# thangvubk/SoftGroup

Measured on AMD Instinct MI355X. Metric: scans/sec ScanNet-v2-like inference (softgroup_scannet.yaml, full forward_test), higher is better.
Workload: dtype f32

## Files before the change

### include/softgroup_hip.h

```cpp
#ifndef SOFTGROUP_HIP_H
#define SOFTGROUP_HIP_H

#include <stddef.h>
#include <stdint.h>

#ifdef __cplusplus
extern "C" {
#endif

typedef void *sg_stream_t;

#define SG_OK 0
#define SG_ERR_ARG (-1)
#define SG_ERR_WORKSPACE (-2)
#define SG_ERR_LAUNCH (-3)
#define SG_ERR_UNSUPPORTED (-4)

#define SG_BALLQUERY_MAX_NEIGHBORS 1000
#define SG_OCTREE_NUM_NODES 585
#define SG_OCTREE_NUM_LEAVES 512
#define SG_LISTS_SORTED 1
#define SG_LISTS_RADIUS 2

int sg_version(void);
const char *sg_last_error(void);
int sg_device_info(char *name_host, int name_cap, int *num_cu_host, int *clock_khz_host);

int sg_stream_release(sg_stream_t stream);
int sg_stream_create(sg_stream_t *stream_out);
int sg_stream_destroy(sg_stream_t stream);
int sg_stream_create_priority(sg_stream_t *stream_out, int level);

int sg_voxelize_idx_host(const int64_t *coords_host, int n, int ncol, int mode,
                         int32_t *input_map_host, int32_t *num_voxels_host,
                         int32_t *max_active_host);
int sg_voxelize_idx_fill_host(const int64_t *coords_host, int n, int ncol, int mode,
                              const int32_t *input_map_host, int num_voxels, int max_active,
                              int64_t *out_coords_host, int32_t *out_map_host);
size_t sg_voxelize_idx_workspace_bytes(int n);
int sg_voxelize_idx_build(const int64_t *coords, int n, int ncol, int mode, int32_t *input_map,
                          int32_t *meta, void *ws, size_t ws_bytes, sg_stream_t stream);
int sg_voxelize_idx_fill(const int64_t *coords, int n, int ncol, int mode,
                         const int32_t *input_map, int num_voxels, int max_active,
                         int64_t *out_coords, int32_t *out_map, void *ws, size_t ws_bytes,
                         sg_stream_t stream);

int sg_voxelize_fp(const float *feats, const int32_t *rules, int num_voxels, int max_active,
                   int channels, int average, float *out, sg_stream_t stream);
int sg_voxelize_bp(const float *d_out, const int32_t *rules, int num_voxels, int max_active,
                   int channels, int average, float *d_feats, sg_stream_t stream);

size_t sg_ballquery_workspace_bytes(int n);
int sg_ballquery_build_grid(const float *xyz, const int32_t *batch_idxs, int n, float radius,
                            void *ws, size_t ws_bytes, sg_stream_t stream);
int sg_ballquery_count(const float *xyz, const int32_t *batch_idxs, int n, float radius,
                       int32_t *start_len, int32_t *meta, void *ws, size_t ws_bytes,
                       sg_stream_t stream);
int sg_ballquery_fill(const float *xyz, const int32_t *batch_idxs, int n, float radius,
                      const int32_t *start_len, int32_t *idx, void *ws, size_t ws_bytes,
                      sg_stream_t stream);
size_t sg_scan_workspace_bytes(int n);
int sg_exclusive_scan_startlen(int32_t *start_len, int n, int32_t *meta, void *ws,
                               size_t ws_bytes, sg_stream_t stream);

int sg_octree_build_host(const float *points_host, const float *xyzwhl_host, int num_points,
                         int num_levels, float *boxes_host, int32_t *pt_inds_host,
                         int32_t *pt_start_len_host);
size_t sg_octree_build_workspace_bytes(int n);
int sg_octree_build(const float *points, int n, float *boxes, int32_t *pt_inds, int32_t *pt_start_len,
                    void *ws, size_t ws_bytes, sg_stream_t stream);
size_t sg_pyramid_inverse_map_workspace_bytes(int n_points, int n_voxels, int n_prop);
int sg_pyramid_inverse_map(const int32_t *proposals_idx, int64_t num_pairs, int n_prop,
                           const int32_t *l2p_map, int n_points, int n_voxels, int32_t *out_idx,
                           int32_t *out_offsets, int32_t *n_out_dev, void *ws, size_t ws_bytes,
                           sg_stream_t stream);
int sg_octree_ballquery_count(const float *points, const float *boxes, const int32_t *pt_inds,
                              const int32_t *pt_start_len, int n, float radius,
                              int32_t *start_len, sg_stream_t stream);
int sg_octree_ballquery_fill(const float *points, const float *boxes, const int32_t *pt_inds,
                             const int32_t *pt_start_len, int n, float radius,
                             const int32_t *start_len, int32_t *idx, sg_stream_t stream);

size_t sg_bfs_workspace_bytes(int n, int64_t n_edges);
int sg_bfs_cluster_label(const int32_t *bq_idxs, const int32_t *start_len, int n,
// ... 558 lines not shown
```

### softgroup_amd/_lib.py

```python
import ctypes as C
import os

_HERE = os.path.dirname(os.path.abspath(__file__))
LIB_PATH = os.path.join(_HERE, 'lib', os.environ.get('SG_LIB_NAME', 'libsoftgroup_hip.so'))

_lib = None

_vp, _i, _f, _i64, _sz, _d = C.c_void_p, C.c_int, C.c_float, C.c_int64, C.c_size_t, C.c_double
_pi32 = C.POINTER(C.c_int32)

SIGNATURES = {
    'sg_version': (_i, []),
    'sg_last_error': (C.c_char_p, []),
    'sg_device_info': (_i, [C.c_char_p, _i, C.POINTER(_i), C.POINTER(_i)]),
    'sg_stream_release': (_i, [_vp]),
    'sg_host_copy_2d': (_i, [_vp, _i64, _vp, _i64, _i64, _i64]),
    'sg_host_cast_f64_f32': (_i, [_vp, _vp, _i64]),
    'sg_host_fill_i64_strided': (_i, [_vp, _i64, _i64, _i64]),
    'sg_host_colmax_i64': (_i, [_vp, _i64, _i64, _vp]),
    'sg_stream_create': (_i, [_vp]),
    'sg_stream_create_priority': (_i, [_vp, _i]),
    'sg_stream_destroy': (_i, [_vp]),
    'sg_voxelize_idx_host': (_i, [_vp, _i, _i, _i, _vp, _pi32, _pi32]),
    'sg_voxelize_idx_fill_host': (_i, [_vp, _i, _i, _i, _vp, _i, _i, _vp, _vp]),
    'sg_voxelize_idx_workspace_bytes': (_sz, [_i]),
    'sg_voxelize_idx_build': (_i, [_vp, _i, _i, _i, _vp, _vp, _vp, _sz, _vp]),
    'sg_voxelize_idx_fill': (_i, [_vp, _i, _i, _i, _vp, _i, _i, _vp, _vp, _vp, _sz, _vp]),
    'sg_voxelize_fp': (_i, [_vp, _vp, _i, _i, _i, _i, _vp, _vp]),
    'sg_voxelize_bp': (_i, [_vp, _vp, _i, _i, _i, _i, _vp, _vp]),
    'sg_ballquery_workspace_bytes': (_sz, [_i]),
    'sg_ballquery_build_grid': (_i, [_vp, _vp, _i, _f, _vp, _sz, _vp]),
    'sg_ballquery_count': (_i, [_vp, _vp, _i, _f, _vp, _vp, _vp, _sz, _vp]),
    'sg_ballquery_fill': (_i, [_vp, _vp, _i, _f, _vp, _vp, _vp, _sz, _vp]),
    'sg_scan_workspace_bytes': (_sz, [_i]),
    'sg_exclusive_scan_startlen': (_i, [_vp, _i, _vp, _vp, _sz, _vp]),
    'sg_octree_build_host': (_i, [_vp, _vp, _i, _i, _vp, _vp, _vp]),
    'sg_octree_build_workspace_bytes': (_sz, [_i]),
    'sg_octree_build': (_i, [_vp, _i, _vp, _vp, _vp, _vp, _sz, _vp]),
    'sg_pyramid_inverse_map_workspace_bytes': (_sz, [_i, _i, _i]),
    'sg_pyramid_inverse_map': (_i, [_vp, _i64, _i, _vp, _i, _i, _vp, _vp, _vp, _vp, _sz, _vp]),
    'sg_octree_ballquery_count': (_i, [_vp, _vp, _vp, _vp, _i, _f, _vp, _vp]),
    'sg_octree_ballquery_fill': (_i, [_vp, _vp, _vp, _vp, _i, _f, _vp, _vp, _vp]),
    'sg_bfs_workspace_bytes': (_sz, [_i, _i64]),
    'sg_bfs_cluster_label': (_i, [_vp, _vp, _i, _i64, _i, _vp, _vp, _i, _pi32, _pi32, _vp, _sz, _vp]),
    'sg_bfs_cluster_emit': (_i, [_vp, _vp, _i, _i64, _vp, _vp, _i, _i, _vp, _vp, _vp, _sz, _vp]),
    'sg_sec_mean': (_i, [_vp, _vp, _i, _i, _vp, _vp]),
    'sg_sec_min': (_i, [_vp, _vp, _i, _i, _vp, _vp]),
    'sg_sec_max': (_i, [_vp, _vp, _i, _i, _vp, _vp]),
    'sg_global_avg_pool_fp': (_i, [_vp, _vp, _i, _i, _vp, _vp]),
    'sg_global_avg_pool_bp': (_i, [_vp, _vp, _vp, _i, _i, _vp]),
    'sg_get_mask_iou_on_cluster': (_i, [_vp, _vp, _vp, _vp, _i, _i, _vp, _vp]),
    'sg_get_mask_iou_on_pred': (_i, [_vp, _vp, _vp, _vp, _vp, _i, _i, _vp, _vp]),
    'sg_get_mask_label': (_i, [_vp, _vp, _vp, _vp, _vp, _i, _i, _f, _vp, _vp]),
    'sg_spconv_hash_workspace_bytes': (_sz, [_i]),
    'sg_spconv_subm_rulebook': (_i, [_vp, _i, _pi32, _vp, _vp, _sz, _vp]),
    'sg_spconv_pyramid_workspace_bytes': (_sz, [_i, _i]),
    'sg_spconv_pyramid_rows': (_i, [_vp, _i, _pi32, _i, _vp, _vp, _sz, _vp]),
    'sg_spconv_pyramid_build_workspace_bytes': (_sz, [_vp, _i]),
    'sg_spconv_pyramid_build': (_i, [_vp, _i, _pi32, _i, _vp, _vp, _sz, _vp, _sz, _vp]),
    'sg_spconv_down_build': (_i, [_vp, _i, _pi32, _vp, _vp, _vp, _sz, _vp]),
    'sg_spconv_down_fill': (_i, [_vp, _i, _vp, _i, _vp, _vp, _vp, _sz, _vp]),
    'sg_spconv_inverse_rulebook': (_i, [_vp, _vp, _i, _vp, _vp]),
    'sg_spconv_plan_workspace_bytes': (_sz, [_i]),
    'sg_spconv_plan': (_i, [_vp, _i, _i, _vp, _vp, _vp, _vp, _sz, _vp]),
    'sg_spconv_set_arithmetic': (_i, [_i]),
    'sg_spconv_set_combine': (_i, [_i]),
    'sg_spconv_set_chain': (_i, [_i]),
    'sg_spconv_chain_stats': (_i, [_vp, _vp]),
# ... 162 lines not shown
```

### softgroup_amd/csrc/bfs.hip

```cpp
#include <stdlib.h>

#include <map>
#include <mutex>
#include <utility>

#include "common.h"
#include "scan.h"

namespace sg {

constexpr int kCap = SG_BALLQUERY_MAX_NEIGHBORS;
constexpr int kEmitThreads = 512;
constexpr int kEmitWaves = kEmitThreads / 64;

#define SG_LD(p) __hip_atomic_load((p), __ATOMIC_RELAXED, __HIP_MEMORY_SCOPE_AGENT)
#define SG_ST(p, v) __hip_atomic_store((p), (v), __ATOMIC_RELAXED, __HIP_MEMORY_SCOPE_AGENT)

struct BfsWs {
  int32_t *parent, *lab, *size, *cid, *coff, *owner, *seeds, *ebase, *wcnt, *asym_nodes;
  int4 *label;
  int2 *erec;
  int32_t *counters;
  void *scan_ws;
  size_t scan_bytes;
  int32_t *big_stage[2];
  unsigned long long *big_rec[2];
};

constexpr int kBigFastWgs = 16;
constexpr int kBigSlice = 8192;
constexpr int kBigClusterMin = 16384;
inline bool big_fast_on() {
  const char *e = getenv("SG_BFS_BIG_FAST");
  return !(e && atoi(e) == 0);
}
inline int thin_levels_on() {
  const char *e = getenv("SG_BFS_THIN");
  return e ? atoi(e) : 0;
}
inline bool big_local_on() {
  const char *e = getenv("SG_BFS_BIG_LOCAL");
  return !(e && atoi(e) == 0);
}
inline size_t big_stage_entries(int n) {
  return n > kBigClusterMin && big_fast_on() ? static_cast<size_t>(n) + static_cast<size_t>(kBigFastWgs) * kBigSlice : 0;
}

static bool bfs_carve(void *ws, size_t ws_bytes, int n, int64_t n_edges, BfsWs *w) {
  Workspace a(ws, ws_bytes);
  const size_t nn = static_cast<size_t>(n > 0 ? n : 1);
  w->parent = a.take<int32_t>(nn);
  w->lab = a.take<int32_t>(nn);
  w->label = a.take<int4>(nn);
  w->size = a.take<int32_t>(nn);
  w->cid = a.take<int32_t>(nn);
  w->coff = a.take<int32_t>(nn);
  w->owner = a.take<int32_t>(nn);
  w->seeds = a.take<int32_t>(nn);
  w->ebase = a.take<int32_t>(nn);
  w->wcnt = a.take<int32_t>(nn);
  w->asym_nodes = a.take<int32_t>(nn);
  w->counters = a.take<int32_t>(64);
  w->scan_bytes = scan_workspace_bytes(n);
  w->scan_ws = a.take<char>(w->scan_bytes);
  w->erec = a.take<int2>(static_cast<size_t>(n_edges > 0 ? n_edges : 1));
  bool ok = w->scan_ws != nullptr && w->erec != nullptr;
  const size_t be = big_stage_entries(n);
  for (int i = 0; i < 2; ++i) {
    w->big_stage[i] = be ? a.take<int32_t>(be) : nullptr;
    w->big_rec[i] = be ? a.take<unsigned long long>(be) : nullptr;
    ok = ok && (be == 0 || (w->big_stage[i] != nullptr && w->big_rec[i] != nullptr));
  }
  return ok;
}

__device__ __forceinline__ int uf_find(int32_t *parent, int x) {
  int cur = SG_LD(&parent[x]);
  if (cur != x) {
    int prev = x, next;
    while (cur > (next = SG_LD(&parent[cur]))) {
      SG_ST(&parent[prev], next);
      prev = cur;
      cur = next;
    }
  }
  return cur;
}

__device__ __forceinline__ void uf_union(int32_t *parent, int a, int b) {
  while (a != b) {
    if (a < b) { const int t = a; a = b; b = t; }
    const int old = atomicCAS(&parent[a], a, b);
    if (old == a) return;
    a = uf_find(parent, old);
    b = uf_find(parent, b);
  }
}

__device__ __forceinline__ bool list_has_sorted(const int32_t *__restrict__ lst, int len, int key) {
  int lo = 0, hi = len;
  while (lo < hi) {
    const int mid = (lo + hi) >> 1;
    const int v = lst[mid];
    if (v < key) lo = mid + 1; else hi = mid;
  }
  return lo < len && lst[lo] == key;
}

__global__ void __launch_bounds__(256) bfs_init_kernel(int n, int32_t *parent, int32_t *size,
                                                      int32_t *owner) {
  const int i = blockIdx.x * 256 + threadIdx.x;
  if (i < n) {
    parent[i] = i;
    size[i] = 0;
    owner[i] = 0x7fffffff;
  }
}

constexpr int kSample = 2;
template <int SAMPLE>
__global__ void __launch_bounds__(256) bfs_union_kernel(const int32_t *__restrict__ idx,
                                                       const int32_t *__restrict__ start_len, int n,
                                                       int lists_sorted, int radius_lists,
                                                       int32_t *parent, int32_t *asym_nodes,
                                                       int32_t *counters) {
  const int wave = threadIdx.x >> 6, lane = threadIdx.x & 63;
  for (int u = blockIdx.x * 4 + wave; u < n; u += gridDim.x * 4) {
    const int st = start_len[2 * u], ln_all = start_len[2 * u + 1];
    const int ln = SAMPLE ? min(ln_all, kSample) : ln_all;
    const bool u_capped = ln_all >= kCap;
    bool any_asym = false;
    const int ru = SAMPLE ? -1 : SG_LD(&parent[u]);
    for (int p0 = 0; p0 < ln; p0 += 64) {
      const int p = p0 + lane;
      const int v = p < ln ? idx[st + p] : u;
      bool sym = true;
      if (v != u) {
        const int vst = start_len[2 * v], vln = start_len[2 * v + 1];
        if (!radius_lists || u_capped || vln >= kCap) {
          if (lists_sorted) {
            sym = list_has_sorted(idx + vst, vln, u);
          } else {
            sym = false;
            for (int j = 0; j < vln; ++j)
              if (idx[vst + j] == u) { sym = true; break; }
          }
        }
        if (sym) {
          if (v < u && (SAMPLE || SG_LD(&parent[v]) != ru)) uf_union(parent, uf_find(parent, u), uf_find(parent, v));
        }
      }
      any_asym |= !sym;
    }
    if (!SAMPLE && __any(any_asym)) {
      if (lane == 0) asym_nodes[atomicAdd(&counters[0], 1)] = u;
    }
  }
}

__global__ void __launch_bounds__(256) bfs_hook_min_kernel(const int32_t *__restrict__ idx,
                                                          const int32_t *__restrict__ start_len, int n,
                                                          int lists_sorted, int radius_lists, int32_t *parent) {
  const int u = blockIdx.x * 256 + threadIdx.x;
  if (u >= n) return;
// ... 1404 lines not shown
  std::lock_guard<std::mutex> g(g_bfs_mu);
  auto it = g_bfs_side.find({dev, stream});
  if (it == g_bfs_side.end()) return;
  if (it->second.side) {
    hipStreamSynchronize(it->second.side);
    hipStreamDestroy(it->second.side);
    hipEventDestroy(it->second.fork);
    hipEventDestroy(it->second.join);
    hipEventDestroy(it->second.back);
  }
  g_bfs_side.erase(it);
}
struct BfsLabelNote {
  const void *ws = nullptr;
  int max_kept = -1;
};
static thread_local BfsLabelNote t_bfs_note;

void bfs_emit_defer(BfsDefer *d) { t_bfs_defer = d; }
int bfs_emit_join(const BfsDefer &d, hipStream_t stream) {
  if (!d.deferred) return SG_OK;
  BfsSide *side = bfs_side(stream);
  if (side == nullptr || side->side != d.side || hipEventRecord(side->join, side->side) != hipSuccess ||
      hipStreamWaitEvent(stream, side->join, 0) != hipSuccess) {
    set_error("bfs_emit_join: joining the side stream failed");
    return SG_ERR_LAUNCH;
  }
  return SG_OK;
}
int bfs_label_max_kept(const void *ws) { return t_bfs_note.ws == ws ? t_bfs_note.max_kept : -1; }

__global__ void __launch_bounds__(256) bfs_kept_members_kernel(const int32_t *__restrict__ l2p, int n_pts,
                                                              const int4 *__restrict__ label,
                                                              const int32_t *__restrict__ size,
                                                              const float *__restrict__ thr_dev,
                                                              int32_t *__restrict__ out) {
  __shared__ int wsum[4];
  const float thr = thr_dev[0];
  int mine = 0;
  for (int p = blockIdx.x * 256 + threadIdx.x; p < n_pts; p += gridDim.x * 256)
    mine += static_cast<float>(size[label[l2p[p]].x]) >= thr ? 1 : 0;
  const int w = wave_sum(mine);
  if ((threadIdx.x & 63) == 0) wsum[threadIdx.x >> 6] = w;
  __syncthreads();
  if (threadIdx.x == 0) atomicAdd(out, wsum[0] + wsum[1] + wsum[2] + wsum[3]);
}
int bfs_count_kept_members(const void *ws, size_t ws_bytes, int n, int64_t n_edges, const int32_t *l2p, int n_pts,
                           const float *thr_dev, int32_t *out, hipStream_t stream) {
  BfsWs w;
  if (!bfs_carve(const_cast<void *>(ws), ws_bytes, n, n_edges, &w)) {
    set_error("bfs_count_kept_members: workspace too small");
    return SG_ERR_WORKSPACE;
  }
  hipMemsetAsync(out, 0, 4, stream);
  bfs_kept_members_kernel<<<grid_for(n_pts, 256, 1024), 256, 0, stream>>>(l2p, n_pts, w.label, w.size, thr_dev, out);
  return check_launch("bfs_count_kept_members");
}

}

using namespace sg;

extern "C" {

size_t sg_bfs_workspace_bytes(int n, int64_t n_edges) {
  const size_t nn = static_cast<size_t>(n > 0 ? n : 1);
  const size_t ne = static_cast<size_t>(n_edges > 0 ? n_edges : 1);
  const size_t be = big_stage_entries(n);
  return 14 * align_up(nn * 4) + align_up(64 * 4) + align_up(scan_workspace_bytes(n)) +
         align_up(ne * sizeof(int2)) + 2 * (align_up(be * 4) + align_up(be * 8)) + 256;
}

int sg_bfs_cluster_label(const int32_t *bq_idxs, const int32_t *start_len, int n, int64_t n_edges,
                         int list_flags, const int32_t *seg_of_point, const float *seg_thr,
                         int n_seg, int32_t *n_cluster_host, int32_t *sum_npoint_host, void *ws,
                         size_t ws_bytes, sg_stream_t stream_) {
  SG_REQUIRE(n >= 0 && n_seg >= 1 && seg_thr != nullptr, "sg_bfs_cluster_label: bad arguments");
  hipStream_t stream = as_stream(stream_);
  BfsWs w;
  if (!bfs_carve(ws, ws_bytes, n, n_edges, &w)) {
    set_error("sg_bfs_cluster_label: workspace too small");
    return SG_ERR_WORKSPACE;
  }
  *n_cluster_host = 0;
  *sum_npoint_host = 0;
  if (n == 0) return SG_OK;
  const int grid = (n + 255) / 256;
  hipMemsetAsync(w.counters, 0, 64 * 4, stream);
  bfs_init_kernel<<<grid, 256, 0, stream>>>(n, w.parent, w.size, w.owner);
  static const bool one_pass = getenv("SG_BFS_ONE_PASS") != nullptr;
  if (!one_pass) {
    static const bool sample_env = getenv("SG_BFS_SAMPLE") != nullptr;
    if (sample_env || !(list_flags & SG_LISTS_SORTED))
      bfs_union_kernel<1><<<grid_for(n, 4, 256 * 16), 256, 0, stream>>>(bq_idxs, start_len, n,
                                                                      list_flags & SG_LISTS_SORTED,
                                                                      list_flags & SG_LISTS_RADIUS,
                                                                      w.parent, w.asym_nodes, w.counters);
    else
      bfs_hook_min_kernel<<<grid, 256, 0, stream>>>(bq_idxs, start_len, n, list_flags & SG_LISTS_SORTED,
                                                   list_flags & SG_LISTS_RADIUS, w.parent);
    bfs_compress_kernel<<<grid, 256, 0, stream>>>(n, w.parent);
  }
  bfs_union_kernel<0><<<grid_for(n, 4, 256 * 16), 256, 0, stream>>>(bq_idxs, start_len, n,
                                                                  list_flags & SG_LISTS_SORTED,
                                                                  list_flags & SG_LISTS_RADIUS,
                                                                  w.parent, w.asym_nodes, w.counters);
  bfs_flatten_kernel<<<grid, 256, 0, stream>>>(n, w.parent, w.lab);
  bfs_store_root_kernel<<<grid, 256, 0, stream>>>(n, w.lab, w.parent);

  int32_t *host_counters = pinned_words();
  SG_REQUIRE(host_counters != nullptr, "sg_bfs_cluster_label: pinned allocation failed");
  for (int i = 0; i < 5; ++i) host_counters[i] = 0;
  for (int pass = 0; pass < 2; ++pass) {
    if (pass == 1) {
      const int n_asym = host_counters[0];
      while (true) {
        hipMemsetAsync(w.counters + 1, 0, 4, stream);
        bfs_propagate_kernel<<<grid_for(n_asym, 4, 256 * 16), 256, 0, stream>>>(
            bq_idxs, start_len, w.asym_nodes, n_asym, w.parent, w.lab, w.counters);
        host_counters[8] = 0;
        hipMemcpyAsync(host_counters + 8, w.counters + 1, 4, hipMemcpyDeviceToHost, stream);
        if (hipStreamSynchronize(stream) != hipSuccess) return check_launch("bfs propagate");
        if (!host_counters[8]) break;
      }
      bfs_zero_size_kernel<<<grid, 256, 0, stream>>>(n, w.size);
    }
    bfs_label_kernel<<<grid, 256, 0, stream>>>(n, w.parent, w.lab, start_len, w.label, w.size);
    const int4 *label = w.label;
    const int32_t *size = w.size;
    int32_t *cid = w.cid, *coff = w.coff;
    auto keep = [label, size, seg_of_point, seg_thr] __device__(int64_t i) -> int {
      if (label[i].x != static_cast<int32_t>(i)) return 0;
      const float thr = seg_thr[seg_of_point ? seg_of_point[i] : 0];
      return static_cast<float>(size[i]) >= thr ? 1 : 0;
    };
    int32_t *max_kept = w.counters + 4;
    auto keep_size = [keep, size, max_kept] __device__(int64_t i) -> int {
      const int s = keep(i) ? size[i] : 0;
      if (s > kBigMin) atomicMax(max_kept, s);
      return s;
    };
    int rc = exclusive_scan(keep, [cid] __device__(int64_t i, int v) { cid[i] = v; }, n,
                            w.counters + 2, w.scan_ws, w.scan_bytes, stream);
    if (rc != SG_OK) return rc;
    rc = exclusive_scan(keep_size, [coff] __device__(int64_t i, int v) { coff[i] = v; }, n,
                        w.counters + 3, w.scan_ws, w.scan_bytes, stream);
    if (rc != SG_OK) return rc;
    hipMemcpyAsync(host_counters, w.counters, 5 * sizeof(int32_t), hipMemcpyDeviceToHost, stream);
    if (hipStreamSynchronize(stream) != hipSuccess) return check_launch("sg_bfs_cluster_label");
    if (host_counters[0] == 0) break;
    if (pass == 0) hipMemsetAsync(w.counters + 4, 0, 4, stream);
  }
  *n_cluster_host = host_counters[2];
  *sum_npoint_host = host_counters[3];
  t_bfs_note.ws = ws;
  t_bfs_note.max_kept = host_counters[4];
  return check_launch("sg_bfs_cluster_label");
}

int sg_bfs_cluster_emit(const int32_t *bq_idxs, const int32_t *start_len, int n, int64_t n_edges,
                        const int32_t *seg_of_point, const float *seg_thr, int n_cluster,
                        int sum_npoint, int32_t *cluster_idxs, int32_t *cluster_offsets, void *ws,
                        size_t ws_bytes, sg_stream_t stream_) {
  SG_REQUIRE(n >= 0 && n_cluster >= 0 && sum_npoint >= 0, "sg_bfs_cluster_emit: bad arguments");
  hipStream_t stream = as_stream(stream_);
  BfsWs w;
  if (!bfs_carve(ws, ws_bytes, n, n_edges, &w)) {
    set_error("sg_bfs_cluster_emit: workspace too small");
    return SG_ERR_WORKSPACE;
  }
  if (n_cluster == 0 || n == 0) {
    hipMemsetAsync(cluster_offsets, 0, 4, stream);
    return SG_OK;
  }
  bfs_seed_kernel<<<(n + 255) / 256, 256, 0, stream>>>(n, w.label, w.size, w.cid, w.coff,
                                                       seg_of_point, seg_thr, w.seeds,
                                                       cluster_offsets);
  bfs_edge_rec_kernel<<<grid_for(n, 4, 256 * 16), 256, 0, stream>>>(bq_idxs, w.label, w.cid, w.seeds, n,
                                                                     n_cluster, w.erec);
  static const bool want_stats = getenv("SG_BFS_STATS") != nullptr;
  int32_t *stats = nullptr;
  if (want_stats) {
    hipMalloc(&stats, 256 * 8 * 4);
    hipMemsetAsync(stats, 0, 256 * 8 * 4, stream);
  }
  static const bool big_on = !(getenv("SG_BFS_BIG") && atoi(getenv("SG_BFS_BIG")) == 0);
  const bool noted = t_bfs_note.ws == ws && t_bfs_note.max_kept >= 0;
  const bool has_big = big_on && n < (1 << 21) && sum_npoint > kBigMin && (!noted || t_bfs_note.max_kept > kBigMin);
  t_bfs_note.ws = nullptr;
  static const bool side_env = !(getenv("SG_BFS_BIG_SIDE") && atoi(getenv("SG_BFS_BIG_SIDE")) == 0);
  BfsSide *side = has_big && side_env && !want_stats ? bfs_side(stream) : nullptr;
  hipStream_t main_stream = stream;
  BfsDefer *defer = t_bfs_defer;
  t_bfs_defer = nullptr;
  if (defer != nullptr) defer->deferred = false;
  if (side != nullptr) {
    if (hipEventRecord(side->fork, stream) != hipSuccess || hipStreamWaitEvent(side->side, side->fork, 0) != hipSuccess) {
      set_error("sg_bfs_cluster_emit: forking the side stream failed");
      return SG_ERR_LAUNCH;
    }
  }
  bfs_emit_kernel<<<min(n_cluster, 4096), kEmitThreads, 0, stream>>>(
      bq_idxs, start_len, w.label, w.erec, w.seeds, cluster_offsets, n_cluster, w.owner, cluster_idxs,
      stats, big_on && n < (1 << 21) ? kBigMin : 0x7fffffff, -1, nullptr, thin_levels_on());
  if (side != nullptr) stream = side->side;
  if (has_big) {
    static const int big_wgs_env = getenv("SG_BFS_BIG_WGS") ? atoi(getenv("SG_BFS_BIG_WGS")) : 16;
    const int big_wgs = big_wgs_env < 8 ? 8 : big_wgs_env > kBigWgsMax ? kBigWgsMax : big_wgs_env;
    int32_t *sync = w.asym_nodes;
    static const bool flags_on = getenv("SG_BFS_BIG_FLAGS") && atoi(getenv("SG_BFS_BIG_FLAGS")) != 0;
    if (static_cast<size_t>(n) >= static_cast<size_t>(kBigSyncWords)) {
      hipMemsetAsync(sync, 0, kBigSyncWords * 4, stream);
      if (const char *e = getenv("SG_BFS_FORCE_FALLBACK"))
        if (atoi(e) & 1) hipMemsetAsync(sync + 1, 1, 1, stream);
      const int32_t *gate = nullptr;
      if (big_local_on() && big_fast_on() && w.big_stage[0] != nullptr &&
          static_cast<size_t>(n) >= static_cast<size_t>(kBigSyncWords) + 96) {
        const int lw_env = getenv("SG_BFS_BIG_LOCAL_WGS") ? atoi(getenv("SG_BFS_BIG_LOCAL_WGS")) : 16;
        const int lw = lw_env < 8 ? 8 : lw_env > kBigWgsMax ? kBigWgsMax : lw_env;
        const int every_env = getenv("SG_BFS_BIG_LOCAL_EVERY") ? atoi(getenv("SG_BFS_BIG_LOCAL_EVERY")) : 4;
        const int warm_env = getenv("SG_BFS_BIG_LOCAL_WARM") ? atoi(getenv("SG_BFS_BIG_LOCAL_WARM")) : 8;
        const int every = every_env < 1 ? 1 : every_env, warm = warm_env < 1 ? 1 : warm_env;
        const bool novis = getenv("SG_BFS_BIG_LOCAL_NOVIS") && atoi(getenv("SG_BFS_BIG_LOCAL_NOVIS")) != 0;
        int32_t *sync3 = sync + kBigSyncWords;
        const size_t rows = big_stage_entries(n) / (2 * static_cast<size_t>(lw));
// ... 93 lines not shown
```

### softgroup_amd/csrc/common.h

```cpp
#pragma once
#include <hip/hip_runtime.h>
#include <stdint.h>
#include <stdio.h>

#include "../../include/softgroup_hip.h"

namespace sg {

constexpr int kWave = 64;

void set_error(const char *fmt, ...);
int32_t *pinned_words();

inline hipStream_t as_stream(sg_stream_t s) { return reinterpret_cast<hipStream_t>(s); }

inline int check_launch(const char *what) {
  hipError_t e = hipGetLastError();
  if (e != hipSuccess) {
    set_error("%s: %s", what, hipGetErrorString(e));
    return SG_ERR_LAUNCH;
  }
  return SG_OK;
}

#define SG_REQUIRE(cond, ...)      \
  do {                             \
    if (!(cond)) {                 \
      sg::set_error(__VA_ARGS__);  \
      return SG_ERR_ARG;           \
    }                              \
  } while (0)

inline size_t align_up(size_t x, size_t a = 256) { return (x + a - 1) / a * a; }

struct Workspace {
  char *base;
  size_t size, off;
  Workspace(void *p, size_t n) : base(static_cast<char *>(p)), size(n), off(0) {}
  template <typename T>
  T *take(size_t count) {
    size_t bytes = align_up(count * sizeof(T));
    if (off + bytes > size) return nullptr;
    T *r = reinterpret_cast<T *>(base + off);
    off += bytes;
    return r;
  }
};

inline int grid_for(int64_t work_items, int block, int max_blocks = 256 * 8) {
  int64_t g = (work_items + block - 1) / block;
  if (g < 1) g = 1;
  if (g > max_blocks) g = max_blocks;
  return static_cast<int>(g);
}

__device__ __forceinline__ int lane_id() { return threadIdx.x & 63; }

__device__ __forceinline__ uint64_t mix64(uint64_t x) {
  x ^= x >> 33;
  x *= 0xff51afd7ed558ccdULL;
  x ^= x >> 33;
  x *= 0xc4ceb9fe1a85ec53ULL;
  return x ^ (x >> 33);
}

__device__ __forceinline__ int mask_prefix(uint64_t m) {
  return __builtin_amdgcn_mbcnt_hi(static_cast<uint32_t>(m >> 32),
                                   __builtin_amdgcn_mbcnt_lo(static_cast<uint32_t>(m), 0u));
}

template <int CTRL, int ROW_MASK = 0xf, int BANK_MASK = 0xf>
__device__ __forceinline__ int dpp_or_zero(int v) {
  return __builtin_amdgcn_update_dpp(0, v, CTRL, ROW_MASK, BANK_MASK, false);
}
__device__ __forceinline__ int wave_incl_scan(int v) {
  v += dpp_or_zero<0x111>(v);
  v += dpp_or_zero<0x112>(v);
  v += dpp_or_zero<0x114>(v);
  v += dpp_or_zero<0x118>(v);
  v += dpp_or_zero<0x142, 0xa>(v);
  v += dpp_or_zero<0x143, 0xc>(v);
  return v;
}
__device__ __forceinline__ int wave_sum(int v) {
  return __builtin_amdgcn_readlane(wave_incl_scan(v), 63);
}
__device__ __forceinline__ int wave_max(int v) {
#pragma unroll
  for (int o = 32; o > 0; o >>= 1) v = max(v, __shfl_xor(v, o, 64));
  return v;
}

constexpr int kFillMax = 16;
struct FillList {
  uint32_t *p[kFillMax];
  size_t words[kFillMax];
  uint32_t pattern[kFillMax];
  int n = 0;
  void add(void *ptr, size_t bytes, int byte) {
    if (bytes == 0 || ptr == nullptr || n >= kFillMax) return;
    p[n] = static_cast<uint32_t *>(ptr);
    words[n] = bytes / 4;
    pattern[n] = 0x01010101u * static_cast<uint32_t>(byte & 0xff);
    ++n;
  }
};
static __global__ void __launch_bounds__(256) fill_many_kernel(FillList f) {
  const int r = blockIdx.y;
  uint32_t *p = f.p[r];
  const size_t w = f.words[r];
  const uint32_t v = f.pattern[r];
  const size_t head = (16 - (reinterpret_cast<uintptr_t>(p) & 15)) / 4 % 4;
  const size_t h = head < w ? head : w;
  const size_t quads = (w - h) / 4;
  uint4 *q = reinterpret_cast<uint4 *>(p + h);
  const uint4 vv = make_uint4(v, v, v, v);
  for (size_t i = blockIdx.x * 256ull + threadIdx.x; i < quads; i += gridDim.x * 256ull) q[i] = vv;
  if (blockIdx.x == 0) {
    if (threadIdx.x < h) p[threadIdx.x] = v;
    const size_t t0 = h + quads * 4;
    if (threadIdx.x < w - t0) p[t0 + threadIdx.x] = v;
  }
}
inline void fill_many(const FillList &f, hipStream_t stream) {
  if (f.n == 0) return;
  size_t mx = 0;
  for (int i = 0; i < f.n; ++i) mx = f.words[i] > mx ? f.words[i] : mx;
  const int gx = grid_for(static_cast<int64_t>(mx / 4 + 1), 256, 1024);
  fill_many_kernel<<<dim3(gx, f.n), 256, 0, stream>>>(f);
}

extern thread_local int t_conv_arith;
void conv_chain_begin(hipStream_t stream);
bool conv_chain_recording();
int conv_chain_end();
void conv_chain_abort();
int conv_chain_concat(const float *a, const float *b, int64_t rows, int ca, int cb, const float *scale,
                      const float *shift, float *out, float *out_act);
int conv_chain_bn_relu(const float *x, const float *scale, const float *shift, int64_t rows, int c, float *out);
int conv_chain_check_abort(const char *who);
int conv_gather_rows(const void *in, int num_in_rows, const int32_t *nbr, int M_out, int K, int Cin, int Cout,
                     const float *w_k8, const float *post_scale, const float *post_shift, const void *residual,
                     const float *act_scale, const float *act_shift, void *out_act, const int32_t *order,
                     const uint32_t *tile_mask, const int32_t *nbr_tiles, void *out, void *ws, size_t ws_bytes,
                     sg_stream_t stream, int in16, int out16, int res16);
int spconv_wgrad_layout(const void *in, int in_bf16, const void *g_out, int g_bf16, const int32_t *nbr_t, int M_out,
                        int K, int Cin, int Cout, float *dw, int out_oki, void *ws, size_t ws_bytes,
                        sg_stream_t stream);
struct PackJob {
  const float *w;
  float *out;
  int cout, kvol, cin, mode;
};
int spconv_pack_weights(const PackJob *jobs, int n, sg_stream_t stream);
size_t octree_stash_bytes(int n);
int octree_ballquery_count_stash(const float *points, const float *boxes, const int32_t *pt_inds,
                                 const int32_t *pt_start_len, int n, float radius, int32_t *start_len, int32_t *stash,
                                 hipStream_t stream);
int octree_ballquery_fill_stash(const float *points, const float *boxes, const int32_t *pt_inds,
                                const int32_t *pt_start_len, int n, float radius, const int32_t *start_len,
                                const int32_t *stash, int32_t *idx, hipStream_t stream);
void conv_release_stream(int dev, hipStream_t stream);
void unet_release_stream(int dev, hipStream_t stream);
void scan_release_stream(int dev, hipStream_t stream);
void bfs_release_stream(int dev, hipStream_t stream);
constexpr int kBfsGiantMin = 16384;
struct BfsDefer {
  bool deferred = false;
  hipStream_t side = nullptr;
};
void bfs_emit_defer(BfsDefer *d);
int bfs_emit_join(const BfsDefer &d, hipStream_t stream);
int bfs_label_max_kept(const void *ws);
int bfs_count_kept_members(const void *ws, size_t ws_bytes, int n, int64_t n_edges, const int32_t *l2p, int n_pts,
                           const float *thr_dev, int32_t *out, hipStream_t stream);

}
```

### softgroup_amd/csrc/core.hip

```cpp
#include <stdarg.h>
#include <string.h>

#include "common.h"
#include "scan.h"

namespace sg {

static thread_local char g_err[512] = "";

int32_t *pinned_words() {
  static thread_local int32_t *p = nullptr;
  if (p == nullptr && hipHostMalloc(reinterpret_cast<void **>(&p), 256) != hipSuccess) p = nullptr;
  return p;
}

void set_error(const char *fmt, ...) {
  va_list ap;
  va_start(ap, fmt);
  vsnprintf(g_err, sizeof(g_err), fmt, ap);
  va_end(ap);
}

__global__ void __launch_bounds__(kScanBlock) scan_block_sums_kernel(int32_t *block_sums,
                                                                    int num_blocks,
                                                                    int32_t *total_out) {
  __shared__ int lds4[4];
  int carry = 0;
  for (int base = 0; base < num_blocks; base += kScanBlock) {
    int idx = base + threadIdx.x;
    int v = idx < num_blocks ? block_sums[idx] : 0;
    int tot;
    int incl = block_incl_scan_256(v, lds4, &tot);
    if (idx < num_blocks) block_sums[idx] = carry + incl - v;
    carry += tot;
  }
  if (threadIdx.x == 0 && total_out) *total_out = carry;
}

void launch_scan_block_sums(int32_t *block_sums, int num_blocks, int32_t *total_out,
                            hipStream_t stream) {
  scan_block_sums_kernel<<<1, kScanBlock, 0, stream>>>(block_sums, num_blocks, total_out);
}

}

extern "C" {

int sg_version(void) { return 1; }

const char *sg_last_error(void) { return sg::g_err; }

int sg_device_info(char *name_host, int name_cap, int *num_cu_host, int *clock_khz_host) {
  int dev = 0;
  if (hipGetDevice(&dev) != hipSuccess) {
    sg::set_error("sg_device_info: no HIP device");
    return SG_ERR_LAUNCH;
  }
  hipDeviceProp_t p;
  if (hipGetDeviceProperties(&p, dev) != hipSuccess) return SG_ERR_LAUNCH;
  if (name_host && name_cap > 0) {
    snprintf(name_host, name_cap, "%s (%s)", p.name, p.gcnArchName);
  }
  if (num_cu_host) *num_cu_host = p.multiProcessorCount;
  if (clock_khz_host) *clock_khz_host = p.clockRate;
  return SG_OK;
}

int sg_stream_release(sg_stream_t stream) {
  int dev = 0;
  if (hipGetDevice(&dev) != hipSuccess) {
    sg::set_error("sg_stream_release: no HIP device");
    return SG_ERR_LAUNCH;
  }
  sg::conv_release_stream(dev, sg::as_stream(stream));
  sg::unet_release_stream(dev, sg::as_stream(stream));
  sg::scan_release_stream(dev, sg::as_stream(stream));
  sg::bfs_release_stream(dev, sg::as_stream(stream));
  return SG_OK;
}

int sg_stream_create(sg_stream_t *stream_out) {
  SG_REQUIRE(stream_out != nullptr, "sg_stream_create: null argument");
  hipStream_t s = nullptr;
  if (hipStreamCreateWithFlags(&s, hipStreamNonBlocking) != hipSuccess) {
    sg::set_error("sg_stream_create: hipStreamCreateWithFlags failed");
    return SG_ERR_LAUNCH;
  }
  *stream_out = reinterpret_cast<sg_stream_t>(s);
  return SG_OK;
}

int sg_stream_create_priority(sg_stream_t *stream_out, int level) {
  SG_REQUIRE(stream_out != nullptr, "sg_stream_create_priority: null argument");
  int least = 0, greatest = 0;
  if (hipDeviceGetStreamPriorityRange(&least, &greatest) != hipSuccess) {
    sg::set_error("sg_stream_create_priority: hipDeviceGetStreamPriorityRange failed");
    return SG_ERR_LAUNCH;
  }
  const int prio = level > 0 ? greatest : level < 0 ? least : (least + greatest) / 2;
  hipStream_t s = nullptr;
  if (hipStreamCreateWithPriority(&s, hipStreamNonBlocking, prio) != hipSuccess) {
    sg::set_error("sg_stream_create_priority: hipStreamCreateWithPriority failed");
    return SG_ERR_LAUNCH;
  }
  *stream_out = reinterpret_cast<sg_stream_t>(s);
  return SG_OK;
}

int sg_stream_destroy(sg_stream_t stream) {
  SG_REQUIRE(stream != nullptr, "sg_stream_destroy: the null stream is not the library's");
  hipStream_t s = sg::as_stream(stream);
  if (hipStreamSynchronize(s) != hipSuccess) {
    sg::set_error("sg_stream_destroy: synchronising the stream failed");
    return SG_ERR_LAUNCH;
  }
  const int rc = sg_stream_release(stream);
  if (rc != SG_OK) return rc;
  if (hipStreamDestroy(s) != hipSuccess) {
    sg::set_error("sg_stream_destroy: hipStreamDestroy failed");
    return SG_ERR_LAUNCH;
  }
  return SG_OK;
}

size_t sg_scan_workspace_bytes(int n) { return sg::scan_workspace_bytes(n); }

int sg_exclusive_scan_startlen(int32_t *start_len, int n, int32_t *meta, void *ws, size_t ws_bytes,
                               sg_stream_t stream) {
  SG_REQUIRE(n >= 0, "sg_exclusive_scan_startlen: n < 0");
  auto in = [start_len] __device__(int64_t i) { return start_len[2 * i + 1]; };
  auto out = [start_len] __device__(int64_t i, int v) { start_len[2 * i] = v; };
  return sg::exclusive_scan(in, out, n, meta, ws, ws_bytes, sg::as_stream(stream));
}

}
```

### softgroup_amd/csrc/instances.hip

```cpp
#include <stdlib.h>

#include <mutex>

#include "common.h"
#include "scan.h"

namespace sg {

__global__ void __launch_bounds__(256) instance_npoint_kernel(const int32_t *__restrict__ pairs,
                                                             const float *__restrict__ mask_scores,
                                                             int64_t S, int stride, float thr, int nc,
                                                             int32_t *__restrict__ npoint) {
  const int lane = threadIdx.x & 63;
  const int64_t n_waves = static_cast<int64_t>(gridDim.x) * 4;
  const int64_t per = (((S + n_waves - 1) / n_waves) + 63) & ~63LL;
  const int64_t begin = (static_cast<int64_t>(blockIdx.x) * 4 + (threadIdx.x >> 6)) * per;
  const int64_t end = begin + per < S ? begin + per : S;
  int cur = -1, acc = 0;
  auto flush = [&]() {
    if (cur >= 0 && lane < nc && acc) atomicAdd(&npoint[static_cast<int64_t>(cur) * nc + lane], acc);
    acc = 0;
  };
  for (int64_t e0 = begin; e0 < end; e0 += 64) {
    const int64_t e = e0 + lane;
// ... 366 lines not shown
    }
    __syncthreads();
    long long ti = 0, tc = 0;
    for (int v = 0; v < kFuseThreads / 64; ++v) {
      ti += red[par][0][v];
      tc += red[par][1][v];
    }
    const bool paste_it = !(static_cast<double>(ti) / (static_cast<double>(tc) + 1e-5) > skip_iou);
    if (paste_it) {
      if (threadIdx.x == 0) label_of_id[next_id] = label_id[k] + cls_offset;
      for (int w = threadIdx.x; w < words; w += kFuseThreads) {
        uint32_t paste = row[w] & ~taken[w];
        if (paste == 0u) continue;
        taken[w] |= paste;
        while (paste) {
          const int bb = __ffs(static_cast<int>(paste)) - 1;
          paste &= paste - 1;
          ids[w * 32 + bb] = static_cast<uint32_t>(next_id);
        }
      }
      ++next_id;
    }
  }
}

__global__ void __launch_bounds__(256) panoptic_encode_kernel(const uint32_t *__restrict__ ids,
                                                             const uint32_t *__restrict__ id_of_rank,
                                                             const int32_t *__restrict__ label_of_id,
                                                             const int64_t *__restrict__ semantic_preds, int n_points,
                                                             int semantic_classes, int thing_class_min,
                                                             uint32_t *__restrict__ out) {
  for (int i = blockIdx.x * 256 + threadIdx.x; i < n_points; i += gridDim.x * 256) {
    uint32_t id = ids[i];
    if (id_of_rank) id = id == 0xffffffffu ? 0u : id_of_rank[id];
    const uint32_t cls = id ? static_cast<uint32_t>(label_of_id[id]) : static_cast<uint32_t>(semantic_preds[i]);
    uint32_t v = (cls & 0xFFFFu) | (id << 16);
    if (cls >= static_cast<uint32_t>(thing_class_min) && id == 0u) v = static_cast<uint32_t>(semantic_classes);
    out[i] = v;
  }
}

}

using namespace sg;

extern "C" {

int sg_instance_npoint(const int32_t *proposals_idx, const float *mask_scores, int64_t S, int stride,
                       int n_classes, float mask_thr, int n_prop, int32_t *npoint,
                       sg_stream_t stream_) {
  SG_REQUIRE(S >= 0 && stride >= n_classes && n_classes >= 1 && n_prop >= 0,
             "sg_instance_npoint: bad arguments");
  hipStream_t stream = as_stream(stream_);
  hipMemsetAsync(npoint, 0, static_cast<size_t>(n_prop) * n_classes * 4, stream);
  if (S == 0 || n_prop == 0) return check_launch("sg_instance_npoint");
  const int grid = grid_for((S + 63) / 64, 4, 1024);
  instance_npoint_kernel<<<grid, 256, 0, stream>>>(proposals_idx, mask_scores, S, stride, mask_thr,
                                                  n_classes, npoint);
  return check_launch("sg_instance_npoint");
}

static int64_t instance_words(int n_points) { return (static_cast<int64_t>(n_points) + 31) / 32; }

size_t sg_instance_runs_workspace_bytes(int n_kept, int n_points) {
  const int64_t tw = static_cast<int64_t>(n_kept > 0 ? n_kept : 1) * instance_words(n_points);
  return align_up(tw * 4) * 2 + align_up(scan_workspace_bytes(tw)) + 512;
}

int sg_instance_runs(const int32_t *proposals_idx, const float *mask_scores, int64_t S, int stride,
                     int n_classes, float mask_thr, const int32_t *inst_of, int n_prop, int n_kept,
                     int n_points, int32_t *starts, int32_t *ends, int64_t *bounds,
                     int64_t runs_capacity, void *ws, size_t ws_bytes, sg_stream_t stream_) {
  SG_REQUIRE(S >= 0 && stride >= n_classes && n_classes >= 1 && n_prop >= 0 && n_kept >= 0 &&
                 n_points >= 0 && runs_capacity >= 0,
             "sg_instance_runs: bad arguments");
  hipStream_t stream = as_stream(stream_);
  if (n_kept == 0) return SG_OK;
  const int words = static_cast<int>(instance_words(n_points));
  const int64_t tw = static_cast<int64_t>(n_kept) * words;
  SG_REQUIRE(tw < (1LL << 31), "sg_instance_runs: %d instances x %d points exceed the bitmap limit",
             n_kept, n_points);
  SG_REQUIRE(ws != nullptr && ws_bytes >= sg_instance_runs_workspace_bytes(n_kept, n_points),
             "sg_instance_runs: workspace too small");
  Workspace a(ws, ws_bytes);
  uint32_t *bits = a.take<uint32_t>(tw);
  int32_t *base = a.take<int32_t>(tw);
  const size_t sbytes = scan_workspace_bytes(tw);
  void *sws = a.take<char>(sbytes);
  int32_t *total = a.take<int32_t>(64);
  hipMemsetAsync(bits, 0, static_cast<size_t>(tw) * 4, stream);
  if (S > 0 && n_prop > 0) {
    const int grid = grid_for(S, 256, 4096);
    instance_bitmap_kernel<<<grid, 256, 0, stream>>>(proposals_idx, mask_scores, S, stride, mask_thr,
                                                    n_classes, inst_of, n_prop, words, bits);
  }
  const uint32_t *cb = bits;
  const int w = words;
  int rc = exclusive_scan(
      [cb, w] __device__(int64_t t) { return __popc(run_starts(cb, t, static_cast<int>(t % w))); },
      [base] __device__(int64_t t, int v) { base[t] = v; }, tw, total, sws, sbytes, stream);
  if (rc != SG_OK) return rc;
  instance_runs_emit_kernel<<<grid_for(tw, 256, 4096), 256, 0, stream>>>(bits, tw, words, base, starts,
                                                                        ends, bounds, runs_capacity);
  instance_runs_total_kernel<<<1, 1, 0, stream>>>(total, n_kept, bounds);
  return check_launch("sg_instance_runs");
}


size_t sg_rle_format_device_workspace_bytes(int64_t run_capacity) {
  const int64_t n = run_capacity > 0 ? run_capacity : 1;
  return align_up(static_cast<size_t>(n) * 4) + align_up(scan_workspace_bytes(n)) + 512;
}

int64_t sg_rle_format_device_text_bytes(int64_t run_capacity, int64_t length) {
  int d = 1;
  for (int64_t v = length + 1; v >= 10; v /= 10) ++d;
  return (run_capacity > 0 ? run_capacity : 1) * (2LL * d + 2);
}

int sg_rle_format_device(const int32_t *starts, const int32_t *ends, const int64_t *bounds, int n_inst,
                         int64_t run_capacity, int64_t length, uint8_t *text, int64_t text_capacity,
                         int64_t *text_off, void *ws, size_t ws_bytes, sg_stream_t stream_) {
  SG_REQUIRE(n_inst >= 0 && run_capacity >= 0 && bounds && text_off && length >= 0 && length < (1LL << 31),
             "sg_rle_format_device: bad arguments");
  const int64_t need = sg_rle_format_device_text_bytes(run_capacity, length);
  SG_REQUIRE(need < (1LL << 31), "sg_rle_format_device: %lld runs exceed the 2 GiB text limit",
             static_cast<long long>(run_capacity));
  SG_REQUIRE(text != nullptr && text_capacity >= need,
             "sg_rle_format_device: text buffer %lld < %lld bytes (sg_rle_format_device_text_bytes)",
             static_cast<long long>(text_capacity), static_cast<long long>(need));
  SG_REQUIRE(ws != nullptr && ws_bytes >= sg_rle_format_device_workspace_bytes(run_capacity),
             "sg_rle_format_device: workspace too small");
  hipStream_t stream = as_stream(stream_);
  const int64_t n = run_capacity > 0 ? run_capacity : 1;
  Workspace a(ws, ws_bytes);
  int32_t *off = a.take<int32_t>(n);
  const size_t sbytes = scan_workspace_bytes(n);
  void *sws = a.take<char>(sbytes);
  int32_t *total = a.take<int32_t>(64);
  const int64_t *n_runs_p = bounds + n_inst;
  int rc = exclusive_scan(
      [starts, ends, n_runs_p] __device__(int64_t r) { return r < *n_runs_p ? run_text_len(starts, ends, r) : 0; },
      [off] __device__(int64_t r, int v) { off[r] = v; }, n, total, sws, sbytes, stream);
// ... 72 lines not shown
```

### softgroup_amd/csrc/radix_sort.h

```cpp
#pragma once
#include <mutex>

#include "common.h"
#include "scan.h"

namespace sg {

constexpr int kRsBlock = 256;
constexpr int kRsItems = 8;
constexpr int kRsTile = kRsBlock * kRsItems;
constexpr int kRsBuckets = 256;

inline size_t radix_sort_workspace_bytes(int64_t n) {
  const int64_t nblk = (n + kRsTile - 1) / kRsTile;
  const int64_t hist = nblk * kRsBuckets + 1;
  return align_up(hist * 4) + align_up(scan_workspace_bytes(hist) + 4 * kRsBuckets * 4) +
         2 * align_up(n * 4) + 256;
}

static __global__ void __launch_bounds__(kRsBlock) rs_hist_kernel(const uint32_t *__restrict__ keys,
                                                          int64_t n, int shift, int nblk, int items,
                                                          int32_t *__restrict__ hist,
                                                          int32_t *totals) {
  __shared__ int h[kRsBuckets];
// ... 103 lines not shown
    const int d = (key >> shift) & 0xff;
    const int off = base[d] + (e - dstart[d]);
    keys_out[off] = key;
    vals_out[off] = sval[e];
  }
}


static inline int radix_sort_pairs(uint32_t *keys, int32_t *vals, int64_t n, int num_bits, void *ws,
                            size_t ws_bytes, hipStream_t stream, uint32_t **keys_sorted,
                            int32_t **vals_sorted) {
  *keys_sorted = keys;
  *vals_sorted = vals;
  if (n <= 1 || num_bits <= 0) return SG_OK;
  if (ws_bytes < radix_sort_workspace_bytes(n)) {
    set_error("radix_sort_pairs: workspace too small");
    return SG_ERR_WORKSPACE;
  }
  int items = kRsItems;
  while (items < 64 && (n + static_cast<int64_t>(items) * kRsBlock - 1) / (static_cast<int64_t>(items) * kRsBlock) > 256)
    items *= 2;
  const int64_t tile = static_cast<int64_t>(items) * kRsBlock;
  const int nblk = static_cast<int>((n + tile - 1) / tile);
  const size_t lds = static_cast<size_t>(tile) * 8;
  {
    static std::mutex mu;
    static uint64_t done_mask = 0;
    int dev = 0;
    hipGetDevice(&dev);
    std::lock_guard<std::mutex> g(mu);
    if (dev < 0 || dev >= 64 || !((done_mask >> dev) & 1)) {
      if (hipFuncSetAttribute(reinterpret_cast<const void *>(rs_scatter_kernel),
                              hipFuncAttributeMaxDynamicSharedMemorySize, 64 * kRsBlock * 8) != hipSuccess) {
        (void)hipGetLastError();
        set_error("radix_sort_pairs: %d bytes of dynamic LDS are not available on this device (gfx950: 160 KB "
                  "per workgroup)", 64 * kRsBlock * 8);
        return SG_ERR_LAUNCH;
      }
      if (dev >= 0 && dev < 64) done_mask |= 1ull << dev;
    }
  }
  const int64_t hist_n = static_cast<int64_t>(nblk) * kRsBuckets;
  Workspace a(ws, ws_bytes);
  int32_t *hist = a.take<int32_t>(hist_n + 1);
  const size_t sbytes = scan_workspace_bytes(hist_n) + 4 * kRsBuckets * 4;
  void *sws = a.take<char>(sbytes);
  uint32_t *k2 = a.take<uint32_t>(n);
  int32_t *v2 = a.take<int32_t>(n);
  uint32_t *kin = keys, *kout = k2;
  int32_t *vin = vals, *vout = v2;
  const int n_pass = (num_bits + 7) / 8;
  const bool local_scan = nblk <= 256 && n_pass <= 4;
  int32_t *totals = static_cast<int32_t *>(sws);
  if (local_scan) hipMemsetAsync(totals, 0, static_cast<size_t>(n_pass) * kRsBuckets * 4, stream);
  for (int shift = 0, pass = 0; shift < num_bits; shift += 8, ++pass) {
    if (local_scan) {
      int32_t *t = totals + pass * kRsBuckets;
      rs_hist_kernel<<<nblk, kRsBlock, 0, stream>>>(kin, n, shift, nblk, items, hist, t);
      rs_scatter_kernel<<<nblk, kRsBlock, lds, stream>>>(kin, vin, n, shift, nblk, items, hist, t, kout, vout);
      if (const int rc = check_launch("radix_sort_pairs(scatter)"); rc != SG_OK) return rc;
    } else {
      rs_hist_kernel<<<nblk, kRsBlock, 0, stream>>>(kin, n, shift, nblk, items, hist, nullptr);
      int32_t *h = hist;
      int rc = exclusive_scan([h] __device__(int64_t i) { return h[i]; },
                              [h] __device__(int64_t i, int v) { h[i] = v; }, hist_n, nullptr, sws,
                              sbytes, stream);
      if (rc != SG_OK) return rc;
      rs_scatter_kernel<<<nblk, kRsBlock, lds, stream>>>(kin, vin, n, shift, nblk, items, hist, nullptr,
                                                         kout, vout);
      if (const int rc = check_launch("radix_sort_pairs(scatter)"); rc != SG_OK) return rc;
    }
    uint32_t *tk = kin; kin = kout; kout = tk;
    int32_t *tv = vin; vin = vout; vout = tv;
  }
  *keys_sorted = kin;
  *vals_sorted = vin;
  return check_launch("radix_sort_pairs");
}

}
```

### softgroup_amd/csrc/scan.h

```cpp
#pragma once
#include "common.h"

namespace sg {

constexpr int kScanBlock = 256;
constexpr int kScanItems = 8;
constexpr int kScanTile = kScanBlock * kScanItems;

inline size_t scan_workspace_bytes(int64_t n) {
  return align_up(((n + kScanTile - 1) / kScanTile + 1) * sizeof(int32_t));
}

__device__ __forceinline__ int block_incl_scan_256(int v, int *lds4, int *block_total) {
  const int w = threadIdx.x >> 6, l = threadIdx.x & 63;
  int s = wave_incl_scan(v);
  if (l == 63) lds4[w] = s;
  __syncthreads();
  int carry = 0;
#pragma unroll
  for (int i = 0; i < 4; ++i)
    if (i < w) carry += lds4[i];
  if (block_total) *block_total = lds4[0] + lds4[1] + lds4[2] + lds4[3];
  __syncthreads();
  return s + carry;
}

template <typename In>
__global__ void __launch_bounds__(kScanBlock) scan_reduce_kernel(In in, int64_t n,
                                                                int32_t *block_sums) {
  __shared__ int lds4[4];
  const int64_t base = static_cast<int64_t>(blockIdx.x) * kScanTile;
  int v = 0;
#pragma unroll
  for (int i = 0; i < kScanItems; ++i) {
    int64_t idx = base + i * kScanBlock + threadIdx.x;
    if (idx < n) v += in(idx);
  }
  v = wave_sum(v);
  if ((threadIdx.x & 63) == 0) lds4[threadIdx.x >> 6] = v;
  __syncthreads();
  if (threadIdx.x == 0) block_sums[blockIdx.x] = lds4[0] + lds4[1] + lds4[2] + lds4[3];
}

void launch_scan_block_sums(int32_t *block_sums, int num_blocks, int32_t *total_out,
                            hipStream_t stream);

constexpr int kScanRawBlocks = 2048;
template <typename In, typename Out, bool RAW = false>
__global__ void __launch_bounds__(kScanBlock) scan_apply_kernel(In in, Out out, int64_t n,
                                                               const int32_t *block_sums,
                                                               int32_t *total_out = nullptr) {
  __shared__ int lds4[4];
  __shared__ int carry_s;
  int carry_in = 0;
  if (RAW) {
    int v = 0;
    for (int b = threadIdx.x; b < static_cast<int>(blockIdx.x); b += kScanBlock) v += block_sums[b];
    v = wave_sum(v);
    if ((threadIdx.x & 63) == 0) lds4[threadIdx.x >> 6] = v;
    __syncthreads();
    if (threadIdx.x == 0) carry_s = lds4[0] + lds4[1] + lds4[2] + lds4[3];
    __syncthreads();
    carry_in = carry_s;
    if (total_out != nullptr && blockIdx.x == gridDim.x - 1 && threadIdx.x == 0)
      *total_out = carry_in + block_sums[blockIdx.x];
  }
  const int64_t base = static_cast<int64_t>(blockIdx.x) * kScanTile;
  const int64_t first = base + static_cast<int64_t>(threadIdx.x) * kScanItems;
  int vals[kScanItems];
  int tsum = 0;
#pragma unroll
  for (int i = 0; i < kScanItems; ++i) {
    int64_t idx = first + i;
    vals[i] = idx < n ? in(idx) : 0;
    tsum += vals[i];
  }
  int incl = block_incl_scan_256(tsum, lds4, nullptr);
  int run = (RAW ? carry_in : block_sums[blockIdx.x]) + incl - tsum;
#pragma unroll
  for (int i = 0; i < kScanItems; ++i) {
    int64_t idx = first + i;
    if (idx < n) out(idx, run);
    run += vals[i];
  }
}

template <typename In, typename Out>
int exclusive_scan(In in, Out out, int64_t n, int32_t *total_out, void *ws, size_t ws_bytes,
                   hipStream_t stream) {
  if (ws_bytes < scan_workspace_bytes(n)) {
    set_error("exclusive_scan: workspace too small (%zu < %zu)", ws_bytes, scan_workspace_bytes(n));
    return SG_ERR_WORKSPACE;
  }
  int32_t *block_sums = static_cast<int32_t *>(ws);
  int num_blocks = static_cast<int>((n + kScanTile - 1) / kScanTile);
  if (num_blocks == 0) {
    if (total_out) hipMemsetAsync(total_out, 0, sizeof(int32_t), stream);
    return SG_OK;
  }
  scan_reduce_kernel<<<num_blocks, kScanBlock, 0, stream>>>(in, n, block_sums);
  if (num_blocks <= kScanRawBlocks) {
    scan_apply_kernel<In, Out, true><<<num_blocks, kScanBlock, 0, stream>>>(in, out, n, block_sums, total_out);
  } else {
    launch_scan_block_sums(block_sums, num_blocks, total_out, stream);
    scan_apply_kernel<In, Out, false><<<num_blocks, kScanBlock, 0, stream>>>(in, out, n, block_sums);
  }
  return check_launch("exclusive_scan");
}

}
```

### softgroup_amd/csrc/scan_exec.hip

```cpp
#include <stdlib.h>
#include <string.h>

#include "common.h"
#include "scan.h"

namespace sg {

constexpr int kSelBlock = 256;
constexpr int kMaxSeg = 32;

__global__ void __launch_bounds__(kSelBlock) select_count_kernel(const float *__restrict__ scores, int n,
                                                                int n_cls, const int32_t *__restrict__ seg_class,
                                                                int n_seg, float thr, int n_blocks,
                                                                int32_t *__restrict__ blk_cnt) {
  __shared__ int part[4][kMaxSeg];
  const int i = blockIdx.x * kSelBlock + threadIdx.x;
  const int wave = threadIdx.x >> 6, lane = threadIdx.x & 63;
  for (int s = 0; s < n_seg; ++s) {
    const bool on = i < n && scores[static_cast<int64_t>(i) * n_cls + seg_class[s]] > thr;
    const int c = __popcll(__ballot(on));
    if (lane == 0) part[wave][s] = c;
  }
  __syncthreads();
  if (threadIdx.x < n_seg)
    blk_cnt[threadIdx.x * n_blocks + blockIdx.x] =
        part[0][threadIdx.x] + part[1][threadIdx.x] + part[2][threadIdx.x] + part[3][threadIdx.x];
}

__global__ void __launch_bounds__(1024) select_scan_kernel(const int32_t *__restrict__ blk_cnt, int n_seg,
                                                          int n_blocks, int min_npoint,
                                                          int32_t *__restrict__ blk_off,
                                                          int32_t *__restrict__ meta) {
  constexpr int kG = 8;
  __shared__ int seg_tot[kMaxSeg], seg_base[kMaxSeg + 1], carry_s[kMaxSeg];
  __shared__ int wtot[kG][16];
  const int wave = threadIdx.x >> 6, lane = threadIdx.x & 63;
  for (int s0 = 0; s0 < n_seg; s0 += kG) {
    int sum[kG];
#pragma unroll
    for (int j = 0; j < kG; ++j) sum[j] = 0;
    for (int b0 = 0; b0 < n_blocks; b0 += 1024) {
      const int b = b0 + threadIdx.x;
      int v[kG];
#pragma unroll
      for (int j = 0; j < kG; ++j) v[j] = (s0 + j < n_seg && b < n_blocks) ? blk_cnt[(s0 + j) * n_blocks + b] : 0;
#pragma unroll
      for (int j = 0; j < kG; ++j) sum[j] += v[j];
    }
#pragma unroll
    for (int j = 0; j < kG; ++j) {
      const int t = wave_sum(sum[j]);
      if (lane == 0) wtot[j][wave] = t;
    }
    __syncthreads();
    if (threadIdx.x < kG && s0 + threadIdx.x < n_seg) {
      int t = 0;
      for (int w = 0; w < 16; ++w) t += wtot[threadIdx.x][w];
      seg_tot[s0 + threadIdx.x] = t >= min_npoint ? t : 0;
    }
    __syncthreads();
  }
  if (threadIdx.x == 0) {
    int acc = 0;
    for (int s = 0; s < n_seg; ++s) {
      seg_base[s] = acc;
      carry_s[s] = acc;
      acc += seg_tot[s];
      meta[1 + s] = seg_tot[s];
    }
    seg_base[n_seg] = acc;
    meta[0] = acc;
  }
  __syncthreads();
  for (int s0 = 0; s0 < n_seg; s0 += kG) {
    for (int b0 = 0; b0 < n_blocks; b0 += 1024) {
      const int b = b0 + threadIdx.x;
      int v[kG], incl[kG];
#pragma unroll
      for (int j = 0; j < kG; ++j)
        v[j] = (s0 + j < n_seg && b < n_blocks && seg_tot[s0 + j] > 0) ? blk_cnt[(s0 + j) * n_blocks + b] : 0;
#pragma unroll
      for (int j = 0; j < kG; ++j) {
        incl[j] = wave_incl_scan(v[j]);
        if (lane == 63) wtot[j][wave] = incl[j];
      }
      __syncthreads();
#pragma unroll
      for (int j = 0; j < kG; ++j) {
        if (s0 + j < n_seg) {
          int before = 0, all = 0;
          for (int w = 0; w < 16; ++w) {
            const int x = wtot[j][w];
            before += w < wave ? x : 0;
            all += x;
          }
          if (b < n_blocks)
            blk_off[(s0 + j) * n_blocks + b] = seg_tot[s0 + j] > 0 ? carry_s[s0 + j] + before + incl[j] - v[j] : -1;
        }
      }
      __syncthreads();
      if (threadIdx.x < kG && s0 + threadIdx.x < n_seg) {
        int all = 0;
        for (int w = 0; w < 16; ++w) all += wtot[threadIdx.x][w];
        carry_s[s0 + threadIdx.x] += all;
      }
      __syncthreads();
    }
  }
}

__global__ void __launch_bounds__(kSelBlock) select_emit_kernel(
    const float *__restrict__ scores, int n, int n_cls, const int32_t *__restrict__ seg_class, int n_seg,
    float thr, int n_blocks, const int32_t *__restrict__ blk_off, const float *__restrict__ coords,
    const float *__restrict__ offsets, const int32_t *__restrict__ batch_idxs, int batch_size,
    int32_t *__restrict__ obj, int32_t *__restrict__ seg_of, float *__restrict__ pts, int32_t *__restrict__ key) {
  __shared__ int wcnt[4];
  const int i = blockIdx.x * kSelBlock + threadIdx.x;
  const int wave = threadIdx.x >> 6;
  float c[3] = {0.f, 0.f, 0.f};
  int bi = 0;
  if (i < n) {
#pragma unroll
    for (int a = 0; a < 3; ++a) c[a] = __fadd_rn(coords[3LL * i + a], offsets[3LL * i + a]);
    bi = batch_idxs[i];
  }
  for (int s = 0; s < n_seg; ++s) {
    const int base = blk_off[s * n_blocks + blockIdx.x];
    if (base < 0) continue;
    const bool on = i < n && scores[static_cast<int64_t>(i) * n_cls + seg_class[s]] > thr;
    const uint64_t m = __ballot(on);
    if ((threadIdx.x & 63) == 0) wcnt[wave] = __popcll(m);
    __syncthreads();
    int before = 0;
    for (int w = 0; w < wave; ++w) before += wcnt[w];
    if (on) {
      const int pos = base + before + mask_prefix(m);
      obj[pos] = i;
      seg_of[pos] = s;
      pts[3LL * pos] = c[0];
      pts[3LL * pos + 1] = c[1];
      pts[3LL * pos + 2] = c[2];
      key[pos] = s * batch_size + bi;
    }
    __syncthreads();
  }
}

__global__ void __launch_bounds__(256) proposal_map_kernel(int32_t *__restrict__ pairs, int64_t S,
                                                          const int32_t *__restrict__ obj) {
  for (int64_t e = blockIdx.x * 256LL + threadIdx.x; e < S; e += gridDim.x * 256LL)
    pairs[2 * e + 1] = obj[pairs[2 * e + 1]];
}

__global__ void __launch_bounds__(256) proposal_box_kernel(const int32_t *__restrict__ pairs,
                                                          const int32_t *__restrict__ offsets, int n_prop,
                                                          const float *__restrict__ coords, float inv_ss,
                                                          float scale_max, float *__restrict__ cscale,
                                                          float *__restrict__ lo_s) {
  __shared__ float rmin[3][256], rmax[3][256];
  for (int p = blockIdx.x; p < n_prop; p += gridDim.x) {
    const int s = offsets[p], e = offsets[p + 1];
    float mn[3] = {INFINITY, INFINITY, INFINITY}, mx[3] = {-INFINITY, -INFINITY, -INFINITY};
#pragma unroll 4
    for (int i = s + threadIdx.x; i < e; i += 256) {
      const int pt = pairs[2LL * i + 1];
#pragma unroll
      for (int a = 0; a < 3; ++a) {
        const float x = coords[3LL * pt + a];
        if (x < mn[a]) mn[a] = x;
        if (x > mx[a]) mx[a] = x;
      }
    }
#pragma unroll
    for (int a = 0; a < 3; ++a) {
      rmin[a][threadIdx.x] = mn[a];
      rmax[a][threadIdx.x] = mx[a];
    }
    __syncthreads();
    for (int w = 128; w > 0; w >>= 1) {
      if (threadIdx.x < w) {
#pragma unroll
        for (int a = 0; a < 3; ++a) {
          const float x = rmin[a][threadIdx.x + w], y = rmax[a][threadIdx.x + w];
          if (x < rmin[a][threadIdx.x]) rmin[a][threadIdx.x] = x;
          if (y > rmax[a][threadIdx.x]) rmax[a][threadIdx.x] = y;
        }
      }
      __syncthreads();
    }
    if (threadIdx.x == 0) {
      float ext = -INFINITY;
      bool nan = false;
#pragma unroll
      for (int a = 0; a < 3; ++a) {
        const float d = __fmul_rn(__fsub_rn(rmax[a][0], rmin[a][0]), inv_ss);
        nan |= d != d;
        if (d > ext) ext = d;
      }
      if (nan) ext = NAN;
      float cs = __fadd_rn(__fmul_rn(__fdiv_rn(1.0f, ext), 1.0f), -0.01f);
      cs = (cs != cs) ? cs : fminf(cs, scale_max);
      cscale[p] = cs;
#pragma unroll
      for (int a = 0; a < 3; ++a) lo_s[3 * p + a] = __fmul_rn(rmin[a][0], cs);
    }
    __syncthreads();
  }
}

__global__ void __launch_bounds__(256) proposal_voxel_coords_kernel(
    const int32_t *__restrict__ pairs, int64_t S, const float *__restrict__ coords,
    const float *__restrict__ cscale, const float *__restrict__ lo_s, int ss, int64_t *__restrict__ vox,
// ... 25 lines not shown
    const int32_t *r = rules + static_cast<int64_t>(row) * (max_active + 1);
    const int cnt = r[0];
    const float m = cnt > 0 ? __fdiv_rn(1.0f, static_cast<float>(cnt)) : 1.0f;
    float acc = 0.0f;
    int i = 1;
    for (; i + 15 <= cnt; i += 16) {
      int a[16], q[16];
      float f[16];
#pragma unroll
      for (int j = 0; j < 16; ++j) a[j] = r[i + j];
#pragma unroll
      for (int j = 0; j < 16; ++j) q[j] = pairs[2LL * a[j] + 1];
#pragma unroll
      for (int j = 0; j < 16; ++j) f[j] = feats[static_cast<int64_t>(q[j]) * C + c];
#pragma unroll
      for (int j = 0; j < 16; ++j) acc = __fadd_rn(acc, __fmul_rn(m, f[j]));
    }
    for (; i + 3 <= cnt; i += 4) {
      const int a0 = r[i], a1 = r[i + 1], a2 = r[i + 2], a3 = r[i + 3];
      const int p0 = pairs[2LL * a0 + 1], p1 = pairs[2LL * a1 + 1], p2 = pairs[2LL * a2 + 1],
                p3 = pairs[2LL * a3 + 1];
      const float f0 = feats[static_cast<int64_t>(p0) * C + c], f1 = feats[static_cast<int64_t>(p1) * C + c],
                  f2 = feats[static_cast<int64_t>(p2) * C + c], f3 = feats[static_cast<int64_t>(p3) * C + c];
      acc = __fadd_rn(acc, __fmul_rn(m, f0));
      acc = __fadd_rn(acc, __fmul_rn(m, f1));
      acc = __fadd_rn(acc, __fmul_rn(m, f2));
      acc = __fadd_rn(acc, __fmul_rn(m, f3));
    }
    for (; i <= cnt; ++i)
      acc = __fadd_rn(acc, __fmul_rn(m, feats[static_cast<int64_t>(pairs[2LL * r[i] + 1]) * C + c]));
    out[t] = acc;
  }
}

__global__ void __launch_bounds__(256) proposal_voxel_pack_kernel(const int64_t *__restrict__ vc, int M,
                                                                 int n_prop, int32_t *__restrict__ out,
                                                                 int32_t *__restrict__ vox_off) {
  for (int m = blockIdx.x * 256 + threadIdx.x; m < M; m += gridDim.x * 256) {
    const int p = static_cast<int>(vc[4LL * m]);
#pragma unroll
    for (int a = 0; a < 4; ++a) out[4LL * m + a] = static_cast<int32_t>(vc[4LL * m + a]);
    if (m == 0 || static_cast<int>(vc[4LL * (m - 1)]) != p) vox_off[p] = m;
    if (m == M - 1) vox_off[n_prop] = M;
  }
}

__global__ void __launch_bounds__(1024) instance_keep_kernel(const float *__restrict__ cls_prob,
                                                           const float *__restrict__ iou, int stride,
                                                           const int32_t *__restrict__ npoint, int n_prop,
                                                           int nc, float cls_thr, int min_npoint,
                                                           int32_t *__restrict__ inst_of,
                                                           int32_t *__restrict__ kept_cls,
                                                           float *__restrict__ kept_score,
                                                           int32_t *__restrict__ head) {
  __shared__ int wsum[16];
  __shared__ int cap_s;
  if (threadIdx.x == 0) cap_s = 0;
  __syncthreads();
  const int total = nc * n_prop;
  const int wave = threadIdx.x >> 6, lane = threadIdx.x & 63;
  int carry = 0, cap = 0;
  for (int base = 0; base < total; base += 1024) {
    const int t = base + threadIdx.x;
    int keep = 0, np = 0, i = 0, p = 0;
    if (t < total) {
      i = t / n_prop;
      p = t - i * n_prop;
      np = npoint[p * nc + i];
      keep = (cls_prob[p * stride + i] > cls_thr && np >= min_npoint) ? 1 : 0;
    }
    int incl = wave_incl_scan(keep);
    if (lane == 63) wsum[wave] = incl;
    __syncthreads();
    int tot = 0;
#pragma unroll
    for (int w = 0; w < 16; ++w) {
      const int x = wsum[w];
      incl += w < wave ? x : 0;
      tot += x;
    }
    __syncthreads();
    if (t < total) {
      const int k = carry + incl - keep;
      inst_of[t] = keep ? k : -1;
      if (keep) {
        kept_cls[k] = i + 1;
        const float q = iou[p * stride + i];
        const float qc = (q != q) ? q : fminf(fmaxf(q, 0.f), 1.f);
        kept_score[k] = __fmul_rn(cls_prob[p * stride + i], qc);
        cap += np;
      }
    }
    carry += tot;
  }
  cap = wave_sum(cap);
  if ((threadIdx.x & 63) == 0) atomicAdd(&cap_s, cap);
  __syncthreads();
  if (threadIdx.x == 0) {
    head[0] = carry;
    head[1] = cap_s;
  }
}

__global__ void __launch_bounds__(256) pp_level_inputs_kernel(const int32_t *__restrict__ obj, int n,
                                                             const float *__restrict__ coords,
                                                             const float *__restrict__ offsets,
                                                             const int32_t *__restrict__ batch_idxs, float inv,
                                                             int64_t *__restrict__ vox, float *__restrict__ c3,
                                                             float *__restrict__ o3) {
  const int i = blockIdx.x * 256 + threadIdx.x;
  if (i >= n) return;
  const int p = obj[i];
  vox[4LL * i] = batch_idxs[p];
#pragma unroll
  for (int a = 0; a < 3; ++a) {
    const float c = coords[3LL * p + a];
    c3[3LL * i + a] = c;
    o3[3LL * i + a] = offsets[3LL * p + a];
    vox[4LL * i + 1 + a] = static_cast<int64_t>(__fmul_rn(c, inv));
  }
}
__global__ void __launch_bounds__(256) pp_level_points_kernel(const float *__restrict__ cl, const float *__restrict__ ol,
                                                             const int64_t *__restrict__ vc, int m,
                                                             float *__restrict__ q, int32_t *__restrict__ qb) {
  const int i = blockIdx.x * 256 + threadIdx.x;
  if (i >= m) return;
#pragma unroll
  for (int a = 0; a < 3; ++a) q[3LL * i + a] = __fadd_rn(cl[3LL * i + a], ol[3LL * i + a]);
  qb[i] = static_cast<int32_t>(vc[4LL * i]);
}
__global__ void __launch_bounds__(256) pp_append_kernel(const int32_t *__restrict__ pairs, int rows,
                                                       const int32_t *__restrict__ offs, int n_prop,
                                                       const int32_t *__restrict__ obj, int prop_base, int row_base,
                                                       int32_t *__restrict__ out_pairs, int32_t *__restrict__ out_offs) {
  const int i = blockIdx.x * 256 + threadIdx.x;
  if (i < rows) {
    out_pairs[2LL * (row_base + i)] = pairs[2LL * i] + prop_base;
    out_pairs[2LL * (row_base + i) + 1] = obj[pairs[2LL * i + 1]];
  }
  if (i < n_prop) out_offs[prop_base + 1 + i] = offs[i + 1] + row_base;
  if (i == 0 && prop_base == 0) out_offs[0] = 0;
}

struct ScanArena {
  char *base;
  size_t cap, off;
  bool ok = true;
  ScanArena(void *p, size_t n) : base(static_cast<char *>(p)), cap(n), off(0) {}
  template <typename T>
  T *take(size_t count) {
    const size_t bytes = align_up((count ? count : 1) * sizeof(T));
    const size_t at = off;
    off += bytes;
    if (off > cap) {
      ok = false;
      return nullptr;
    }
    return reinterpret_cast<T *>(base + at);
  }
  size_t at(const void *p) const { return static_cast<size_t>(static_cast<const char *>(p) - base); }
};

__global__ void __launch_bounds__(64) read_back_kernel(const int32_t *__restrict__ dev, int words, int32_t *host) {
  if (static_cast<int>(threadIdx.x) < words)
    __hip_atomic_store(host + threadIdx.x, dev[threadIdx.x], __ATOMIC_RELAXED, __HIP_MEMORY_SCOPE_SYSTEM);
}
static int read_back(int32_t *host, const int32_t *dev, int words, hipStream_t stream, const char *what) {
  static const bool by_kernel = getenv("SG_READBACK_KERNEL") && atoi(getenv("SG_READBACK_KERNEL")) != 0;
  if (by_kernel && words <= 64) {
    read_back_kernel<<<1, 64, 0, stream>>>(dev, words, host);
    if (hipStreamSynchronize(stream) != hipSuccess) {
      set_error("%s: device -> host read-back failed", what);
      return SG_ERR_LAUNCH;
    }
    return SG_OK;
  }
  if (hipMemcpyAsync(host, dev, sizeof(int32_t) * words, hipMemcpyDeviceToHost, stream) != hipSuccess ||
      hipStreamSynchronize(stream) != hipSuccess) {
    set_error("%s: device -> host read-back failed", what);
    return SG_ERR_LAUNCH;
  }
  return SG_OK;
}

#define SG_TRY(expr)              \
  do {                            \
    const int rc_ = (expr);       \
    if (rc_ != SG_OK) return rc_; \
  } while (0)
#define SG_TAKE(var, T, count)                                                                    \
  T *var = ar.take<T>(count);                                                                     \
  if (var == nullptr) {                                                                           \
    res->arena_needed = ar.off + ar.off / 2 + (8 << 20);                                          \
    set_error("%s: arena too small (%zu bytes, need about %zu)", kWhat, ar.cap, res->arena_needed); \
    return SG_ERR_WORKSPACE;                                                                      \
  }

thread_local void (*t_scan_emit_hook)(void *) = nullptr;
thread_local void *t_scan_emit_ctx = nullptr;

}

using namespace sg;

static int voxelise_proposals(const sg_grouping_cfg *cfg, const int32_t *pairs, const int32_t *poff, int n_prop, int S,
                              const float *coords_float, const float *point_feats, ScanArena &ar, int32_t *meta,
                              int32_t *host, sg_grouping_result *res, sg_stream_t stream_, const char *kWhat) {
  hipStream_t stream = as_stream(stream_);
  const int C = cfg->feat_channels;
  SG_TAKE(cscale, float, n_prop);
  SG_TAKE(lo_s, float, 3 * static_cast<size_t>(n_prop));
  SG_TAKE(vox, int64_t, 4 * static_cast<size_t>(S));
  SG_TAKE(bad, int32_t, 64);
  hipMemsetAsync(bad, 0, sizeof(int32_t), stream);
  const float inv_ss = 1.0f / static_cast<float>(cfg->voxel_shape);
  proposal_box_kernel<<<n_prop < 1024 ? n_prop : 1024, 256, 0, stream>>>(pairs, poff, n_prop, coords_float, inv_ss,
                                                                        cfg->voxel_scale, cscale, lo_s);
  proposal_voxel_coords_kernel<<<grid_for(S, 256), 256, 0, stream>>>(pairs, S, coords_float, cscale, lo_s,
                                                                    cfg->voxel_shape, vox, bad);
  const size_t vx_bytes = sg_voxelize_idx_workspace_bytes(S);
  SG_TAKE(vx_ws, char, vx_bytes);
  SG_TAKE(inp_map, int32_t, S);
  SG_TRY(sg_voxelize_idx_build(vox, S, 4, 4, inp_map, meta + 40, vx_ws, vx_bytes, stream_));
  hipMemcpyAsync(meta + 42, bad, sizeof(int32_t), hipMemcpyDeviceToDevice, stream);
  SG_TRY(read_back(host, meta + 40, 3, stream, kWhat));
  const int M = host[0], mA = host[1];
  SG_REQUIRE(host[2] == 0, "%s: a proposal voxel coordinate fell outside [0, %d) "
             "(the reference asserts here, softgroup.py:698)", kWhat, cfg->voxel_shape);
  res->n_voxels = M;
  res->max_active = mA;
  SG_TAKE(vc64, int64_t, 4 * static_cast<size_t>(M));
  SG_TAKE(rules, int32_t, static_cast<size_t>(M) * (mA + 1));
  SG_TRY(sg_voxelize_idx_fill(vox, S, 4, 4, inp_map, M, mA, vc64, rules, vx_ws, vx_bytes, stream_));
  SG_TAKE(vc32, int32_t, 4 * static_cast<size_t>(M));
  SG_TAKE(vox_off, int32_t, static_cast<size_t>(n_prop) + 1);
  SG_TAKE(vfeat, float, static_cast<size_t>(M) * C);
  proposal_voxel_pack_kernel<<<grid_for(M, 256), 256, 0, stream>>>(vc64, M, n_prop, vc32, vox_off);
  proposal_voxel_feats_kernel<<<grid_for(static_cast<int64_t>(M) * C, 256), 256, 0, stream>>>(
      point_feats, pairs, rules, M, mA, C, vfeat);
  res->voxel_coords = ar.at(vc32);
  res->voxel_offsets = ar.at(vox_off);
  res->voxel_feats = ar.at(vfeat);
  res->point_to_voxel = ar.at(inp_map);
  res->arena_used = ar.off;
  return check_launch(kWhat);
}

extern "C" {

int sg_scan_grouping(const sg_grouping_cfg *cfg, const float *scores, const float *pt_offsets,
                     const float *coords_float, const int32_t *batch_idxs, const float *point_feats,
                     void *arena, size_t arena_bytes, sg_grouping_result *res, sg_stream_t stream_) {
  static const char *kWhat = "sg_scan_grouping";
  SG_REQUIRE(cfg != nullptr && res != nullptr, "sg_scan_grouping: null descriptor");
  SG_REQUIRE(cfg->n_points >= 0 && cfg->n_sem_classes >= 1 && cfg->n_seg >= 0 && cfg->n_seg <= kMaxSeg &&
                 cfg->batch_size >= 1 && cfg->feat_channels >= 1 && cfg->voxel_shape >= 0,
             "sg_scan_grouping: bad configuration (n_seg must be <= %d)", kMaxSeg);
  memset(res, 0, sizeof(*res));
  hipStream_t stream = as_stream(stream_);
  int32_t *host = pinned_words();
  SG_REQUIRE(host != nullptr, "sg_scan_grouping: no pinned host words");
  ScanArena ar(arena, arena_bytes);
  const int n = cfg->n_points, n_seg = cfg->n_seg;
  if (n == 0 || n_seg == 0) return SG_OK;

  const int n_blocks = (n + kSelBlock - 1) / kSelBlock;
  SG_TAKE(meta, int32_t, 64);
  SG_TAKE(blk_cnt, int32_t, static_cast<size_t>(n_seg) * n_blocks);
  SG_TAKE(blk_off, int32_t, static_cast<size_t>(n_seg) * n_blocks);
  select_count_kernel<<<n_blocks, kSelBlock, 0, stream>>>(scores, n, cfg->n_sem_classes, cfg->seg_class, n_seg,
                                                         cfg->score_thr, n_blocks, blk_cnt);
  select_scan_kernel<<<1, 1024, 0, stream>>>(blk_cnt, n_seg, n_blocks, cfg->min_npoint, blk_off, meta);
  SG_TRY(check_launch(kWhat));
  SG_TRY(read_back(host, meta, 1, stream, kWhat));
  const int n_sel = host[0];
  res->n_selected = n_sel;
  if (n_sel == 0) return SG_OK;
  SG_TAKE(obj, int32_t, n_sel);
  SG_TAKE(seg_of, int32_t, n_sel);
  SG_TAKE(pts, float, 3 * static_cast<size_t>(n_sel));
  SG_TAKE(key, int32_t, n_sel);
  select_emit_kernel<<<n_blocks, kSelBlock, 0, stream>>>(scores, n, cfg->n_sem_classes, cfg->seg_class, n_seg,
                                                        cfg->score_thr, n_blocks, blk_off, coords_float,
                                                        pt_offsets, batch_idxs, cfg->batch_size, obj, seg_of,
                                                        pts, key);

  const size_t bq_bytes = sg_ballquery_workspace_bytes(n_sel);
  SG_TAKE(bq_ws, char, bq_bytes);
  SG_TAKE(start_len, int32_t, 2 * static_cast<size_t>(n_sel));
  const size_t sc_bytes = sg_scan_workspace_bytes(n_sel);
  SG_TAKE(sc_ws, char, sc_bytes);
  hipMemsetAsync(start_len, 0, sizeof(int32_t) * 2 * n_sel, stream);
  SG_TRY(sg_ballquery_build_grid(pts, key, n_sel, cfg->radius, bq_ws, bq_bytes, stream_));
  SG_TRY(sg_ballquery_count(pts, key, n_sel, cfg->radius, start_len, nullptr, bq_ws, bq_bytes, stream_));
  SG_TRY(sg_exclusive_scan_startlen(start_len, n_sel, meta + 32, sc_ws, sc_bytes, stream_));
  SG_TRY(read_back(host, meta + 32, 1, stream, kWhat));
  const int n_active = host[0];
  res->n_neighbours = n_active;
  SG_TAKE(bq_idx, int32_t, n_active);
  SG_TRY(sg_ballquery_fill(pts, key, n_sel, cfg->radius, start_len, bq_idx, bq_ws, bq_bytes, stream_));

  const size_t bfs_bytes = sg_bfs_workspace_bytes(n_sel, n_active);
  SG_TAKE(bfs_ws, char, bfs_bytes);
  int32_t n_prop = 0, S = 0;
  SG_TRY(sg_bfs_cluster_label(bq_idx, start_len, n_sel, n_active, SG_LISTS_SORTED | SG_LISTS_RADIUS, seg_of,
                              cfg->seg_thr, n_seg, &n_prop, &S, bfs_ws, bfs_bytes, stream_));
  res->n_proposals = n_prop;
  res->sum_npoint = S;
  if (S == 0) return SG_OK;
  SG_TAKE(pairs, int32_t, 2 * static_cast<size_t>(S));
  SG_TAKE(poff, int32_t, static_cast<size_t>(n_prop) + 1);
  hipMemsetAsync(poff, 0, sizeof(int32_t) * (n_prop + 1), stream);
  if (t_scan_emit_hook != nullptr) t_scan_emit_hook(t_scan_emit_ctx);
  SG_TRY(sg_bfs_cluster_emit(bq_idx, start_len, n_sel, n_active, seg_of, cfg->seg_thr, n_prop, S, pairs, poff,
                             bfs_ws, bfs_bytes, stream_));
  proposal_map_kernel<<<grid_for(S, 256), 256, 0, stream>>>(pairs, S, obj);
  res->proposals_idx = ar.at(pairs);
  res->proposals_offset = ar.at(poff);
  if (cfg->voxel_shape == 0) {
    res->arena_used = ar.off;
    return check_launch(kWhat);
  }

  return voxelise_proposals(cfg, pairs, poff, n_prop, S, coords_float, point_feats, ar, meta, host, res, stream_, kWhat);
}

int sg_scan_grouping_pp(const sg_grouping_pp_cfg *pcfg, const float *scores, const float *pt_offsets,
                        const float *coords_float, const int32_t *batch_idxs, const float *point_feats,
                        void *arena, size_t arena_bytes, sg_grouping_result *res, sg_stream_t stream_) {
  static const char *kWhat = "sg_scan_grouping_pp";
  SG_REQUIRE(pcfg != nullptr && res != nullptr, "sg_scan_grouping_pp: null descriptor");
  const sg_grouping_cfg *cfg = &pcfg->base;
  SG_REQUIRE(cfg->n_points >= 0 && cfg->n_sem_classes >= 1 && cfg->n_seg >= 0 && cfg->n_seg <= kMaxSeg &&
                 cfg->batch_size >= 1 && cfg->feat_channels >= 1 && cfg->voxel_shape >= 0,
             "sg_scan_grouping_pp: bad configuration (n_seg must be <= %d)", kMaxSeg);
  SG_REQUIRE(pcfg->radius > 0 && (!pcfg->with_pyramid || pcfg->base_size > 0),
             "sg_scan_grouping_pp: radius and pyramid_base_size must be positive");
  memset(res, 0, sizeof(*res));
  hipStream_t stream = as_stream(stream_);
  int32_t *host = pinned_words();
  SG_REQUIRE(host != nullptr, "sg_scan_grouping_pp: no pinned host words");
  ScanArena ar(arena, arena_bytes);
  const int n = cfg->n_points, n_seg = cfg->n_seg;
  if (n == 0 || n_seg == 0) return SG_OK;

  const int n_blocks = (n + kSelBlock - 1) / kSelBlock;
  SG_TAKE(meta, int32_t, 128);
  SG_TAKE(blk_cnt, int32_t, static_cast<size_t>(n_seg) * n_blocks);
  SG_TAKE(blk_off, int32_t, static_cast<size_t>(n_seg) * n_blocks);
  select_count_kernel<<<n_blocks, kSelBlock, 0, stream>>>(scores, n, cfg->n_sem_classes, cfg->seg_class, n_seg,
                                                         cfg->score_thr, n_blocks, blk_cnt);
  select_scan_kernel<<<1, 1024, 0, stream>>>(blk_cnt, n_seg, n_blocks, cfg->min_npoint, blk_off, meta);
  SG_TRY(check_launch(kWhat));
  SG_TRY(read_back(host, meta, 1 + n_seg, stream, kWhat));
  const int n_sel = host[0];
  int count[kMaxSeg];
  for (int s = 0; s < n_seg; ++s) count[s] = host[1 + s];
  res->n_selected = n_sel;
  if (n_sel == 0) return SG_OK;
  SG_TAKE(obj, int32_t, n_sel);
  SG_TAKE(seg_of, int32_t, n_sel);
  SG_TAKE(pts, float, 3 * static_cast<size_t>(n_sel));
  SG_TAKE(key, int32_t, n_sel);
  select_emit_kernel<<<n_blocks, kSelBlock, 0, stream>>>(scores, n, cfg->n_sem_classes, cfg->seg_class, n_seg,
                                                        cfg->score_thr, n_blocks, blk_off, coords_float,
                                                        pt_offsets, batch_idxs, cfg->batch_size, obj, seg_of,
                                                        pts, key);
  SG_TAKE(pairs, int32_t, 2 * static_cast<size_t>(n_sel));
  SG_TAKE(poff, int32_t, static_cast<size_t>(n_sel) + 2);
  int n_prop = 0, S = 0;
  int64_t n_nbr = 0;
  const size_t loop_mark0 = ar.off;
  size_t loop_mark = loop_mark0;
  bool hook_pending = t_scan_emit_hook != nullptr;
  const bool defer_on = !(getenv("SG_PP_DEFER") && atoi(getenv("SG_PP_DEFER")) == 0);
  BfsDefer def;
  int def_rows = -1;
  bool def_mapped = false;
  struct DeferGuard {
    BfsDefer &d;
    ~DeferGuard() {
      if (d.deferred && d.side != nullptr) hipStreamSynchronize(d.side);
    }
  } defer_guard{def};
  int s0 = 0;
  for (int s = 0; s < n_seg; s0 += count[s], ++s) {
    const int nc_pts = count[s];
    if (nc_pts == 0) continue;
    ar.off = loop_mark;
    int level = 1;
    if (pcfg->with_pyramid) level = nc_pts > 1000000 ? 3 : nc_pts > 100000 ? 2 : 1;
    const float radius = static_cast<float>(pcfg->with_pyramid ? pcfg->radius * level : pcfg->radius);
    const bool mapped = pcfg->with_pyramid && (level > 1 || !pcfg->lvl_fusion);
    const float *q = pts + 3 * static_cast<size_t>(s0);
    const int32_t *qb = key + s0;
    int n_q = nc_pts, n_lvl = 0;
    const int32_t *l2p = nullptr;
    if (mapped) {
      const float inv = 1.0f / static_cast<float>(pcfg->base_size * level);
      SG_TAKE(vox, int64_t, 4 * static_cast<size_t>(nc_pts));
      SG_TAKE(c3, float, 3 * static_cast<size_t>(nc_pts));
      SG_TAKE(o3, float, 3 * static_cast<size_t>(nc_pts));
      pp_level_inputs_kernel<<<grid_for(nc_pts, 256, 1 << 22), 256, 0, stream>>>(obj + s0, nc_pts, coords_float, pt_offsets,
                                                                            batch_idxs, inv, vox, c3, o3);
      const size_t vx_bytes = sg_voxelize_idx_workspace_bytes(nc_pts);
      SG_TAKE(vx_ws, char, vx_bytes);
      SG_TAKE(l2p_, int32_t, nc_pts);
      SG_TRY(sg_voxelize_idx_build(vox, nc_pts, 4, 4, l2p_, meta + 40, vx_ws, vx_bytes, stream_));
      SG_TRY(read_back(host, meta + 40, 2, stream, kWhat));
      const int M = host[0], mA = host[1];
      SG_TAKE(vc64, int64_t, 4 * static_cast<size_t>(M));
      SG_TAKE(rules, int32_t, static_cast<size_t>(M) * (mA + 1));
      SG_TRY(sg_voxelize_idx_fill(vox, nc_pts, 4, 4, l2p_, M, mA, vc64, rules, vx_ws, vx_bytes, stream_));
      SG_TAKE(cl, float, 3 * static_cast<size_t>(M));
      SG_TAKE(ol, float, 3 * static_cast<size_t>(M));
      SG_TAKE(ql, float, 3 * static_cast<size_t>(M));
      SG_TAKE(qbl, int32_t, M);
      SG_TRY(sg_voxelize_fp(c3, rules, M, mA, 3, 1, cl, stream_));
      SG_TRY(sg_voxelize_fp(o3, rules, M, mA, 3, 1, ol, stream_));
      pp_level_points_kernel<<<grid_for(M, 256, 1 << 22), 256, 0, stream>>>(cl, ol, vc64, M, ql, qbl);
      q = ql;
      qb = qbl;
      n_q = n_lvl = M;
      l2p = l2p_;
    }
    SG_TAKE(start_len, int32_t, 2 * static_cast<size_t>(n_q));
    const size_t sc_bytes = sg_scan_workspace_bytes(n_q);
    SG_TAKE(sc_ws, char, sc_bytes);
    hipMemsetAsync(start_len, 0, sizeof(int32_t) * 2 * n_q, stream);
    int32_t *bq_idx = nullptr;
    int n_active = 0, flags = 0;
    if (pcfg->with_octree) {
      SG_TAKE(boxes, float, (1 + 8 + 64 + 512) * 6);
      SG_TAKE(pt_inds, int32_t, n_q);
      SG_TAKE(pt_sl, int32_t, 512 * 2);
      const size_t ob = sg_octree_build_workspace_bytes(n_q);
      SG_TAKE(o_ws, char, ob);
      SG_TAKE(stash, int32_t, octree_stash_bytes(n_q) / sizeof(int32_t));
      SG_TRY(sg_octree_build(q, n_q, boxes, pt_inds, pt_sl, o_ws, ob, stream_));
      SG_TRY(octree_ballquery_count_stash(q, boxes, pt_inds, pt_sl, n_q, radius, start_len, stash, stream));
      SG_TRY(sg_exclusive_scan_startlen(start_len, n_q, meta + 56, sc_ws, sc_bytes, stream_));
      SG_TRY(read_back(host, meta + 56, 1, stream, kWhat));
      n_active = host[0];
      SG_TAKE(idx_, int32_t, n_active);
      SG_TRY(octree_ballquery_fill_stash(q, boxes, pt_inds, pt_sl, n_q, radius, start_len, stash, idx_, stream));
      bq_idx = idx_;
      flags = SG_LISTS_RADIUS;
    } else {
      const size_t bq_bytes = sg_ballquery_workspace_bytes(n_q);
      SG_TAKE(bq_ws, char, bq_bytes);
      SG_TRY(sg_ballquery_build_grid(q, qb, n_q, radius, bq_ws, bq_bytes, stream_));
      SG_TRY(sg_ballquery_count(q, qb, n_q, radius, start_len, nullptr, bq_ws, bq_bytes, stream_));
      SG_TRY(sg_exclusive_scan_startlen(start_len, n_q, meta + 56, sc_ws, sc_bytes, stream_));
      SG_TRY(read_back(host, meta + 56, 1, stream, kWhat));
      n_active = host[0];
      SG_TAKE(idx_, int32_t, n_active);
      SG_TRY(sg_ballquery_fill(q, qb, n_q, radius, start_len, idx_, bq_ws, bq_bytes, stream_));
      bq_idx = idx_;
      flags = SG_LISTS_SORTED | SG_LISTS_RADIUS;
    }
    n_nbr += n_active;
    const size_t bfs_bytes = sg_bfs_workspace_bytes(n_q, n_active);
    SG_TAKE(bfs_ws, char, bfs_bytes);
    int32_t nc = 0, sp = 0;
    SG_TRY(sg_bfs_cluster_label(bq_idx, start_len, n_q, n_active, flags, nullptr, cfg->seg_thr + s, 1, &nc, &sp, bfs_ws,
                                bfs_bytes, stream_));
    if (sp == 0) continue;
    bool later = false;
    for (int t = s + 1; t < n_seg; ++t) later = later || count[t] > 0;
    const bool want_defer = defer_on && def_rows < 0 && later && bfs_label_max_kept(bfs_ws) > kBfsGiantMin;
    int rows = sp;
    if (want_defer && mapped) {
      SG_TRY(bfs_count_kept_members(bfs_ws, bfs_bytes, n_q, n_active, l2p, nc_pts, cfg->seg_thr + s, meta + 72, stream));
      SG_TRY(read_back(host, meta + 72, 1, stream, kWhat));
      rows = host[0];
    }
    SG_TAKE(cidx, int32_t, 2 * static_cast<size_t>(sp));
    SG_TAKE(coff, int32_t, static_cast<size_t>(nc) + 1);
    hipMemsetAsync(coff, 0, sizeof(int32_t) * (nc + 1), stream);
    if (hook_pending) {
      t_scan_emit_hook(t_scan_emit_ctx);
      hook_pending = false;
    }
    if (want_defer) bfs_emit_defer(&def);
    SG_TRY(sg_bfs_cluster_emit(bq_idx, start_len, n_q, n_active, nullptr, cfg->seg_thr + s, nc, sp, cidx, coff, bfs_ws,
                               bfs_bytes, stream_));
    const bool deferred = want_defer && def.deferred;
    hipStream_t tail = deferred ? def.side : stream;
    const int32_t *src_idx = cidx, *src_off = coff;
    if (mapped) {
      SG_TAKE(oidx, int32_t, 2 * static_cast<size_t>(nc_pts));
      SG_TAKE(ooff, int32_t, static_cast<size_t>(nc) + 1);
      const size_t ib = sg_pyramid_inverse_map_workspace_bytes(nc_pts, n_lvl, nc);
      SG_TAKE(i_ws, char, ib);
      SG_TRY(sg_pyramid_inverse_map(cidx, sp, nc, l2p, nc_pts, n_lvl, oidx, ooff, deferred ? meta + 80 : meta + 48, i_ws,
                                    ib, reinterpret_cast<sg_stream_t>(tail)));
      if (!deferred) {
        SG_TRY(read_back(host, meta + 48, 1, stream, kWhat));
        rows = host[0];
      }
      src_idx = oidx;
      src_off = ooff;
    }
    if (deferred) {
      def_rows = rows;
      def_mapped = mapped;
      loop_mark = ar.off;
    }
    if (rows == 0) continue;
    SG_REQUIRE(S + rows <= n_sel, "sg_scan_grouping_pp: more proposal rows than selected points");
    pp_append_kernel<<<grid_for(rows > nc ? rows : nc, 256, 1 << 22), 256, 0, tail>>>(src_idx, rows, src_off, nc, obj + s0,
                                                                                  n_prop, S, pairs, poff);
    n_prop += nc;
    S += rows;
  }
  res->deferred_classes = def_rows >= 0 ? 1 : 0;
  if (def.deferred) {
    SG_TRY(bfs_emit_join(def, stream));
    def.deferred = false;
    if (def_mapped) {
      SG_TRY(read_back(host, meta + 80, 1, stream, kWhat));
      SG_REQUIRE(host[0] == def_rows, "sg_scan_grouping_pp: the deferred class's rows were predicted as %d, the inverse map made %d",
                 def_rows, host[0]);
    }
  }
  ar.off = loop_mark0;
  res->n_neighbours = static_cast<int>(n_nbr < 0x7fffffff ? n_nbr : 0x7fffffff);
  res->n_proposals = n_prop;
  res->sum_npoint = S;
  if (S == 0) return check_launch(kWhat);
  res->proposals_idx = ar.at(pairs);
  res->proposals_offset = ar.at(poff);
  if (cfg->voxel_shape == 0) {
    res->arena_used = ar.off;
    return check_launch(kWhat);
  }
  return voxelise_proposals(cfg, pairs, poff, n_prop, S, coords_float, point_feats, ar, meta, host, res, stream_, kWhat);
}

int sg_scan_instances(const sg_instances_cfg *cfg, const int32_t *proposals_idx, const float *mask_scores,
                      const float *cls_prob, const float *iou_scores, void *arena, size_t arena_bytes,
                      void *host_out, size_t host_bytes, sg_instances_result *res, sg_stream_t stream_) {
  static const char *kWhat = "sg_scan_instances";
  SG_REQUIRE(cfg != nullptr && res != nullptr, "sg_scan_instances: null descriptor");
  SG_REQUIRE(cfg->n_classes >= 1 && cfg->score_stride >= cfg->n_classes && cfg->n_proposals >= 0 &&
                 cfg->sum_npoint >= 0 && cfg->n_points >= 0,
             "sg_scan_instances: bad configuration");
  memset(res, 0, sizeof(*res));
  hipStream_t stream = as_stream(stream_);
  int32_t *host = pinned_words();
  SG_REQUIRE(host != nullptr, "sg_scan_instances: no pinned host words");
  ScanArena ar(arena, arena_bytes);
  const int nP = cfg->n_proposals, nc = cfg->n_classes, stride = cfg->score_stride;
  const int64_t S = cfg->sum_npoint;
  if (nP == 0 || S == 0) return SG_OK;
  SG_TAKE(npoint, int32_t, static_cast<size_t>(nP) * nc);
  SG_TAKE(inst_of, int32_t, static_cast<size_t>(nP) * nc);
  SG_TAKE(kept_cls, int32_t, static_cast<size_t>(nP) * nc);
  SG_TAKE(kept_score, float, static_cast<size_t>(nP) * nc);
  SG_TAKE(head, int32_t, 64);
  SG_TRY(sg_instance_npoint(proposals_idx, mask_scores, S, stride, nc, cfg->mask_score_thr, nP, npoint, stream_));
  instance_keep_kernel<<<1, 1024, 0, stream>>>(cls_prob, iou_scores, stride, npoint, nP, nc, cfg->cls_score_thr,
                                             cfg->min_npoint, inst_of, kept_cls, kept_score, head);
  SG_TRY(check_launch(kWhat));
  SG_TRY(read_back(host, head, 2, stream, kWhat));
  const int n_kept = host[0];
  const int64_t cap = host[1] > 0 ? host[1] : 1;
  res->n_kept = n_kept;
  if (n_kept == 0) return SG_OK;
  SG_TAKE(starts, int32_t, cap);
  SG_TAKE(ends, int32_t, cap);
  SG_TAKE(bounds, int64_t, static_cast<size_t>(n_kept) + 1);
  const size_t rws_bytes = sg_instance_runs_workspace_bytes(n_kept, cfg->n_points);
  SG_TAKE(rws, char, rws_bytes);
  SG_TRY(sg_instance_runs(proposals_idx, mask_scores, S, stride, nc, cfg->mask_score_thr, inst_of, nP, n_kept,
                          cfg->n_points, starts, ends, bounds, cap, rws, rws_bytes, stream_));
  const int64_t tcap = sg_rle_format_device_text_bytes(cap, cfg->n_points);
  SG_TAKE(text, uint8_t, static_cast<size_t>(tcap));
  SG_TAKE(text_off, int64_t, static_cast<size_t>(n_kept) + 1);
  const size_t fws_bytes = sg_rle_format_device_workspace_bytes(cap);
  SG_TAKE(fws, char, fws_bytes);
  SG_TRY(sg_rle_format_device(starts, ends, bounds, n_kept, cap, cfg->n_points, text, tcap, text_off, fws,
                              fws_bytes, stream_));
  const size_t off_cls = sizeof(int64_t) * (static_cast<size_t>(n_kept) + 1);
  const size_t off_score = off_cls + sizeof(int32_t) * static_cast<size_t>(n_kept);
  const size_t off_text = align_up(off_score + sizeof(float) * static_cast<size_t>(n_kept), 8);
  res->host_needed = off_text + static_cast<size_t>(tcap);
  if (host_out == nullptr || host_bytes < off_text + 16) {
    set_error("sg_scan_instances: host buffer too small (%zu bytes, need up to %zu)", host_bytes, res->host_needed);
    return SG_ERR_WORKSPACE;
  }
  char *h = static_cast<char *>(host_out);
  if (hipMemcpyAsync(h, text_off, off_cls, hipMemcpyDeviceToHost, stream) != hipSuccess ||
      hipMemcpyAsync(h + off_cls, kept_cls, sizeof(int32_t) * n_kept, hipMemcpyDeviceToHost, stream) != hipSuccess ||
      hipMemcpyAsync(h + off_score, kept_score, sizeof(float) * n_kept, hipMemcpyDeviceToHost, stream) != hipSuccess ||
      hipStreamSynchronize(stream) != hipSuccess) {
    set_error("sg_scan_instances: result copy failed");
    return SG_ERR_LAUNCH;
  }
  const int64_t text_bytes = reinterpret_cast<const int64_t *>(h)[n_kept];
  res->host_needed = off_text + static_cast<size_t>(text_bytes);
  if (host_bytes < res->host_needed) {
    set_error("sg_scan_instances: host buffer too small (%zu bytes, need %zu)", host_bytes, res->host_needed);
    return SG_ERR_WORKSPACE;
  }
  if (text_bytes > 0 &&
      (hipMemcpyAsync(h + off_text, text, static_cast<size_t>(text_bytes), hipMemcpyDeviceToHost, stream) != hipSuccess ||
       hipStreamSynchronize(stream) != hipSuccess)) {
    set_error("sg_scan_instances: text copy failed");
    return SG_ERR_LAUNCH;
  }
  res->bits = ar.at(rws);
  res->label_id = ar.at(kept_cls);
  res->off_class = off_cls;
  res->off_score = off_score;
  res->off_text = off_text;
  res->text_bytes = static_cast<size_t>(text_bytes);
  res->arena_used = ar.off;
  return SG_OK;
}

}
```

### softgroup_amd/csrc/spconv_rulebook.hip

```cpp
#include <stdlib.h>

#include <mutex>

#include "common.h"
#include "radix_sort.h"
#include "scan.h"

namespace sg {

constexpr uint64_t kKeyEmpty = ~0ULL;

struct HashWs {
  uint64_t *keys;
  int32_t *vals;
  int32_t *owner, *rank;
  void *scan_ws;
  size_t scan_bytes;
  uint32_t cap;
};

static size_t hash_cap(int n) {
  size_t cap = 1024;
  while (cap < static_cast<size_t>(n) * 2) cap <<= 1;
  return cap;
}
static bool hash_carve(void *ws, size_t ws_bytes, int n, HashWs *w) {
  Workspace a(ws, ws_bytes);
  const size_t nn = static_cast<size_t>(n > 0 ? n : 1);
  w->cap = static_cast<uint32_t>(hash_cap(n));
  w->keys = a.take<uint64_t>(w->cap);
  w->vals = a.take<int32_t>(w->cap);
  w->owner = a.take<int32_t>(nn);
  w->rank = a.take<int32_t>(nn);
  w->scan_bytes = scan_workspace_bytes(n);
  w->scan_ws = a.take<char>(w->scan_bytes);
  return w->scan_ws != nullptr;
}

struct Shape3 {
  int s0, s1, s2;
};
__device__ __forceinline__ uint64_t lin_key(int b, int x, int y, int z, Shape3 s) {
  return ((static_cast<uint64_t>(b) * s.s0 + x) * s.s1 + y) * s.s2 + z;
}

__device__ __forceinline__ uint32_t hash_insert_min(uint64_t *keys, int32_t *vals, uint32_t mask,
                                                    uint64_t key, int32_t val) {
  uint32_t s = static_cast<uint32_t>(mix64(key)) & mask;
  while (true) {
    const uint64_t seen = __hip_atomic_load(&keys[s], __ATOMIC_RELAXED, __HIP_MEMORY_SCOPE_AGENT);
    if (seen == key) {
      if (__hip_atomic_load(&vals[s], __ATOMIC_RELAXED, __HIP_MEMORY_SCOPE_AGENT) > val) atomicMin(&vals[s], val);
      return s;
    }
    if (seen == kKeyEmpty) {
      unsigned long long prev = atomicCAS(reinterpret_cast<unsigned long long *>(&keys[s]),
                                          static_cast<unsigned long long>(kKeyEmpty),
// ... 77 lines not shown
                                                       const int32_t *__restrict__ owner,
                                                       int32_t *__restrict__ out_indices,
                                                       int32_t *__restrict__ child) {
  const int i = blockIdx.x * 256 + threadIdx.x;
  if (i >= M) return;
  const int o = in2out[i];
  if (o < 0) return;
  const int4 c = reinterpret_cast<const int4 *>(indices)[i];
  child[o * 8 + (c.y & 1) * 4 + (c.z & 1) * 2 + (c.w & 1)] = i;
  if (owner[i] == i) reinterpret_cast<int4 *>(out_indices)[o] = make_int4(c.x, c.y >> 1, c.z >> 1, c.w >> 1);
}
__global__ void __launch_bounds__(256) inverse_rulebook_kernel(const int32_t *__restrict__ indices,
                                                              const int32_t *__restrict__ in2out,
                                                              int M, int32_t *__restrict__ inv) {
  const int64_t total = static_cast<int64_t>(M) * 8;
  for (int64_t t = blockIdx.x * 256LL + threadIdx.x; t < total; t += gridDim.x * 256LL) {
    const int i = static_cast<int>(t >> 3), k = static_cast<int>(t & 7);
    const int4 c = reinterpret_cast<const int4 *>(indices)[i];
    const int kk = (c.y & 1) * 4 + (c.z & 1) * 2 + (c.w & 1);
    inv[t] = (k == kk) ? in2out[i] : -1;
  }
}


constexpr int kPyrMaxLevels = SG_PYRAMID_MAX_LEVELS;
constexpr int kPyrMaxSegs = 3 * kPyrMaxLevels;
constexpr uint32_t kPlanKeyBits = 27;

__global__ void __launch_bounds__(256) pyr_insert_kernel(const int32_t *__restrict__ indices, int M0,
                                                        Shape3 shape, int L, uint64_t *keys,
                                                        int32_t *vals, uint32_t cap,
                                                        int32_t *__restrict__ slot) {
  const int i = blockIdx.x * 256 + threadIdx.x;
  if (i >= M0) return;
  int4 c = reinterpret_cast<const int4 *>(indices)[i];
  Shape3 s = shape;
  bool alive = true;
  for (int l = 0; l < L; ++l) {
    if (l > 0) {
      const Shape3 os{s.s0 / 2, s.s1 / 2, s.s2 / 2};
      c.y >>= 1; c.z >>= 1; c.w >>= 1;
      alive = alive && c.y < os.s0 && c.z < os.s1 && c.w < os.s2;
      s = os;
    }
    int32_t sl = -1;
    if (alive)
      sl = static_cast<int32_t>(hash_insert_min(keys + static_cast<size_t>(l) * cap,
                                                vals + static_cast<size_t>(l) * cap, cap - 1,
                                                lin_key(c.x, c.y, c.z, c.w, s), i));
    slot[static_cast<size_t>(l) * M0 + i] = sl;
  }
}

__global__ void pyr_rows_kernel(const int32_t *__restrict__ pos, int M0, int L, int32_t *rows) {
  const int l = threadIdx.x;
  if (l < L) rows[l] = pos[static_cast<size_t>(l + 1) * M0] - pos[static_cast<size_t>(l) * M0];
}

struct PyrOut {
  int32_t *indices[kPyrMaxLevels];
  int32_t *nbr[kPyrMaxLevels];
  int32_t *in2out[kPyrMaxLevels];
  int32_t *child[kPyrMaxLevels];
  int32_t *inv[kPyrMaxLevels];
  long long pre27[kPyrMaxLevels + 1];
  Shape3 shape[kPyrMaxLevels];
};

__global__ void __launch_bounds__(256) pyr_emit_kernel(const int32_t *__restrict__ indices0, int M0,
                                                      int L, const int32_t *__restrict__ vals,
                                                      int32_t *__restrict__ rowtab, uint32_t cap,
                                                      const int32_t *__restrict__ slot,
                                                      const int32_t *__restrict__ pos, PyrOut o) {
  const int64_t total = static_cast<int64_t>(L) * M0;
  for (int64_t t = blockIdx.x * 256LL + threadIdx.x; t < total; t += gridDim.x * 256LL) {
    const int l = static_cast<int>(t / M0), i = static_cast<int>(t - static_cast<int64_t>(l) * M0);
    const int sl = slot[t];
    if (sl < 0 || vals[static_cast<size_t>(l) * cap + sl] != i) continue;
    const int r = pos[t] - pos[static_cast<size_t>(l) * M0];
    rowtab[static_cast<size_t>(l) * cap + sl] = r;
    const int4 c = reinterpret_cast<const int4 *>(indices0)[i];
    if (o.indices[l] != nullptr)
      reinterpret_cast<int4 *>(o.indices[l])[r] = make_int4(c.x, c.y >> l, c.z >> l, c.w >> l);
  }
}

__global__ void __launch_bounds__(256) pyr_link_kernel(const int32_t *__restrict__ indices0, int M0,
                                                      int L, const int32_t *__restrict__ vals,
                                                      const int32_t *__restrict__ rowtab,
                                                      uint32_t cap, const int32_t *__restrict__ slot,
                                                      const int32_t *__restrict__ pos, PyrOut o) {
  const int64_t total = static_cast<int64_t>(L - 1) * M0;
  for (int64_t t = blockIdx.x * 256LL + threadIdx.x; t < total; t += gridDim.x * 256LL) {
    const int l = static_cast<int>(t / M0), i = static_cast<int>(t - static_cast<int64_t>(l) * M0);
    const int sl = slot[t];
    if (sl < 0 || vals[static_cast<size_t>(l) * cap + sl] != i) continue;
    const int j = pos[t] - pos[static_cast<size_t>(l) * M0];
    const int s2 = slot[t + M0];
    const int up = s2 >= 0 ? rowtab[static_cast<size_t>(l + 1) * cap + s2] : -1;
    const int4 c = reinterpret_cast<const int4 *>(indices0)[i];
    const int k = (((c.y >> l) & 1) << 2) | (((c.z >> l) & 1) << 1) | ((c.w >> l) & 1);
    o.in2out[l][j] = up;
    if (up >= 0) o.child[l][static_cast<int64_t>(up) * 8 + k] = j;
    int4 *dst = reinterpret_cast<int4 *>(o.inv[l] + static_cast<int64_t>(j) * 8);
    dst[0] = make_int4(k == 0 ? up : -1, k == 1 ? up : -1, k == 2 ? up : -1, k == 3 ? up : -1);
    dst[1] = make_int4(k == 4 ? up : -1, k == 5 ? up : -1, k == 6 ? up : -1, k == 7 ? up : -1);
  }
}

// ... 316 lines not shown
      if (P.s[i].K <= 8) big[nb++] = P.s[i];
    for (int i = 0; i < nb; ++i) {
      big[i].key_bits = i < P.n_wide ? static_cast<int>(kPlanKeyBits) : 8;
      big[i].seg_code = i < P.n_wide ? i : i - P.n_wide;
    }
  } else {
    for (int i = 0; i < P.n; ++i) small[ns++] = P.s[i];
  }
  int row_base = 0, tile_base = 0, sb_base = 0;
  P.n_big = nb;
  for (int i = 0; i < P.n; ++i) {
    PlanSeg &S = P.s[i];
    S = i < nb ? big[i] : small[i - nb];
    S.row_base = row_base;
    S.tile_base = tile_base;
    S.sb_base = sb_base;
    S.sb_rows = mode == 0 ? (S.rows + 31) / 32 * 32 : plan_sb_rows(S.rows);
    row_base += S.rows;
    tile_base += (S.rows + 31) / 32;
    if (i >= nb) sb_base += (S.rows + S.sb_rows - 1) / S.sb_rows;
    if (i + 1 == nb) P.big_rows = row_base;
    if (i + 1 == P.n_wide) P.wide_rows = row_base;
  }
  if (nb == 0) P.big_rows = 0;
  P.total_rows = row_base;
  P.total_tiles = tile_base;
  P.total_sbs = sb_base;
}

static int build_plans(const PlanSegs &P, void *ws2, size_t ws2_bytes, bool zero_freq, hipStream_t stream,
                       const char *who) {
  Workspace wsp(ws2, ws2_bytes);
  const size_t R = static_cast<size_t>(P.total_rows);
  uint32_t *mask = wsp.take<uint32_t>(R);
  int32_t *val = wsp.take<int32_t>(R);
  uint32_t *tmask = wsp.take<uint32_t>(P.total_tiles);
  int32_t *torder = wsp.take<int32_t>(P.total_tiles);
  int32_t *freq = wsp.take<int32_t>(kPyrMaxSegs * 32);
  int32_t *bitpos = wsp.take<int32_t>(kPyrMaxSegs * 32);
  const size_t rs_bytes = radix_sort_workspace_bytes(static_cast<int64_t>(R));
  void *rs_ws = wsp.take<char>(rs_bytes);
  if (!rs_ws) {
    set_error("%s: build workspace too small", who);
    return SG_ERR_WORKSPACE;
  }
  if (zero_freq) hipMemsetAsync(freq, 0, kPyrMaxSegs * 32 * 4, stream);
  int max_rows = 0, max_big = 0;
  for (int i = 0; i < P.n; ++i) {
    max_rows = P.s[i].rows > max_rows ? P.s[i].rows : max_rows;
    if (i < P.n_big) max_big = P.s[i].rows > max_big ? P.s[i].rows : max_big;
  }
  const dim3 grid((max_rows + 255) / 256, P.n);
  plan_mask_all_kernel<<<grid, 256, 0, stream>>>(P, mask, val, freq);
  static const bool raw_env = getenv("SG_PLAN_RAW") != nullptr;
  if (raw_env) hipMemsetAsync(freq, 0, kPyrMaxSegs * 32 * 4, stream);
  plan_pos_all_kernel<<<P.n, 32, 0, stream>>>(P, freq, bitpos);
  const int mode = plan_order_mode();
  PlanSegs Q = P;
  if (P.n_big > 0) {
    const dim3 gbig((max_big + 255) / 256, P.n_big);
    plan_key_all_kernel<<<gbig, 256, 0, stream>>>(P, bitpos, mask);
    struct Group { int first, count, row0, rows, key_bits; } groups[2] = {
        {0, P.n_wide, 0, P.wide_rows, static_cast<int>(kPlanKeyBits)},
        {P.n_wide, P.n_big - P.n_wide, P.wide_rows, P.big_rows - P.wide_rows, 8}};
    for (const Group &g : groups) {
      if (g.count == 0 || g.rows == 0) continue;
      int nbits = g.key_bits;
      for (int n = g.count - 1; n > 0; n >>= 1) ++nbits;
      uint32_t *ms;
      int32_t *vs;
      int rc = radix_sort_pairs(mask + g.row0, val + g.row0, static_cast<int64_t>(g.rows), nbits, rs_ws, rs_bytes,
                                stream, &ms, &vs);
      if (rc != SG_OK) return rc;
      if (ms != mask + g.row0) {
        hipMemcpyAsync(mask + g.row0, ms, static_cast<size_t>(g.rows) * 4, hipMemcpyDeviceToDevice, stream);
        hipMemcpyAsync(val + g.row0, vs, static_cast<size_t>(g.rows) * 4, hipMemcpyDeviceToDevice, stream);
      }
      for (int i = g.first; i < g.first + g.count; ++i) {
        Q.s[i].key_sorted = mask;
        Q.s[i].val_sorted = val;
      }
    }
    plan_tiles_all_kernel<<<gbig, 256, 0, stream>>>(Q, bitpos, tmask);
  }
  if (P.total_sbs > 0) {
    int max_sb = 64;
    for (int i = P.n_big; i < P.n; ++i)
      while (max_sb < P.s[i].sb_rows && max_sb < P.s[i].rows) max_sb <<= 1;
    static std::once_flag once;
    std::call_once(once, [] {
      hipFuncSetAttribute(reinterpret_cast<const void *>(plan_sort_sb_kernel), hipFuncAttributeMaxDynamicSharedMemorySize,
                          kSbRowsMax * 8);
    });
    plan_sort_sb_kernel<<<P.total_sbs, 1024, static_cast<size_t>(max_sb) * 8, stream>>>(Q, mask, bitpos, val, tmask);
  }
  if (mode == 0) plan_tile_order_all_kernel<<<P.n, 1024, 0, stream>>>(Q, tmask, torder);
  else plan_tile_order_xcd_kernel<<<dim3(P.n, 8), 1024, 0, stream>>>(Q, tmask, mode, torder);
  plan_emit_all_kernel<<<dim3(min((max_rows + 31) / 32, 2048), P.n), 256, 0, stream>>>(Q, val, tmask, torder);
  return check_launch(who);
}

struct PyrWs {
  uint64_t *keys;
  int32_t *vals;
  int32_t *rowtab;
  int32_t *slot;
  int32_t *pos;
  void *scan_ws;
  size_t scan_bytes;
  uint32_t cap;
};
static bool pyr_carve(void *ws, size_t ws_bytes, int M0, int L, PyrWs *w) {
  Workspace a(ws, ws_bytes);
  const size_t nn = static_cast<size_t>(M0 > 0 ? M0 : 1);
  w->cap = static_cast<uint32_t>(hash_cap(M0));
  w->keys = a.take<uint64_t>(static_cast<size_t>(L) * w->cap);
  w->vals = a.take<int32_t>(static_cast<size_t>(L) * w->cap);
  w->rowtab = a.take<int32_t>(static_cast<size_t>(L) * w->cap);
  w->slot = a.take<int32_t>(static_cast<size_t>(L) * nn);
  w->pos = a.take<int32_t>(static_cast<size_t>(L) * nn + 1);
  w->scan_bytes = scan_workspace_bytes(static_cast<int64_t>(L) * nn);
  w->scan_ws = a.take<char>(w->scan_bytes);
  return w->scan_ws != nullptr;
}

}

using namespace sg;

extern "C" {

size_t sg_spconv_hash_workspace_bytes(int M) {
  const size_t nn = static_cast<size_t>(M > 0 ? M : 1);
  return align_up(hash_cap(M) * 8) + align_up(hash_cap(M) * 4) + 3 * align_up(nn * 4) +
         align_up(scan_workspace_bytes(M)) + 256;
}

static int build_hash_common(HashWs *w, void *ws, size_t ws_bytes, int M, hipStream_t stream,
                             const char *who) {
  if (!hash_carve(ws, ws_bytes, M, w)) {
    set_error("%s: workspace too small", who);
    return SG_ERR_WORKSPACE;
  }
  hipMemsetAsync(w->keys, 0xff, static_cast<size_t>(w->cap) * 8, stream);
  hipMemsetAsync(w->vals, 0x7f, static_cast<size_t>(w->cap) * 4, stream);
  return SG_OK;
}

int sg_spconv_subm_rulebook(const int32_t *indices, int M, const int32_t *shape_host, int32_t *nbr,
                            void *ws, size_t ws_bytes, sg_stream_t stream_) {
  SG_REQUIRE(M >= 0 && shape_host, "sg_spconv_subm_rulebook: bad arguments");
// ... 22 lines not shown
  const Shape3 oshape{shape_host[0] / 2, shape_host[1] / 2, shape_host[2] / 2};
  const int grid = (M + 255) / 256;
  int32_t *slot_of = w.rank;
  down_insert_kernel<<<grid, 256, 0, stream>>>(indices, M, oshape, w.keys, w.vals, w.cap - 1,
                                               slot_of);
  down_owner_kernel<<<grid, 256, 0, stream>>>(w.vals, slot_of, M, w.owner);
  const int32_t *owner = w.owner;
  int32_t *rank = w.rank;
  rc = exclusive_scan(
      [owner] __device__(int64_t i) { return owner[i] == static_cast<int32_t>(i) ? 1 : 0; },
      [rank] __device__(int64_t i, int v) { rank[i] = v; }, M, meta, w.scan_ws, w.scan_bytes,
      stream);
  if (rc != SG_OK) return rc;
  down_map_kernel<<<grid, 256, 0, stream>>>(w.owner, w.rank, M, in2out);
  return check_launch("sg_spconv_down_build");
}

int sg_spconv_down_fill(const int32_t *indices, int M, const int32_t *in2out, int M_out,
                        int32_t *out_indices, int32_t *child, void *ws, size_t ws_bytes,
                        sg_stream_t stream_) {
  SG_REQUIRE(M >= 0 && M_out >= 0, "sg_spconv_down_fill: bad arguments");
  if (M == 0 || M_out == 0) return SG_OK;
  hipStream_t stream = as_stream(stream_);
  HashWs w;
  if (!hash_carve(ws, ws_bytes, M, &w)) {
    set_error("sg_spconv_down_fill: workspace too small");
    return SG_ERR_WORKSPACE;
  }
  hipMemsetAsync(child, 0xff, static_cast<size_t>(M_out) * 8 * 4, stream);
  down_fill_kernel<<<(M + 255) / 256, 256, 0, stream>>>(indices, M, in2out, w.owner, out_indices,
                                                       child);
  return check_launch("sg_spconv_down_fill");
}

int sg_spconv_inverse_rulebook(const int32_t *indices_fine, const int32_t *in2out, int M,
                               int32_t *inv_nbr, sg_stream_t stream) {
  SG_REQUIRE(M >= 0, "sg_spconv_inverse_rulebook: bad arguments");
  if (M == 0) return SG_OK;
  inverse_rulebook_kernel<<<grid_for(static_cast<int64_t>(M) * 8, 256, 256 * 32), 256, 0,
                            as_stream(stream)>>>(indices_fine, in2out, M, inv_nbr);
  return check_launch("sg_spconv_inverse_rulebook");
}


size_t sg_spconv_pyramid_workspace_bytes(int M0, int n_levels) {
  const size_t nn = static_cast<size_t>(M0 > 0 ? M0 : 1), L = static_cast<size_t>(n_levels > 0 ? n_levels : 1);
  const size_t cap = hash_cap(M0);
  return align_up(L * cap * 8) + 2 * align_up(L * cap * 4) + align_up(L * nn * 4) +
         align_up((L * nn + 1) * 4) + align_up(scan_workspace_bytes(static_cast<int64_t>(L * nn))) + 256;
}

int sg_spconv_pyramid_rows(const int32_t *indices, int M0, const int32_t *shape_host, int n_levels,
                           int32_t *rows_dev, void *ws, size_t ws_bytes, sg_stream_t stream_) {
  SG_REQUIRE(M0 >= 0 && shape_host && rows_dev && n_levels >= 1 && n_levels <= kPyrMaxLevels,
             "sg_spconv_pyramid_rows: bad arguments (M0=%d n_levels=%d)", M0, n_levels);
  hipStream_t stream = as_stream(stream_);
  if (M0 == 0) {
    hipMemsetAsync(rows_dev, 0, static_cast<size_t>(n_levels) * 4, stream);
    return check_launch("sg_spconv_pyramid_rows");
  }
  PyrWs w;
  if (!pyr_carve(ws, ws_bytes, M0, n_levels, &w)) {
    set_error("sg_spconv_pyramid_rows: workspace too small (%zu bytes)", ws_bytes);
    return SG_ERR_WORKSPACE;
  }
  const int L = n_levels;
  {
    FillList f;
    f.add(w.keys, static_cast<size_t>(L) * w.cap * 8, 0xff);
    f.add(w.vals, static_cast<size_t>(L) * w.cap * 4, 0x7f);
    fill_many(f, stream);
  }
  const Shape3 shape{shape_host[0], shape_host[1], shape_host[2]};
  pyr_insert_kernel<<<(M0 + 255) / 256, 256, 0, stream>>>(indices, M0, shape, L, w.keys, w.vals, w.cap,
                                                         w.slot);
  const int32_t *slot = w.slot, *vals = w.vals;
  int32_t *pos = w.pos;
  const int m0 = M0;
  const uint32_t cap = w.cap;
  const int64_t n = static_cast<int64_t>(L) * M0;
  int rc = exclusive_scan(
      [slot, vals, m0, cap] __device__(int64_t t) {
        const int64_t l = t / m0;
        const int sl = slot[t];
        return (sl >= 0 && vals[l * cap + sl] == static_cast<int32_t>(t - l * m0)) ? 1 : 0;
      },
      [pos] __device__(int64_t t, int v) { pos[t] = v; }, n, pos + n, w.scan_ws, w.scan_bytes, stream);
  if (rc != SG_OK) return rc;
  pyr_rows_kernel<<<1, 64, 0, stream>>>(w.pos, M0, L, rows_dev);
  return check_launch("sg_spconv_pyramid_rows");
}

static long long pyr_seg_rows(const sg_pyramid_level *lv, int L, int seg_kind, int l) {
  return seg_kind == 1 ? lv[l + 1].rows : lv[l].rows;
}

size_t sg_spconv_pyramid_build_workspace_bytes(const sg_pyramid_level *levels, int n_levels) {
  long long total = 0;
  for (int l = 0; l < n_levels; ++l) {
    total += levels[l].rows;
    if (l + 1 < n_levels) total += levels[l + 1].rows + levels[l].rows;
  }
  const size_t R = static_cast<size_t>(total > 0 ? total : 1);
  const size_t T = R / 32 + static_cast<size_t>(3 * n_levels) + 1;
  return plan_scratch_bytes(R, T);
}

int sg_spconv_pyramid_build(const int32_t *indices, int M0, const int32_t *shape_host, int n_levels,
                            const sg_pyramid_level *levels, void *ws, size_t ws_bytes, void *ws2,
                            size_t ws2_bytes, sg_stream_t stream_) {
  SG_REQUIRE(M0 >= 0 && shape_host && levels && n_levels >= 1 && n_levels <= kPyrMaxLevels,
             "sg_spconv_pyramid_build: bad arguments (M0=%d n_levels=%d)", M0, n_levels);
  SG_REQUIRE(levels[0].rows == M0, "sg_spconv_pyramid_build: levels[0].rows must be num_rows");
  if (M0 == 0) return SG_OK;
  hipStream_t stream = as_stream(stream_);
  const int L = n_levels;
  PyrWs w;
  if (!pyr_carve(ws, ws_bytes, M0, L, &w)) {
    set_error("sg_spconv_pyramid_build: workspace too small (%zu bytes)", ws_bytes);
    return SG_ERR_WORKSPACE;
  }
  SG_REQUIRE(ws2 != nullptr && ws2_bytes >= sg_spconv_pyramid_build_workspace_bytes(levels, L),
             "sg_spconv_pyramid_build: build workspace too small (%zu bytes)", ws2_bytes);
  PyrOut o;
  PlanSegs P;
  P.n = 0;
  auto add_seg = [&](const int32_t *nbr, int rows, int K, const sg_plan_ptrs &pl) {
    PlanSeg &S = P.s[P.n++];
    S.nbr = nbr; S.order = pl.order; S.tile_mask = pl.tile_mask; S.nbr_tiles = pl.nbr_tiles;
    S.rows = rows; S.K = K;
  };
  Shape3 s{shape_host[0], shape_host[1], shape_host[2]};
  o.pre27[0] = 0;
  for (int l = 0; l < kPyrMaxLevels; ++l) {
    const bool in = l < L;
    o.indices[l] = in ? levels[l].indices : nullptr;
    o.nbr[l] = in ? levels[l].nbr : nullptr;
    o.in2out[l] = in ? levels[l].in2out : nullptr;
    o.child[l] = in ? levels[l].child : nullptr;
    o.inv[l] = in ? levels[l].inv : nullptr;
    o.shape[l] = s;
    o.pre27[l + 1] = o.pre27[l] + (in ? static_cast<long long>(levels[l].rows) * 27 : 0);
    s = Shape3{s.s0 / 2, s.s1 / 2, s.s2 / 2};
  }
  for (int l = 0; l < L; ++l) {
    SG_REQUIRE(levels[l].rows >= 0 && levels[l].nbr && levels[l].indices && levels[l].subm.order,
               "sg_spconv_pyramid_build: level %d: missing output pointers", l);
    if (l + 1 < L)
      SG_REQUIRE(levels[l].in2out && levels[l].child && levels[l].inv && levels[l].down.order &&
                     levels[l].up.order, "sg_spconv_pyramid_build: level %d: missing output pointers", l);
  }
  for (int l = 0; l < L; ++l) {
    if (levels[l].rows > 0) add_seg(levels[l].nbr, levels[l].rows, 27, levels[l].subm);
    if (l + 1 < L) {
      if (levels[l + 1].rows > 0) add_seg(levels[l].child, levels[l + 1].rows, 8, levels[l].down);
      if (levels[l].rows > 0) add_seg(levels[l].inv, levels[l].rows, 8, levels[l].up);
    }
  }
  if (P.n == 0) return check_launch("sg_spconv_pyramid_build");
  finalize_segs(P);
  int32_t *freq;
  {
    Workspace wsp(ws2, ws2_bytes);
    const size_t R = static_cast<size_t>(P.total_rows);
    wsp.take<uint32_t>(R);
    wsp.take<int32_t>(R);
    wsp.take<uint32_t>(P.total_tiles);
    wsp.take<int32_t>(P.total_tiles);
    freq = wsp.take<int32_t>(kPyrMaxSegs * 32);
    if (!freq) {
      set_error("sg_spconv_pyramid_build: build workspace too small");
      return SG_ERR_WORKSPACE;
    }
  }
  {
    static_assert(kPyrMaxLevels + 1 <= kFillMax, "one fill region per level + the histogram");
    FillList f;
    for (int l = 0; l + 1 < L; ++l)
      if (levels[l + 1].rows > 0) f.add(levels[l].child, static_cast<size_t>(levels[l + 1].rows) * 8 * 4, 0xff);
    f.add(freq, kPyrMaxSegs * 32 * 4, 0);
    fill_many(f, stream);
  }
  const int g_all = grid_for(static_cast<int64_t>(L) * M0, 256, 4096);
  pyr_emit_kernel<<<g_all, 256, 0, stream>>>(indices, M0, L, w.vals, w.rowtab, w.cap, w.slot, w.pos, o);
  if (L > 1) {
    pyr_link_kernel<<<grid_for(static_cast<int64_t>(L - 1) * M0, 256, 4096), 256, 0, stream>>>(
        indices, M0, L, w.vals, w.rowtab, w.cap, w.slot, w.pos, o);
  }
  pyr_subm_kernel<<<grid_for(o.pre27[L], 256, 8192), 256, 0, stream>>>(L, w.keys, w.rowtab, w.cap, o);
  return build_plans(P, ws2, ws2_bytes, false, stream, "sg_spconv_pyramid_build");
}

size_t sg_spconv_plan_workspace_bytes(int M) {
  const size_t nn = static_cast<size_t>(M > 0 ? M : 1);
  return plan_scratch_bytes(nn, (nn + 31) / 32 + 1);
}

int sg_spconv_plan(const int32_t *nbr, int M, int K, int32_t *order, uint32_t *tile_mask,
                   int32_t *nbr_tiles, void *ws, size_t ws_bytes, sg_stream_t stream_) {
  SG_REQUIRE(M >= 0 && K >= 1 && K <= 27, "sg_spconv_plan: bad arguments (M=%d K=%d)", M, K);
  if (M == 0) return SG_OK;
  PlanSegs P;
  P.n = 1;
  P.s[0] = PlanSeg{nbr, order, tile_mask, nbr_tiles, M, K, 0, 0, 0, 0, 0, 0, nullptr, nullptr};
  finalize_segs(P);
  return build_plans(P, ws, ws_bytes, true, as_stream(stream_), "sg_spconv_plan");
}

}
```

### softgroup_amd/csrc/unet_exec.hip

```cpp
#include <map>
#include <mutex>
#include <utility>
#include <vector>

#include <stdlib.h>

#include "common.h"
#include "radix_sort.h"
#include "unet_common.h"

namespace sg {

__global__ void __launch_bounds__(256) batch_max_kernel(const int32_t *__restrict__ indices, int M,
                                                       int32_t *__restrict__ bmax) {
  int m = 0;
  for (int i = blockIdx.x * 256 + threadIdx.x; i < M; i += gridDim.x * 256) m = max(m, indices[4 * i]);
#pragma unroll
  for (int o = 32; o > 0; o >>= 1) m = max(m, __shfl_xor(m, o, 64));
  if ((threadIdx.x & 63) == 0 && m > 0) atomicMax(bmax, m);
}
__device__ __forceinline__ uint64_t spread3(uint32_t v) {
  uint64_t x = v & 0x1fffffu;
  x = (x | (x << 32)) & 0x1f00000000ffffull;
  x = (x | (x << 16)) & 0x1f0000ff0000ffull;
  x = (x | (x << 8)) & 0x100f00f00f00f00full;
  x = (x | (x << 4)) & 0x10c30c30c30c30c3ull;
  x = (x | (x << 2)) & 0x1249249249249249ull;
  return x;
}
__global__ void __launch_bounds__(256) morton_key_kernel(const int32_t *__restrict__ indices, int M,
                                                        int dim_bits, const int32_t *__restrict__ bmax,
                                                        uint32_t *__restrict__ key, int32_t *__restrict__ val) {
  const int i = blockIdx.x * 256 + threadIdx.x;
  if (i >= M) return;
  const int4 c = reinterpret_cast<const int4 *>(indices)[i];
  const int bb = 32 - __clz(*bmax);
  const uint64_t code = (static_cast<uint64_t>(static_cast<uint32_t>(c.x)) << (3 * dim_bits)) |
                        (spread3(c.y) << 2) | (spread3(c.z) << 1) | spread3(c.w);
  const int total = bb + 3 * dim_bits;
  key[i] = static_cast<uint32_t>(total > 24 ? code >> (total - 24) : code);
  val[i] = i;
}
__global__ void __launch_bounds__(256) permute_indices_kernel(const int32_t *__restrict__ indices,
                                                             const int32_t *__restrict__ perm, int M,
                                                             int32_t *__restrict__ out) {
  const int i = blockIdx.x * 256 + threadIdx.x;
  if (i < M) reinterpret_cast<int4 *>(out)[i] = reinterpret_cast<const int4 *>(indices)[perm[i]];
}
template <bool SCATTER>
__global__ void __launch_bounds__(256) permute_rows_kernel(const float4 *__restrict__ in,
                                                          const int32_t *__restrict__ perm, int64_t rows,
                                                          int c4, float4 *__restrict__ out) {
  const int64_t total = rows * c4;
  for (int64_t t = blockIdx.x * 256LL + threadIdx.x; t < total; t += gridDim.x * 256LL) {
    const int64_t r = t / c4;
    const int c = static_cast<int>(t - r * c4);
    const int64_t o = perm[r];
    if (SCATTER) out[o * c4 + c] = in[t];
    else out[t] = in[o * c4 + c];
  }
// ... 94 lines not shown
      }
      hipEventDestroy(st->ev_start);
      hipEventDestroy(st->ev_index);
      hipHostFree(st->host_rows);
      hipFree(st->dev_rows);
    }
  }
  delete st;
}

int unet_build_index(const char *who, int L, const int32_t *indices, int num_rows,
                     const int32_t *spatial_shape_host, void *arena, size_t arena_bytes, sg_stream_t stream,
                     LevelIdx *li, size_t *used, std::unique_lock<std::mutex> *lock) {
  int dev = 0;
  SG_REQUIRE(hipGetDevice(&dev) == hipSuccess && dev >= 0, "%s: no current device", who);
  StreamState *stp = nullptr;
  {
    std::lock_guard<std::mutex> g(table_mu);
    StreamState *&slot = table[std::make_pair(dev, as_stream(stream))];
    if (slot == nullptr) slot = new StreamState();
    stp = slot;
  }
  StreamState &st = *stp;
  std::unique_lock<std::mutex> guard(st.mu);
  if (!st.ready) {
    SG_REQUIRE(hipHostMalloc(reinterpret_cast<void **>(&st.host_rows), SG_PYRAMID_MAX_LEVELS * 4) == hipSuccess,
               "%s: pinned allocation failed", who);
    SG_REQUIRE(hipMalloc(reinterpret_cast<void **>(&st.dev_rows), SG_PYRAMID_MAX_LEVELS * 4) == hipSuccess,
               "%s: device allocation failed", who);
    SG_REQUIRE(!index_stream_on() || hipStreamCreateWithFlags(&st.istream, hipStreamNonBlocking) == hipSuccess,
               "%s: stream creation failed", who);
    SG_REQUIRE(hipEventCreateWithFlags(&st.ev_start, hipEventDisableTiming) == hipSuccess &&
                   hipEventCreateWithFlags(&st.ev_index, hipEventDisableTiming) == hipSuccess,
               "%s: event creation failed", who);
    st.ready = true;
  }
  const bool own_istream = index_stream_on();
  hipStream_t istream = own_istream ? st.istream : as_stream(stream);
  sg_stream_t is = reinterpret_cast<sg_stream_t>(istream);
  if (own_istream && (hipEventRecord(st.ev_start, as_stream(stream)) != hipSuccess ||
                      hipStreamWaitEvent(istream, st.ev_start, 0) != hipSuccess)) {
    set_error("%s: event record/wait failed", who);
    return SG_ERR_LAUNCH;
  }
  Arena ix(arena, arena_bytes);
#define SG_IALLOC(var, T, count)                                                       \
  T *var = ix.take<T>(count);                                                          \
  if (var == nullptr) {                                                                \
    set_error("%s: arena too small (%zu bytes) for the index tables", who, arena_bytes); \
    return SG_ERR_WORKSPACE;                                                           \
  }
  const size_t pws_bytes = sg_spconv_pyramid_workspace_bytes(num_rows, L);
  SG_IALLOC(pws, char, pws_bytes);
  SG_TRY(sg_spconv_pyramid_rows(indices, num_rows, spatial_shape_host, L, st.dev_rows, pws, pws_bytes, is));
  if (hipMemcpyAsync(st.host_rows, st.dev_rows, sizeof(int32_t) * L, hipMemcpyDeviceToHost, istream) != hipSuccess ||
      hipStreamSynchronize(istream) != hipSuccess) {
    set_error("%s: reading the level row counts failed", who);
    return SG_ERR_LAUNCH;
  }
  SG_REQUIRE(st.host_rows[0] == num_rows, "%s: duplicate voxel coordinates in the input "
             "(%d distinct of %d rows)", who, st.host_rows[0], num_rows);
  sg_pyramid_level pl[SG_PYRAMID_MAX_LEVELS];
  for (int l = 0; l < L; ++l) {
    const int rows = st.host_rows[l];
    const int rows2 = l + 1 < L ? st.host_rows[l + 1] : 0;
    const size_t r = static_cast<size_t>(rows ? rows : 1), r2 = static_cast<size_t>(rows2 ? rows2 : 1);
    const size_t t = (r + 31) / 32, t2 = (r2 + 31) / 32;
    sg_pyramid_level &P = pl[l];
    P = sg_pyramid_level();
    P.rows = rows;
    SG_IALLOC(indices_l, int32_t, r * 4);
    SG_IALLOC(nbr, int32_t, r * 27);
    SG_IALLOC(so, int32_t, t * 32);
    SG_IALLOC(sm, uint32_t, t + SG_PLAN_HIST_WORDS);
    SG_IALLOC(sn, int32_t, t * 32 * 27);
    P.indices = indices_l; P.nbr = nbr;
    P.subm = sg_plan_ptrs{so, sm, sn};
    LevelIdx &I = li[l];
    I.rows = rows;
    for (int a = 0; a < 3; ++a) I.shape[a] = spatial_shape_host[a] >> l;
    I.subm.nbr = nbr; I.subm.order = so; I.subm.tile_mask = sm; I.subm.nbr_tiles = sn;
    I.subm.rows = rows; I.subm.kvol = 27;
    if (l + 1 < L) {
      SG_IALLOC(in2out, int32_t, r);
      SG_IALLOC(child, int32_t, r2 * 8);
      SG_IALLOC(inv, int32_t, r * 8);
      SG_IALLOC(dord, int32_t, t2 * 32);
      SG_IALLOC(dm, uint32_t, t2 + SG_PLAN_HIST_WORDS);
      SG_IALLOC(dn, int32_t, t2 * 32 * 8);
      SG_IALLOC(uo, int32_t, t * 32);
      SG_IALLOC(um, uint32_t, t + SG_PLAN_HIST_WORDS);
      SG_IALLOC(un, int32_t, t * 32 * 8);
      P.in2out = in2out; P.child = child; P.inv = inv;
      P.down = sg_plan_ptrs{dord, dm, dn};
      P.up = sg_plan_ptrs{uo, um, un};
      I.down.nbr = child; I.down.order = dord; I.down.tile_mask = dm; I.down.nbr_tiles = dn;
      I.down.rows = rows2; I.down.kvol = 8;
      I.up.nbr = inv; I.up.order = uo; I.up.tile_mask = um; I.up.nbr_tiles = un;
      I.up.rows = rows; I.up.kvol = 8;
    }
  }
  {
    const size_t nb = sg_spconv_pyramid_build_workspace_bytes(pl, L);
    SG_IALLOC(ws2, char, nb);
    SG_TRY(sg_spconv_pyramid_build(indices, num_rows, spatial_shape_host, L, pl, pws, pws_bytes, ws2, nb, is));
  }
  if (L > 1) {
    IdentSegs segs;
    segs.n = L - 1;
    for (int l = 0; l + 1 < L; ++l) {
      const size_t tiles = (static_cast<size_t>(li[l].rows) + 31) / 32;
      SG_IALLOC(ord, int32_t, tiles ? tiles * 32 : 32);
      SG_IALLOC(tm, uint32_t, tiles + SG_PLAN_HIST_WORDS);
      segs.order[l] = ord;
      segs.mask[l] = tm;
      segs.rows[l] = li[l].rows;
      Plan &P = li[l].ident;
      P.nbr = ord; P.order = ord; P.nbr_tiles = ord; P.tile_mask = tm;
      P.rows = li[l].rows; P.kvol = 1;
    }
    ident_plan_kernel<<<dim3(grid_for(num_rows, 256), L - 1), 256, 0, istream>>>(segs);
  }
#undef SG_IALLOC
  if (own_istream && (hipEventRecord(st.ev_index, istream) != hipSuccess ||
                      hipStreamWaitEvent(as_stream(stream), st.ev_index, 0) != hipSuccess)) {
    set_error("%s: event record/wait failed", who);
    return SG_ERR_LAUNCH;
  }
  *used = ix.off;
  *lock = std::move(guard);
  return SG_OK;
}

__global__ void __launch_bounds__(256) pad_channels_kernel(const float *__restrict__ in, int64_t rows, int cin,
                                                          int cpad, const int32_t *__restrict__ perm,
                                                          float *__restrict__ out) {
  const int64_t total = rows * cpad;
  for (int64_t t = blockIdx.x * 256LL + threadIdx.x; t < total; t += gridDim.x * 256LL) {
    const int64_t r = t / cpad;
    const int c = static_cast<int>(t - r * cpad);
    const int64_t src = perm ? perm[r] : r;
    out[t] = c < cin ? in[src * cin + c] : 0.f;
  }
}

#define SG_ALLOC(var, T, count)                                                        \
  T *var = ar.take<T>(count);                                                          \
  if (var == nullptr) {                                                                \
    set_error("sg_unet_forward: arena too small (%zu bytes, need more than %zu)", ar.cap, ar.off); \
    return SG_ERR_WORKSPACE;                                                           \
  }

thread_local void (*t_unet_conv_hook)(void *) = nullptr;
thread_local void *t_unet_conv_ctx = nullptr;

struct Exec {
  const sg_unet_desc *d;
  Arena ar;
  sg_stream_t stream;
  const LevelIdx *idx;
  const int32_t *perm = nullptr;

  Exec(const sg_unet_desc *desc, void *arena, size_t bytes, sg_stream_t s, const LevelIdx *li)
      : d(desc), ar(arena, bytes), stream(s), idx(li) {}

  bool r16 = false;
  size_t fsz(size_t n) const { return r16 ? (n + 1) / 2 : n; }
  bool chain_open = false;
  bool chain_from(int l) const {
    static const int max_rows = getenv("SG_CONV_CHAIN_ROWS") ? atoi(getenv("SG_CONV_CHAIN_ROWS")) : 6144;
    if (r16 || chain_open || idx[l].rows > max_rows || idx[l].rows <= 0) return false;
    for (int k = l; k < d->n_levels; ++k)
      if (d->levels[k].planes % 32 != 0) return false;
    return true;
  }
  struct ChainScope {
    Exec &e;
    bool on;
    ChainScope(Exec &ex, bool open) : e(ex), on(open) {
      if (on) {
        conv_chain_begin(as_stream(e.stream));
        e.chain_open = true;
      }
// ... 311 lines not shown
```

### softgroup_amd/csrc/voxelize_idx.hip

```cpp
#include "common.h"
#include "scan.h"

namespace sg {

constexpr int32_t kEmpty = 0x7f7f7f7f;

struct VKey {
  int32_t b, x, y, z;
};
__device__ __forceinline__ VKey load_vkey(const int64_t *__restrict__ coords, int i, int ncol) {
  const int64_t *r = coords + static_cast<int64_t>(i) * ncol;
  VKey k;
  if (ncol == 3) { k.b = 0; k.x = static_cast<int32_t>(r[0]); k.y = static_cast<int32_t>(r[1]); k.z = static_cast<int32_t>(r[2]); }
  else { k.b = static_cast<int32_t>(r[0]); k.x = static_cast<int32_t>(r[1]); k.y = static_cast<int32_t>(r[2]); k.z = static_cast<int32_t>(r[3]); }
  return k;
}
__device__ __forceinline__ bool same(const VKey &a, const VKey &b) {
  return a.b == b.b && a.x == b.x && a.y == b.y && a.z == b.z;
}
__device__ __forceinline__ uint32_t vkey_slot(const VKey &k, uint32_t cap_mask) {
  uint64_t h = (static_cast<uint64_t>(static_cast<uint32_t>(k.b)) << 32) | static_cast<uint32_t>(k.x);
  h = mix64(h) ^ ((static_cast<uint64_t>(static_cast<uint32_t>(k.y)) << 32) | static_cast<uint32_t>(k.z));
  return static_cast<uint32_t>(mix64(h)) & cap_mask;
}
// ... 89 lines not shown

struct VoxWs {
  int32_t *table, *slot_of, *owner, *rank, *count, *last, *csr_off, *cursor, *seg;
  void *scan_ws;
  size_t scan_bytes;
  uint32_t cap;
};

static size_t vox_cap(int n) {
  size_t cap = 1024;
  while (cap < static_cast<size_t>(n) * 2) cap <<= 1;
  return cap;
}

static bool vox_carve(void *ws, size_t ws_bytes, int n, VoxWs *w) {
  Workspace a(ws, ws_bytes);
  const size_t nn = static_cast<size_t>(n > 0 ? n : 1);
  w->cap = static_cast<uint32_t>(vox_cap(n));
  w->table = a.take<int32_t>(w->cap);
  w->slot_of = a.take<int32_t>(nn);
  w->owner = a.take<int32_t>(nn);
  w->rank = a.take<int32_t>(nn);
  w->count = a.take<int32_t>(nn);
  w->last = a.take<int32_t>(nn);
  w->csr_off = a.take<int32_t>(nn);
  w->cursor = a.take<int32_t>(nn);
  w->seg = a.take<int32_t>(nn);
  w->scan_bytes = scan_workspace_bytes(n);
  w->scan_ws = a.take<char>(w->scan_bytes);
  return w->scan_ws != nullptr;
}

}

using namespace sg;

extern "C" {

size_t sg_voxelize_idx_workspace_bytes(int n) {
  const size_t nn = static_cast<size_t>(n > 0 ? n : 1);
  return align_up(vox_cap(n) * 4) + 8 * align_up(nn * 4) + align_up(scan_workspace_bytes(n)) + 256;
}

int sg_voxelize_idx_build(const int64_t *coords, int n, int ncol, int mode, int32_t *input_map,
                          int32_t *meta, void *ws, size_t ws_bytes, sg_stream_t stream_) {
  SG_REQUIRE(n >= 0 && (ncol == 3 || ncol == 4) && mode >= 0 && mode <= 4,
             "sg_voxelize_idx_build: bad arguments (n=%d ncol=%d mode=%d)", n, ncol, mode);
  hipStream_t stream = as_stream(stream_);
  VoxWs w;
  if (!vox_carve(ws, ws_bytes, n, &w)) {
    set_error("sg_voxelize_idx_build: workspace too small");
    return SG_ERR_WORKSPACE;
  }
  const int32_t init_meta[2] = {0, 1};
  hipMemcpyAsync(meta, init_meta, sizeof(init_meta), hipMemcpyHostToDevice, stream);
  if (n == 0) return SG_OK;
  const int grid = (n + 255) / 256;
  {
    FillList f;
    f.add(w.table, static_cast<size_t>(w.cap) * 4, 0x7f);
    f.add(w.count, static_cast<size_t>(n) * 4, 0);
    f.add(w.last, static_cast<size_t>(n) * 4, 0);
    fill_many(f, stream);
  }
  vox_insert_kernel<<<grid, 256, 0, stream>>>(coords, n, ncol, w.table, w.cap - 1, w.slot_of);
  vox_owner_kernel<<<grid, 256, 0, stream>>>(w.table, w.slot_of, n, w.owner);
  const int32_t *owner = w.owner;
  int32_t *rank = w.rank;
  auto in = [owner] __device__(int64_t i) { return owner[i] == static_cast<int32_t>(i) ? 1 : 0; };
  auto out = [rank] __device__(int64_t i, int v) { rank[i] = v; };
  int rc = exclusive_scan(in, out, n, meta, w.scan_ws, w.scan_bytes, stream);
  if (rc != SG_OK) return rc;
  vox_map_kernel<<<grid, 256, 0, stream>>>(w.owner, w.rank, n, (mode == 3 || mode == 4) ? 1 : 0,
                                           input_map, w.count, w.last, meta);
  return check_launch("sg_voxelize_idx_build");
}

int sg_voxelize_idx_fill(const int64_t *coords, int n, int ncol, int mode, const int32_t *input_map,
                         int num_voxels, int max_active, int64_t *out_coords, int32_t *out_map,
                         void *ws, size_t ws_bytes, sg_stream_t stream_) {
  SG_REQUIRE(n >= 0 && num_voxels >= 0 && num_voxels <= n && max_active >= 1,
             "sg_voxelize_idx_fill: bad arguments");
  hipStream_t stream = as_stream(stream_);
  VoxWs w;
  if (!vox_carve(ws, ws_bytes, n, &w)) {
    set_error("sg_voxelize_idx_fill: workspace too small");
    return SG_ERR_WORKSPACE;
  }
  if (n == 0 || num_voxels == 0) return SG_OK;
  {
    FillList f;
    f.add(out_map, static_cast<size_t>(num_voxels) * (max_active + 1) * 4, 0);
    f.add(w.cursor, static_cast<size_t>(num_voxels) * 4, 0);
    fill_many(f, stream);
  }
  const int32_t *count = w.count;
  int32_t *csr = w.csr_off;
  auto in = [count] __device__(int64_t v) { return count[v]; };
  auto out = [csr] __device__(int64_t v, int x) { csr[v] = x; };
  int rc = exclusive_scan(in, out, num_voxels, nullptr, w.scan_ws, w.scan_bytes, stream);
  if (rc != SG_OK) return rc;
  const int grid = (n + 255) / 256;
  vox_scatter_kernel<<<grid, 256, 0, stream>>>(input_map, w.csr_off, n, w.cursor, w.seg);
  vox_fill_kernel<<<grid, 256, 0, stream>>>(coords, n, ncol, mode, input_map, w.csr_off, w.count,
                                            w.last, w.seg, max_active, out_coords, out_map);
  return check_launch("sg_voxelize_idx_fill");
}

}
```

Baseline: 417.4.

## Read back small device counters through a mapped-memory mailbox instead of memcpy+sync

After: 409.3. 0.981x the previous value.

```diff
diff --git a/include/softgroup_hip.h b/include/softgroup_hip.h
--- a/include/softgroup_hip.h
+++ b/include/softgroup_hip.h
@@ -30,6 +30,10 @@
 int sg_stream_create(sg_stream_t *stream_out);
 int sg_stream_destroy(sg_stream_t stream);
 int sg_stream_create_priority(sg_stream_t *stream_out, int level);
+
+int sg_mailbox_enable(int on);
+int sg_mailbox_selftest(int words, int count, int set_seq, uint32_t seq, int silent, int32_t *out_host, int *path_out,
+                        sg_stream_t stream);
 
 int sg_voxelize_idx_host(const int64_t *coords_host, int n, int ncol, int mode,
                          int32_t *input_map_host, int32_t *num_voxels_host,
diff --git a/softgroup_amd/_lib.py b/softgroup_amd/_lib.py
--- a/softgroup_amd/_lib.py
+++ b/softgroup_amd/_lib.py
@@ -14,6 +14,8 @@
     'sg_last_error': (C.c_char_p, []),
     'sg_device_info': (_i, [C.c_char_p, _i, C.POINTER(_i), C.POINTER(_i)]),
     'sg_stream_release': (_i, [_vp]),
+    'sg_mailbox_enable': (_i, [_i]),
+    'sg_mailbox_selftest': (_i, [_i, _i, _i, C.c_uint32, _i, _vp, C.POINTER(_i), _vp]),
     'sg_host_copy_2d': (_i, [_vp, _i64, _vp, _i64, _i64, _i64]),
     'sg_host_cast_f64_f32': (_i, [_vp, _vp, _i64]),
     'sg_host_fill_i64_strided': (_i, [_vp, _i64, _i64, _i64]),
diff --git a/softgroup_amd/csrc/bfs.hip b/softgroup_amd/csrc/bfs.hip
--- a/softgroup_amd/csrc/bfs.hip
+++ b/softgroup_amd/csrc/bfs.hip
@@ -5,6 +5,7 @@
 #include <utility>
 
 #include "common.h"
+#include "mailbox.h"
 #include "scan.h"
 
 namespace sg {
@@ -108,8 +109,9 @@
 }
 
 __global__ void __launch_bounds__(256) bfs_init_kernel(int n, int32_t *parent, int32_t *size,
-                                                      int32_t *owner) {
+                                                      int32_t *owner, int32_t *counters) {
   const int i = blockIdx.x * 256 + threadIdx.x;
+  if (i < 64) counters[i] = 0;
   if (i < n) {
     parent[i] = i;
     size[i] = 0;
@@ -1620,7 +1622,7 @@
     set_error("bfs_count_kept_members: workspace too small");
     return SG_ERR_WORKSPACE;
   }
-  hipMemsetAsync(out, 0, 4, stream);
+  fill_one(out, 4, 0, stream);
   bfs_kept_members_kernel<<<grid_for(n_pts, 256, 1024), 256, 0, stream>>>(l2p, n_pts, w.label, w.size, thr_dev, out);
   return check_launch("bfs_count_kept_members");
 }
@@ -1654,8 +1656,7 @@
   *sum_npoint_host = 0;
   if (n == 0) return SG_OK;
   const int grid = (n + 255) / 256;
-  hipMemsetAsync(w.counters, 0, 64 * 4, stream);
-  bfs_init_kernel<<<grid, 256, 0, stream>>>(n, w.parent, w.size, w.owner);
+  bfs_init_kernel<<<grid, 256, 0, stream>>>(n, w.parent, w.size, w.owner, w.counters);
   static const bool one_pass = getenv("SG_BFS_ONE_PASS") != nullptr;
   if (!one_pass) {
     static const bool sample_env = getenv("SG_BFS_SAMPLE") != nullptr;
@@ -1714,10 +1715,12 @@
     rc = exclusive_scan(keep_size, [coff] __device__(int64_t i, int v) { coff[i] = v; }, n,
                         w.counters + 3, w.scan_ws, w.scan_bytes, stream);
     if (rc != SG_OK) return rc;
-    hipMemcpyAsync(host_counters, w.counters, 5 * sizeof(int32_t), hipMemcpyDeviceToHost, stream);
-    if (hipStreamSynchronize(stream) != hipSuccess) return check_launch("sg_bfs_cluster_label");
+    if (const int rc2 = mailbox_fetch(mailbox_for(stream), w.counters, 5, nullptr, 0, host_counters, stream,
+                                      "sg_bfs_cluster_label");
+        rc2 != SG_OK)
+      return rc2;
     if (host_counters[0] == 0) break;
-    if (pass == 0) hipMemsetAsync(w.counters + 4, 0, 4, stream);
+    if (pass == 0) fill_one(w.counters + 4, 4, 0, stream);
   }
   *n_cluster_host = host_counters[2];
   *sum_npoint_host = host_counters[3];
@@ -1738,7 +1741,7 @@
     return SG_ERR_WORKSPACE;
   }
   if (n_cluster == 0 || n == 0) {
-    hipMemsetAsync(cluster_offsets, 0, 4, stream);
+    fill_one(cluster_offsets, 4, 0, stream);
     return SG_OK;
   }
   bfs_seed_kernel<<<(n + 255) / 256, 256, 0, stream>>>(n, w.label, w.size, w.cid, w.coff,
diff --git a/softgroup_amd/csrc/common.h b/softgroup_amd/csrc/common.h
--- a/softgroup_amd/csrc/common.h
+++ b/softgroup_amd/csrc/common.h
@@ -11,6 +11,9 @@
 
 void set_error(const char *fmt, ...);
 int32_t *pinned_words();
+
+void host_mark(const char *label);
+void host_mark_flush(const char *who);
 
 inline hipStream_t as_stream(sg_stream_t s) { return reinterpret_cast<hipStream_t>(s); }
 
@@ -104,6 +107,13 @@
     pattern[n] = 0x01010101u * static_cast<uint32_t>(byte & 0xff);
     ++n;
   }
+  void add_words(void *ptr, size_t count, uint32_t word) {
+    if (count == 0 || ptr == nullptr || n >= kFillMax) return;
+    p[n] = static_cast<uint32_t *>(ptr);
+    words[n] = count;
+    pattern[n] = word;
+    ++n;
+  }
 };
 static __global__ void __launch_bounds__(256) fill_many_kernel(FillList f) {
   const int r = blockIdx.y;
@@ -128,6 +138,11 @@
   for (int i = 0; i < f.n; ++i) mx = f.words[i] > mx ? f.words[i] : mx;
   const int gx = grid_for(static_cast<int64_t>(mx / 4 + 1), 256, 1024);
   fill_many_kernel<<<dim3(gx, f.n), 256, 0, stream>>>(f);
+}
+inline void fill_one(void *ptr, size_t bytes, int byte, hipStream_t stream) {
+  FillList f;
+  f.add(ptr, bytes, byte);
+  fill_many(f, stream);
 }
 
 extern thread_local int t_conv_arith;
diff --git a/softgroup_amd/csrc/core.hip b/softgroup_amd/csrc/core.hip
--- a/softgroup_amd/csrc/core.hip
+++ b/softgroup_amd/csrc/core.hip
@@ -1,7 +1,16 @@
 #include <stdarg.h>
+#include <stdlib.h>
 #include <string.h>
 
+#include <atomic>
+#include <chrono>
+#include <map>
+#include <mutex>
+#include <thread>
+#include <tuple>
+
 #include "common.h"
+#include "mailbox.h"
 #include "scan.h"
 
 namespace sg {
@@ -21,9 +30,194 @@
   va_end(ap);
 }
 
+static bool host_trace_on() {
+  static const bool on = getenv("SG_HOST_TRACE") && atoi(getenv("SG_HOST_TRACE")) != 0;
+  return on;
+}
+struct HostMarks {
+  const char *label[64];
+  int64_t ns[64];
+  int n = 0;
+};
+static thread_local HostMarks t_marks;
+void host_mark(const char *label) {
+  if (!host_trace_on() || t_marks.n >= 64) return;
+  t_marks.label[t_marks.n] = label;
+  t_marks.ns[t_marks.n++] =
+      std::chrono::duration_cast<std::chrono::nanoseconds>(std::chrono::steady_clock::now().time_since_epoch()).count();
+}
+void host_mark_flush(const char *who) {
+  if (!host_trace_on()) return;
+  fprintf(stderr, "[host trace] %s:", who);
+  for (int i = 1; i < t_marks.n; ++i) fprintf(stderr, " %s %.1f", t_marks.label[i], (t_marks.ns[i] - t_marks.ns[i - 1]) * 1e-3);
+  fprintf(stderr, "\n");
+  t_marks.n = 0;
+}
+
+static std::atomic<int> g_mail_override{-1};
+bool mailbox_enabled() {
+  static const bool env_on = !(getenv("SG_MAILBOX") && atoi(getenv("SG_MAILBOX")) == 0);
+  const int o = g_mail_override.load(std::memory_order_relaxed);
+  return o < 0 ? env_on : o != 0;
+}
+
+struct MailKey {
+  int dev;
+  hipStream_t stream;
+  std::thread::id tid;
+  bool operator<(const MailKey &o) const { return std::tie(dev, stream, tid) < std::tie(o.dev, o.stream, o.tid); }
+};
+static std::mutex g_mail_mu;
+static std::map<MailKey, Mailbox *> g_mail;
+static std::atomic<uint64_t> g_mail_gen{1};
+
+static Mailbox *mailbox_make(hipStream_t stream) {
+  Mailbox *mb = new Mailbox();
+  void *h = nullptr, *d = nullptr;
+  if (hipHostMalloc(&h, 512, hipHostMallocMapped | hipHostMallocCoherent) != hipSuccess ||
+      hipHostGetDevicePointer(&d, h, 0) != hipSuccess || d == nullptr ||
+      hipEventCreateWithFlags(&mb->ev, hipEventDisableTiming) != hipSuccess) {
+    (void)hipGetLastError();
+    if (h != nullptr) hipHostFree(h);
+    delete mb;
+    return nullptr;
+  }
+  memset(h, 0, 512);
+  mb->host = static_cast<int32_t *>(h);
+  mb->dev = static_cast<int32_t *>(d);
+  mb->stream = stream;
+  return mb;
+}
+
+Mailbox *mailbox_for(hipStream_t stream) {
+  if (!mailbox_enabled()) return nullptr;
+  struct Cache {
+    uint64_t gen = 0;
+    int dev = -1;
+    hipStream_t stream = nullptr;
+    Mailbox *mb = nullptr;
+  };
+  static thread_local Cache c;
+  int dev = 0;
+  if (hipGetDevice(&dev) != hipSuccess) return nullptr;
+  const uint64_t gen = g_mail_gen.load(std::memory_order_acquire);
+  if (c.gen == gen && c.dev == dev && c.stream == stream) return c.mb;
+  std::lock_guard<std::mutex> g(g_mail_mu);
+  const MailKey key{dev, stream, std::this_thread::get_id()};
+  auto it = g_mail.find(key);
+  if (it == g_mail.end()) it = g_mail.emplace(key, mailbox_make(stream)).first;
+  c.gen = g_mail_gen.load(std::memory_order_acquire);
+  c.dev = dev;
+  c.stream = stream;
+  c.mb = it->second;
+  return c.mb;
+}
+
+void mailbox_release_stream(int dev, hipStream_t stream) {
+  std::lock_guard<std::mutex> g(g_mail_mu);
+  for (auto it = g_mail.begin(); it != g_mail.end();) {
+    if (it->first.dev == dev && it->first.stream == stream) {
+      if (Mailbox *mb = it->second) {
+        hipEventDestroy(mb->ev);
+        hipHostFree(mb->host);
+        delete mb;
+      }
+      it = g_mail.erase(it);
+    } else {
+      ++it;
+    }
+  }
+  g_mail_gen.fetch_add(1, std::memory_order_release);
+}
+
+static inline void cpu_pause() {
+#if defined(__x86_64__) || defined(__i386__)
+  __builtin_ia32_pause();
+#elif defined(__aarch64__)
+  __asm__ __volatile__("yield");
+#endif
+}
+
+static int mail_copy_path(int32_t *out, const int32_t *dev_a, int words_a, const int32_t *dev_b, int words_b,
+                          hipStream_t stream, const char *what) {
+  if ((words_a > 0 && hipMemcpyAsync(out, dev_a, sizeof(int32_t) * words_a, hipMemcpyDeviceToHost, stream) != hipSuccess) ||
+      (words_b > 0 &&
+       hipMemcpyAsync(out + words_a, dev_b, sizeof(int32_t) * words_b, hipMemcpyDeviceToHost, stream) != hipSuccess) ||
+      hipStreamSynchronize(stream) != hipSuccess) {
+    (void)hipGetLastError();
+    set_error("%s: device -> host read-back failed", what);
+    return SG_ERR_LAUNCH;
+  }
+  return SG_OK;
+}
+
+int mailbox_wait(Mailbox *mb, const MailPost &p, const int32_t *dev_src, int words, int32_t *out, const char *what) {
+  const uint32_t *stamp = reinterpret_cast<const uint32_t *>(mb->host + kMailStampAt);
+  auto arrived = [&] { return __atomic_load_n(stamp, __ATOMIC_ACQUIRE) == p.stamp; };
+  auto take = [&] {
+    for (int i = 0; i < words; ++i) out[i] = __atomic_load_n(mb->host + i, __ATOMIC_RELAXED);
+    return SG_OK;
+  };
+  mb->last_path = 0;
+  if (hipEventRecord(mb->ev, mb->stream) != hipSuccess) {
+    (void)hipGetLastError();
+    set_error("%s: recording the event behind the size's producer failed", what);
+    return SG_ERR_LAUNCH;
+  }
+  constexpr int kSpinsPerQuery = 256;
+  for (;;) {
+    for (int i = 0; i < kSpinsPerQuery; ++i) {
+      if (arrived()) return take();
+      cpu_pause();
+    }
+    const hipError_t q = hipEventQuery(mb->ev);
+    if (q == hipErrorNotReady) continue;
+    if (q != hipSuccess) {
+      (void)hipGetLastError();
+      set_error("%s: device -> host read-back failed (%s)", what, hipGetErrorString(q));
+      return SG_ERR_LAUNCH;
+    }
+    break;
+  }
+  if (arrived()) return take();
+  mb->last_path = 1;
+  if (hipStreamSynchronize(mb->stream) != hipSuccess) {
+    (void)hipGetLastError();
+    set_error("%s: device -> host read-back failed", what);
+    return SG_ERR_LAUNCH;
+  }
+  if (arrived()) return take();
+  mb->last_path = 2;
+  if (dev_src == nullptr) {
+    set_error("%s: the size's producer completed without posting it", what);
+    return SG_ERR_LAUNCH;
+  }
+  return mail_copy_path(out, dev_src, words, nullptr, 0, mb->stream, what);
+}
+
+__global__ void __launch_bounds__(64) mail_publish_kernel(const int32_t *__restrict__ a, int na,
+                                                          const int32_t *__restrict__ b, int nb, MailPost p) {
+  const int i = threadIdx.x;
+  if (i < na) mail_store(p, i, a[i]);
+  else if (i < na + nb) mail_store(p, i, b[i - na]);
+  mail_stamp(p, i == 0);
+}
+
+int mailbox_fetch(Mailbox *mb, const int32_t *dev_a, int words_a, const int32_t *dev_b, int words_b, int32_t *out,
+                  hipStream_t stream, const char *what) {
+  if (words_a + words_b > kMailWords) mb = nullptr;
+  if (mb == nullptr) return mail_copy_path(out, dev_a, words_a, dev_b, words_b, stream, what);
+  const MailPost p = mailbox_next(mb);
+  mail_publish_kernel<<<1, 64, 0, stream>>>(dev_a, words_a, dev_b, words_b, p);
+  if (words_b == 0) return mailbox_wait(mb, p, dev_a, words_a, out, what);
+  const int rc = mailbox_wait(mb, p, nullptr, words_a + words_b, out, what);
+  if (rc != SG_OK && mb->last_path == 2) return mail_copy_path(out, dev_a, words_a, dev_b, words_b, stream, what);
+  return rc;
+}
+
 __global__ void __launch_bounds__(kScanBlock) scan_block_sums_kernel(int32_t *block_sums,
                                                                     int num_blocks,
-                                                                    int32_t *total_out) {
+                                                                    int32_t *total_out, MailPost post) {
   __shared__ int lds4[4];
   int carry = 0;
   for (int base = 0; base < num_blocks; base += kScanBlock) {
@@ -34,12 +228,50 @@
     if (idx < num_blocks) block_sums[idx] = carry + incl - v;
     carry += tot;
   }
-  if (threadIdx.x == 0 && total_out) *total_out = carry;
+  if (threadIdx.x == 0) {
+    if (total_out) *total_out = carry;
+    if (post.words != nullptr) {
+      mail_store(post, 0, carry);
+      mail_stamp(post, true);
+    }
+  }
 }
 
 void launch_scan_block_sums(int32_t *block_sums, int num_blocks, int32_t *total_out,
-                            hipStream_t stream) {
-  scan_block_sums_kernel<<<1, kScanBlock, 0, stream>>>(block_sums, num_blocks, total_out);
+                            hipStream_t stream, MailPost post) {
+  scan_block_sums_kernel<<<1, kScanBlock, 0, stream>>>(block_sums, num_blocks, total_out, post);
+}
+
+__global__ void __launch_bounds__(64) scan_empty_total_kernel(int32_t *total_out, MailPost post) {
+  if (threadIdx.x != 0) return;
+  if (total_out) *total_out = 0;
+  if (post.words != nullptr) {
+    mail_store(post, 0, 0);
+    mail_stamp(post, true);
+  }
+}
+void launch_scan_empty_total(int32_t *total_out, hipStream_t stream, MailPost post) {
+  scan_empty_total_kernel<<<1, 64, 0, stream>>>(total_out, post);
+}
+
+__global__ void __launch_bounds__(64) mail_test_fill_kernel(uint32_t k, int words, int32_t *dev_words, MailPost p) {
+  const int i = threadIdx.x;
+  const int32_t v = static_cast<int32_t>(k * 1000003u + static_cast<uint32_t>(i) * 7919u);
+  if (i < words) {
+    dev_words[i] = v;
+    if (p.words != nullptr) mail_store(p, i, v);
+  }
+  if (p.words != nullptr) mail_stamp(p, i == 0);
+}
+__global__ void mail_test_empty_kernel() {}
+
+
+int exclusive_scan_startlen_post(int32_t *start_len, int n, int32_t *meta, void *ws, size_t ws_bytes, sg_stream_t stream,
+                                 MailPost post) {
+  SG_REQUIRE(n >= 0, "sg_exclusive_scan_startlen: n < 0");
+  auto in = [start_len] __device__(int64_t i) { return start_len[2 * i + 1]; };
+  auto out = [start_len] __device__(int64_t i, int v) { start_len[2 * i] = v; };
+  return exclusive_scan(in, out, n, meta, ws, ws_bytes, as_stream(stream), post);
 }
 
 }
@@ -76,7 +308,49 @@
   sg::unet_release_stream(dev, sg::as_stream(stream));
   sg::scan_release_stream(dev, sg::as_stream(stream));
   sg::bfs_release_stream(dev, sg::as_stream(stream));
-  return SG_OK;
+  sg::mailbox_release_stream(dev, sg::as_stream(stream));
+  return SG_OK;
+}
+
+int sg_mailbox_enable(int on) {
+  const int was = sg::mailbox_enabled() ? 1 : 0;
+  sg::g_mail_override.store(on < 0 ? -1 : (on != 0), std::memory_order_relaxed);
+  return was;
+}
+
+int sg_mailbox_selftest(int words, int count, int set_seq, uint32_t seq, int silent, int32_t *out_host, int *path_out,
+                        sg_stream_t stream_) {
+  SG_REQUIRE(words >= 1 && words <= sg::kMailWords && count >= 0 && out_host != nullptr,
+             "sg_mailbox_selftest: 1..%d words", sg::kMailWords);
+  hipStream_t stream = sg::as_stream(stream_);
+  sg::Mailbox *mb = sg::mailbox_for(stream);
+  SG_REQUIRE(mb != nullptr, "sg_mailbox_selftest: no mailbox (switched off, or the mapped allocation was refused)");
+  if (set_seq) {
+    mb->seq = seq;
+    __atomic_store_n(reinterpret_cast<uint32_t *>(mb->host + sg::kMailStampAt), seq, __ATOMIC_RELEASE);
+  }
+  int32_t *dev_words = nullptr;
+  if (hipMalloc(reinterpret_cast<void **>(&dev_words), sg::kMailWords * 4) != hipSuccess) {
+    sg::set_error("sg_mailbox_selftest: device allocation failed");
+    return SG_ERR_LAUNCH;
+  }
+  int rc = SG_OK, worst = 0;
+  for (int k = 0; k < count && rc == SG_OK; ++k) {
+    const sg::MailPost p = sg::mailbox_next(mb);
+    if (silent) {
+      sg::mail_test_fill_kernel<<<1, 64, 0, stream>>>(static_cast<uint32_t>(k), words, dev_words, sg::MailPost());
+      sg::mail_test_empty_kernel<<<1, 1, 0, stream>>>();
+    } else {
+      sg::mail_test_fill_kernel<<<1, 64, 0, stream>>>(static_cast<uint32_t>(k), words, dev_words, p);
+    }
+    rc = sg::check_launch("sg_mailbox_selftest");
+    if (rc == SG_OK) rc = sg::mailbox_wait(mb, p, dev_words, words, out_host + static_cast<size_t>(k) * words, "sg_mailbox_selftest");
+    worst = mb->last_path > worst ? mb->last_path : worst;
+  }
+  hipStreamSynchronize(stream);
+  hipFree(dev_words);
+  if (path_out) *path_out = worst;
+  return rc;
 }
 
 int sg_stream_create(sg_stream_t *stream_out) {
@@ -127,10 +401,7 @@
 
 int sg_exclusive_scan_startlen(int32_t *start_len, int n, int32_t *meta, void *ws, size_t ws_bytes,
                                sg_stream_t stream) {
-  SG_REQUIRE(n >= 0, "sg_exclusive_scan_startlen: n < 0");
-  auto in = [start_len] __device__(int64_t i) { return start_len[2 * i + 1]; };
-  auto out = [start_len] __device__(int64_t i, int v) { start_len[2 * i] = v; };
-  return sg::exclusive_scan(in, out, n, meta, ws, ws_bytes, sg::as_stream(stream));
-}
-
-}
+  return sg::exclusive_scan_startlen_post(start_len, n, meta, ws, ws_bytes, stream, sg::MailPost());
+}
+
+}
diff --git a/softgroup_amd/csrc/instances.hip b/softgroup_amd/csrc/instances.hip
--- a/softgroup_amd/csrc/instances.hip
+++ b/softgroup_amd/csrc/instances.hip
@@ -442,7 +442,7 @@
   SG_REQUIRE(S >= 0 && stride >= n_classes && n_classes >= 1 && n_prop >= 0,
              "sg_instance_npoint: bad arguments");
   hipStream_t stream = as_stream(stream_);
-  hipMemsetAsync(npoint, 0, static_cast<size_t>(n_prop) * n_classes * 4, stream);
+  fill_one(npoint, static_cast<size_t>(n_prop) * n_classes * 4, 0, stream);
   if (S == 0 || n_prop == 0) return check_launch("sg_instance_npoint");
   const int grid = grid_for((S + 63) / 64, 4, 1024);
   instance_npoint_kernel<<<grid, 256, 0, stream>>>(proposals_idx, mask_scores, S, stride, mask_thr,
@@ -478,7 +478,7 @@
   const size_t sbytes = scan_workspace_bytes(tw);
   void *sws = a.take<char>(sbytes);
   int32_t *total = a.take<int32_t>(64);
-  hipMemsetAsync(bits, 0, static_cast<size_t>(tw) * 4, stream);
+  fill_one(bits, static_cast<size_t>(tw) * 4, 0, stream);
   if (S > 0 && n_prop > 0) {
     const int grid = grid_for(S, 256, 4096);
     instance_bitmap_kernel<<<grid, 256, 0, stream>>>(proposals_idx, mask_scores, S, stride, mask_thr,
diff --git a/softgroup_amd/csrc/mailbox.h b/softgroup_amd/csrc/mailbox.h
--- /dev/null
+++ b/softgroup_amd/csrc/mailbox.h
@@ -0,0 +1,56 @@
+#pragma once
+#include "common.h"
+
+namespace sg {
+
+constexpr int kMailWords = 64;
+constexpr int kMailStampAt = kMailWords;
+
+struct MailPost {
+  int32_t *words = nullptr;
+  uint32_t stamp = 0;
+};
+
+struct Mailbox {
+  int32_t *host = nullptr;
+  int32_t *dev = nullptr;
+  hipEvent_t ev = nullptr;
+  hipStream_t stream = nullptr;
+  uint32_t seq = 0;
+  int last_path = 0;
+};
+
+Mailbox *mailbox_for(hipStream_t stream);
+void mailbox_release_stream(int dev, hipStream_t stream);
+bool mailbox_enabled();
+
+inline MailPost mailbox_next(Mailbox *mb) {
+  MailPost p;
+  if (mb != nullptr) {
+    p.words = mb->dev;
+    p.stamp = ++mb->seq;
+  }
+  return p;
+}
+
+int mailbox_wait(Mailbox *mb, const MailPost &p, const int32_t *dev_src, int words, int32_t *out, const char *what);
+
+int mailbox_fetch(Mailbox *mb, const int32_t *dev_a, int words_a, const int32_t *dev_b, int words_b, int32_t *out,
+                  hipStream_t stream, const char *what);
+
+__device__ __forceinline__ void mail_store(const MailPost &p, int i, int32_t v) {
+  __hip_atomic_store(p.words + i, v, __ATOMIC_RELAXED, __HIP_MEMORY_SCOPE_SYSTEM);
+}
+__device__ __forceinline__ void mail_stamp(const MailPost &p, bool leader) {
+  __builtin_amdgcn_fence(__ATOMIC_RELEASE, "");
+  if (leader)
+    __hip_atomic_store(reinterpret_cast<uint32_t *>(p.words + kMailStampAt), p.stamp, __ATOMIC_RELAXED,
+                       __HIP_MEMORY_SCOPE_SYSTEM);
+}
+
+int spconv_pyramid_rows_post(const int32_t *indices, int M0, const int32_t *shape_host, int n_levels, int32_t *rows_dev,
+                             void *ws, size_t ws_bytes, sg_stream_t stream, MailPost post);
+int exclusive_scan_startlen_post(int32_t *start_len, int n, int32_t *meta, void *ws, size_t ws_bytes, sg_stream_t stream,
+                                 MailPost post);
+
+}
diff --git a/softgroup_amd/csrc/radix_sort.h b/softgroup_amd/csrc/radix_sort.h
--- a/softgroup_amd/csrc/radix_sort.h
+++ b/softgroup_amd/csrc/radix_sort.h
@@ -179,7 +179,7 @@
   const int n_pass = (num_bits + 7) / 8;
   const bool local_scan = nblk <= 256 && n_pass <= 4;
   int32_t *totals = static_cast<int32_t *>(sws);
-  if (local_scan) hipMemsetAsync(totals, 0, static_cast<size_t>(n_pass) * kRsBuckets * 4, stream);
+  if (local_scan) fill_one(totals, static_cast<size_t>(n_pass) * kRsBuckets * 4, 0, stream);
   for (int shift = 0, pass = 0; shift < num_bits; shift += 8, ++pass) {
     if (local_scan) {
       int32_t *t = totals + pass * kRsBuckets;
diff --git a/softgroup_amd/csrc/scan.h b/softgroup_amd/csrc/scan.h
--- a/softgroup_amd/csrc/scan.h
+++ b/softgroup_amd/csrc/scan.h
@@ -1,5 +1,6 @@
 #pragma once
 #include "common.h"
+#include "mailbox.h"
 
 namespace sg {
 
@@ -43,13 +44,15 @@
 }
 
 void launch_scan_block_sums(int32_t *block_sums, int num_blocks, int32_t *total_out,
-                            hipStream_t stream);
+                            hipStream_t stream, MailPost post = MailPost());
+void launch_scan_empty_total(int32_t *total_out, hipStream_t stream, MailPost post);
 
 constexpr int kScanRawBlocks = 2048;
 template <typename In, typename Out, bool RAW = false>
 __global__ void __launch_bounds__(kScanBlock) scan_apply_kernel(In in, Out out, int64_t n,
                                                                const int32_t *block_sums,
-                                                               int32_t *total_out = nullptr) {
+                                                               int32_t *total_out = nullptr,
+                                                               MailPost post = MailPost()) {
   __shared__ int lds4[4];
   __shared__ int carry_s;
   int carry_in = 0;
@@ -62,8 +65,14 @@
     if (threadIdx.x == 0) carry_s = lds4[0] + lds4[1] + lds4[2] + lds4[3];
     __syncthreads();
     carry_in = carry_s;
-    if (total_out != nullptr && blockIdx.x == gridDim.x - 1 && threadIdx.x == 0)
-      *total_out = carry_in + block_sums[blockIdx.x];
+    if (blockIdx.x == gridDim.x - 1 && threadIdx.x == 0) {
+      const int total = carry_in + block_sums[blockIdx.x];
+      if (total_out != nullptr) *total_out = total;
+      if (post.words != nullptr) {
+        mail_store(post, 0, total);
+        mail_stamp(post, true);
+      }
+    }
   }
   const int64_t base = static_cast<int64_t>(blockIdx.x) * kScanTile;
   const int64_t first = base + static_cast<int64_t>(threadIdx.x) * kScanItems;
@@ -87,7 +96,7 @@
 
 template <typename In, typename Out>
 int exclusive_scan(In in, Out out, int64_t n, int32_t *total_out, void *ws, size_t ws_bytes,
-                   hipStream_t stream) {
+                   hipStream_t stream, MailPost post = MailPost()) {
   if (ws_bytes < scan_workspace_bytes(n)) {
     set_error("exclusive_scan: workspace too small (%zu < %zu)", ws_bytes, scan_workspace_bytes(n));
     return SG_ERR_WORKSPACE;
@@ -95,14 +104,14 @@
   int32_t *block_sums = static_cast<int32_t *>(ws);
   int num_blocks = static_cast<int>((n + kScanTile - 1) / kScanTile);
   if (num_blocks == 0) {
-    if (total_out) hipMemsetAsync(total_out, 0, sizeof(int32_t), stream);
+    if (total_out || post.words) launch_scan_empty_total(total_out, stream, post);
     return SG_OK;
   }
   scan_reduce_kernel<<<num_blocks, kScanBlock, 0, stream>>>(in, n, block_sums);
   if (num_blocks <= kScanRawBlocks) {
-    scan_apply_kernel<In, Out, true><<<num_blocks, kScanBlock, 0, stream>>>(in, out, n, block_sums, total_out);
+    scan_apply_kernel<In, Out, true><<<num_blocks, kScanBlock, 0, stream>>>(in, out, n, block_sums, total_out, post);
   } else {
-    launch_scan_block_sums(block_sums, num_blocks, total_out, stream);
+    launch_scan_block_sums(block_sums, num_blocks, total_out, stream, post);
     scan_apply_kernel<In, Out, false><<<num_blocks, kScanBlock, 0, stream>>>(in, out, n, block_sums);
   }
   return check_launch("exclusive_scan");
diff --git a/softgroup_amd/csrc/scan_exec.hip b/softgroup_amd/csrc/scan_exec.hip
--- a/softgroup_amd/csrc/scan_exec.hip
+++ b/softgroup_amd/csrc/scan_exec.hip
@@ -2,6 +2,7 @@
 #include <string.h>
 
 #include "common.h"
+#include "mailbox.h"
 #include "scan.h"
 
 namespace sg {
@@ -30,7 +31,7 @@
 __global__ void __launch_bounds__(1024) select_scan_kernel(const int32_t *__restrict__ blk_cnt, int n_seg,
                                                           int n_blocks, int min_npoint,
                                                           int32_t *__restrict__ blk_off,
-                                                          int32_t *__restrict__ meta) {
+                                                          int32_t *__restrict__ meta, MailPost post) {
   constexpr int kG = 8;
   __shared__ int seg_tot[kMaxSeg], seg_base[kMaxSeg + 1], carry_s[kMaxSeg];
   __shared__ int wtot[kG][16];
@@ -70,6 +71,11 @@
     }
     seg_base[n_seg] = acc;
     meta[0] = acc;
+    if (post.words != nullptr) {
+      mail_store(post, 0, acc);
+      for (int s = 0; s < n_seg; ++s) mail_store(post, 1 + s, seg_tot[s]);
+      mail_stamp(post, true);
+    }
   }
   __syncthreads();
   for (int s0 = 0; s0 < n_seg; s0 += kG) {
@@ -113,9 +119,11 @@
     const float *__restrict__ scores, int n, int n_cls, const int32_t *__restrict__ seg_class, int n_seg,
     float thr, int n_blocks, const int32_t *__restrict__ blk_off, const float *__restrict__ coords,
     const float *__restrict__ offsets, const int32_t *__restrict__ batch_idxs, int batch_size,
-    int32_t *__restrict__ obj, int32_t *__restrict__ seg_of, float *__restrict__ pts, int32_t *__restrict__ key) {
+    int32_t *__restrict__ obj, int32_t *__restrict__ seg_of, float *__restrict__ pts, int32_t *__restrict__ key,
+    int32_t *__restrict__ zero, int64_t n_zero) {
   __shared__ int wcnt[4];
   const int i = blockIdx.x * kSelBlock + threadIdx.x;
+  for (int64_t z = i; z < n_zero; z += static_cast<int64_t>(gridDim.x) * kSelBlock) zero[z] = 0;
   const int wave = threadIdx.x >> 6;
   float c[3] = {0.f, 0.f, 0.f};
   int bi = 0;
@@ -156,8 +164,9 @@
                                                           const int32_t *__restrict__ offsets, int n_prop,
                                                           const float *__restrict__ coords, float inv_ss,
                                                           float scale_max, float *__restrict__ cscale,
-                                                          float *__restrict__ lo_s) {
+                                                          float *__restrict__ lo_s, int32_t *__restrict__ bad) {
   __shared__ float rmin[3][256], rmax[3][256];
+  if (blockIdx.x == 0 && threadIdx.x == 0) bad[0] = 0;
   for (int p = blockIdx.x; p < n_prop; p += gridDim.x) {
     const int s = offsets[p], e = offsets[p + 1];
     float mn[3] = {INFINITY, INFINITY, INFINITY}, mx[3] = {-INFINITY, -INFINITY, -INFINITY};
@@ -289,7 +298,7 @@
                                                            int32_t *__restrict__ inst_of,
                                                            int32_t *__restrict__ kept_cls,
                                                            float *__restrict__ kept_score,
-                                                           int32_t *__restrict__ head) {
+                                                           int32_t *__restrict__ head, MailPost post) {
   __shared__ int wsum[16];
   __shared__ int cap_s;
   if (threadIdx.x == 0) cap_s = 0;
@@ -336,6 +345,31 @@
   if (threadIdx.x == 0) {
     head[0] = carry;
     head[1] = cap_s;
+    if (post.words != nullptr) {
+      mail_store(post, 0, carry);
+      mail_store(post, 1, cap_s);
+      mail_stamp(post, true);
+    }
+  }
+}
+
+__global__ void __launch_bounds__(256) instance_result_block_kernel(const int64_t *__restrict__ text_off,
+                                                                   const int32_t *__restrict__ kept_cls,
+                                                                   const float *__restrict__ kept_score, int n_kept,
+                                                                   int64_t *__restrict__ h_off, int32_t *__restrict__ h_cls,
+                                                                   float *__restrict__ h_score, MailPost post) {
+  for (int i = threadIdx.x; i <= n_kept; i += 256) h_off[i] = text_off[i];
+  for (int i = threadIdx.x; i < n_kept; i += 256) {
+    h_cls[i] = kept_cls[i];
+    h_score[i] = kept_score[i];
+  }
+  __threadfence_system();
+  __syncthreads();
+  if (threadIdx.x == 0) {
+    const int64_t tb = text_off[n_kept];
+    mail_store(post, 0, static_cast<int32_t>(tb & 0xffffffff));
+    mail_store(post, 1, static_cast<int32_t>(tb >> 32));
+    mail_stamp(post, true);
   }
 }
 
@@ -398,26 +432,8 @@
   size_t at(const void *p) const { return static_cast<size_t>(static_cast<const char *>(p) - base); }
 };
 
-__global__ void __launch_bounds__(64) read_back_kernel(const int32_t *__restrict__ dev, int words, int32_t *host) {
-  if (static_cast<int>(threadIdx.x) < words)
-    __hip_atomic_store(host + threadIdx.x, dev[threadIdx.x], __ATOMIC_RELAXED, __HIP_MEMORY_SCOPE_SYSTEM);
-}
 static int read_back(int32_t *host, const int32_t *dev, int words, hipStream_t stream, const char *what) {
-  static const bool by_kernel = getenv("SG_READBACK_KERNEL") && atoi(getenv("SG_READBACK_KERNEL")) != 0;
-  if (by_kernel && words <= 64) {
-    read_back_kernel<<<1, 64, 0, stream>>>(dev, words, host);
-    if (hipStreamSynchronize(stream) != hipSuccess) {
-      set_error("%s: device -> host read-back failed", what);
-      return SG_ERR_LAUNCH;
-    }
-    return SG_OK;
-  }
-  if (hipMemcpyAsync(host, dev, sizeof(int32_t) * words, hipMemcpyDeviceToHost, stream) != hipSuccess ||
-      hipStreamSynchronize(stream) != hipSuccess) {
-    set_error("%s: device -> host read-back failed", what);
-    return SG_ERR_LAUNCH;
-  }
-  return SG_OK;
+  return mailbox_fetch(mailbox_for(stream), dev, words, nullptr, 0, host, stream, what);
 }
 
 #define SG_TRY(expr)              \
@@ -449,18 +465,16 @@
   SG_TAKE(lo_s, float, 3 * static_cast<size_t>(n_prop));
   SG_TAKE(vox, int64_t, 4 * static_cast<size_t>(S));
   SG_TAKE(bad, int32_t, 64);
-  hipMemsetAsync(bad, 0, sizeof(int32_t), stream);
   const float inv_ss = 1.0f / static_cast<float>(cfg->voxel_shape);
   proposal_box_kernel<<<n_prop < 1024 ? n_prop : 1024, 256, 0, stream>>>(pairs, poff, n_prop, coords_float, inv_ss,
-                                                                        cfg->voxel_scale, cscale, lo_s);
+                                                                        cfg->voxel_scale, cscale, lo_s, bad);
   proposal_voxel_coords_kernel<<<grid_for(S, 256), 256, 0, stream>>>(pairs, S, coords_float, cscale, lo_s,
                                                                     cfg->voxel_shape, vox, bad);
   const size_t vx_bytes = sg_voxelize_idx_workspace_bytes(S);
   SG_TAKE(vx_ws, char, vx_bytes);
   SG_TAKE(inp_map, int32_t, S);
   SG_TRY(sg_voxelize_idx_build(vox, S, 4, 4, inp_map, meta + 40, vx_ws, vx_bytes, stream_));
-  hipMemcpyAsync(meta + 42, bad, sizeof(int32_t), hipMemcpyDeviceToDevice, stream);
-  SG_TRY(read_back(host, meta + 40, 3, stream, kWhat));
+  SG_TRY(mailbox_fetch(mailbox_for(stream), meta + 40, 2, bad, 1, host, stream, kWhat));
   const int M = host[0], mA = host[1];
   SG_REQUIRE(host[2] == 0, "%s: a proposal voxel coordinate fell outside [0, %d) "
              "(the reference asserts here, softgroup.py:698)", kWhat, cfg->voxel_shape);
@@ -507,9 +521,14 @@
   SG_TAKE(blk_off, int32_t, static_cast<size_t>(n_seg) * n_blocks);
   select_count_kernel<<<n_blocks, kSelBlock, 0, stream>>>(scores, n, cfg->n_sem_classes, cfg->seg_class, n_seg,
                                                          cfg->score_thr, n_blocks, blk_cnt);
-  select_scan_kernel<<<1, 1024, 0, stream>>>(blk_cnt, n_seg, n_blocks, cfg->min_npoint, blk_off, meta);
-  SG_TRY(check_launch(kWhat));
-  SG_TRY(read_back(host, meta, 1, stream, kWhat));
+  Mailbox *mb = mailbox_for(stream);
+  {
+    const MailPost post = mailbox_next(mb);
+    select_scan_kernel<<<1, 1024, 0, stream>>>(blk_cnt, n_seg, n_blocks, cfg->min_npoint, blk_off, meta, post);
+    SG_TRY(check_launch(kWhat));
+    if (mb != nullptr) SG_TRY(mailbox_wait(mb, post, meta, 1, host, kWhat));
+    else SG_TRY(read_back(host, meta, 1, stream, kWhat));
+  }
   const int n_sel = host[0];
   res->n_selected = n_sel;
   if (n_sel == 0) return SG_OK;
@@ -517,21 +536,23 @@
   SG_TAKE(seg_of, int32_t, n_sel);
   SG_TAKE(pts, float, 3 * static_cast<size_t>(n_sel));
   SG_TAKE(key, int32_t, n_sel);
-  select_emit_kernel<<<n_blocks, kSelBlock, 0, stream>>>(scores, n, cfg->n_sem_classes, cfg->seg_class, n_seg,
-                                                        cfg->score_thr, n_blocks, blk_off, coords_float,
-                                                        pt_offsets, batch_idxs, cfg->batch_size, obj, seg_of,
-                                                        pts, key);
-
   const size_t bq_bytes = sg_ballquery_workspace_bytes(n_sel);
   SG_TAKE(bq_ws, char, bq_bytes);
   SG_TAKE(start_len, int32_t, 2 * static_cast<size_t>(n_sel));
   const size_t sc_bytes = sg_scan_workspace_bytes(n_sel);
   SG_TAKE(sc_ws, char, sc_bytes);
-  hipMemsetAsync(start_len, 0, sizeof(int32_t) * 2 * n_sel, stream);
+  select_emit_kernel<<<n_blocks, kSelBlock, 0, stream>>>(scores, n, cfg->n_sem_classes, cfg->seg_class, n_seg,
+                                                        cfg->score_thr, n_blocks, blk_off, coords_float,
+                                                        pt_offsets, batch_idxs, cfg->batch_size, obj, seg_of,
+                                                        pts, key, start_len, 2 * static_cast<int64_t>(n_sel));
   SG_TRY(sg_ballquery_build_grid(pts, key, n_sel, cfg->radius, bq_ws, bq_bytes, stream_));
   SG_TRY(sg_ballquery_count(pts, key, n_sel, cfg->radius, start_len, nullptr, bq_ws, bq_bytes, stream_));
-  SG_TRY(sg_exclusive_scan_startlen(start_len, n_sel, meta + 32, sc_ws, sc_bytes, stream_));
-  SG_TRY(read_back(host, meta + 32, 1, stream, kWhat));
+  {
+    const MailPost post = mailbox_next(mb);
+    SG_TRY(exclusive_scan_startlen_post(start_len, n_sel, meta + 32, sc_ws, sc_bytes, stream_, post));
+    if (mb != nullptr) SG_TRY(mailbox_wait(mb, post, meta + 32, 1, host, kWhat));
+    else SG_TRY(read_back(host, meta + 32, 1, stream, kWhat));
+  }
   const int n_active = host[0];
   res->n_neighbours = n_active;
   SG_TAKE(bq_idx, int32_t, n_active);
@@ -547,7 +568,7 @@
   if (S == 0) return SG_OK;
   SG_TAKE(pairs, int32_t, 2 * static_cast<size_t>(S));
   SG_TAKE(poff, int32_t, static_cast<size_t>(n_prop) + 1);
-  hipMemsetAsync(poff, 0, sizeof(int32_t) * (n_prop + 1), stream);
+  fill_one(poff, sizeof(int32_t) * (static_cast<size_t>(n_prop) + 1), 0, stream);
   if (t_scan_emit_hook != nullptr) t_scan_emit_hook(t_scan_emit_ctx);
   SG_TRY(sg_bfs_cluster_emit(bq_idx, start_len, n_sel, n_active, seg_of, cfg->seg_thr, n_prop, S, pairs, poff,
                              bfs_ws, bfs_bytes, stream_));
@@ -587,7 +608,7 @@
   SG_TAKE(blk_off, int32_t, static_cast<size_t>(n_seg) * n_blocks);
   select_count_kernel<<<n_blocks, kSelBlock, 0, stream>>>(scores, n, cfg->n_sem_classes, cfg->seg_class, n_seg,
                                                          cfg->score_thr, n_blocks, blk_cnt);
-  select_scan_kernel<<<1, 1024, 0, stream>>>(blk_cnt, n_seg, n_blocks, cfg->min_npoint, blk_off, meta);
+  select_scan_kernel<<<1, 1024, 0, stream>>>(blk_cnt, n_seg, n_blocks, cfg->min_npoint, blk_off, meta, MailPost());
   SG_TRY(check_launch(kWhat));
   SG_TRY(read_back(host, meta, 1 + n_seg, stream, kWhat));
   const int n_sel = host[0];
@@ -602,7 +623,7 @@
   select_emit_kernel<<<n_blocks, kSelBlock, 0, stream>>>(scores, n, cfg->n_sem_classes, cfg->seg_class, n_seg,
                                                         cfg->score_thr, n_blocks, blk_off, coords_float,
                                                         pt_offsets, batch_idxs, cfg->batch_size, obj, seg_of,
-                                                        pts, key);
+                                                        pts, key, nullptr, 0);
   SG_TAKE(pairs, int32_t, 2 * static_cast<size_t>(n_sel));
   SG_TAKE(poff, int32_t, static_cast<size_t>(n_sel) + 2);
   int n_prop = 0, S = 0;
@@ -664,7 +685,7 @@
     SG_TAKE(start_len, int32_t, 2 * static_cast<size_t>(n_q));
     const size_t sc_bytes = sg_scan_workspace_bytes(n_q);
     SG_TAKE(sc_ws, char, sc_bytes);
-    hipMemsetAsync(start_len, 0, sizeof(int32_t) * 2 * n_q, stream);
+    fill_one(start_len, sizeof(int32_t) * 2 * static_cast<size_t>(n_q), 0, stream);
     int32_t *bq_idx = nullptr;
     int n_active = 0, flags = 0;
     if (pcfg->with_octree) {
@@ -714,7 +735,7 @@
     }
     SG_TAKE(cidx, int32_t, 2 * static_cast<size_t>(sp));
     SG_TAKE(coff, int32_t, static_cast<size_t>(nc) + 1);
-    hipMemsetAsync(coff, 0, sizeof(int32_t) * (nc + 1), stream);
+    fill_one(coff, sizeof(int32_t) * (static_cast<size_t>(nc) + 1), 0, stream);
     if (hook_pending) {
       t_scan_emit_hook(t_scan_emit_ctx);
       hook_pending = false;
@@ -797,10 +818,15 @@
   SG_TAKE(kept_score, float, static_cast<size_t>(nP) * nc);
   SG_TAKE(head, int32_t, 64);
   SG_TRY(sg_instance_npoint(proposals_idx, mask_scores, S, stride, nc, cfg->mask_score_thr, nP, npoint, stream_));
-  instance_keep_kernel<<<1, 1024, 0, stream>>>(cls_prob, iou_scores, stride, npoint, nP, nc, cfg->cls_score_thr,
-                                             cfg->min_npoint, inst_of, kept_cls, kept_score, head);
-  SG_TRY(check_launch(kWhat));
-  SG_TRY(read_back(host, head, 2, stream, kWhat));
+  Mailbox *mb = mailbox_for(stream);
+  {
+    const MailPost post = mailbox_next(mb);
+    instance_keep_kernel<<<1, 1024, 0, stream>>>(cls_prob, iou_scores, stride, npoint, nP, nc, cfg->cls_score_thr,
+                                               cfg->min_npoint, inst_of, kept_cls, kept_score, head, post);
+    SG_TRY(check_launch(kWhat));
+    if (mb != nullptr) SG_TRY(mailbox_wait(mb, post, head, 2, host, kWhat));
+    else SG_TRY(read_back(host, head, 2, stream, kWhat));
+  }
   const int n_kept = host[0];
   const int64_t cap = host[1] > 0 ? host[1] : 1;
   res->n_kept = n_kept;
@@ -828,14 +854,34 @@
     return SG_ERR_WORKSPACE;
   }
   char *h = static_cast<char *>(host_out);
-  if (hipMemcpyAsync(h, text_off, off_cls, hipMemcpyDeviceToHost, stream) != hipSuccess ||
-      hipMemcpyAsync(h + off_cls, kept_cls, sizeof(int32_t) * n_kept, hipMemcpyDeviceToHost, stream) != hipSuccess ||
-      hipMemcpyAsync(h + off_score, kept_score, sizeof(float) * n_kept, hipMemcpyDeviceToHost, stream) != hipSuccess ||
-      hipStreamSynchronize(stream) != hipSuccess) {
-    set_error("sg_scan_instances: result copy failed");
-    return SG_ERR_LAUNCH;
-  }
-  const int64_t text_bytes = reinterpret_cast<const int64_t *>(h)[n_kept];
+  void *h_dev = nullptr;
+  if (mb != nullptr && (hipHostGetDevicePointer(&h_dev, h, 0) != hipSuccess || h_dev == nullptr)) {
+    (void)hipGetLastError();
+    h_dev = nullptr;
+  }
+  int64_t text_bytes = 0;
+  if (mb != nullptr && h_dev != nullptr) {
+    char *hd = static_cast<char *>(h_dev);
+    const MailPost post = mailbox_next(mb);
+    instance_result_block_kernel<<<1, 256, 0, stream>>>(text_off, kept_cls, kept_score, n_kept,
+                                                       reinterpret_cast<int64_t *>(hd),
+                                                       reinterpret_cast<int32_t *>(hd + off_cls),
+                                                       reinterpret_cast<float *>(hd + off_score), post);
+    SG_TRY(check_launch(kWhat));
+    SG_TRY(mailbox_wait(mb, post, reinterpret_cast<const int32_t *>(text_off + n_kept), 2, host, kWhat));
+    text_bytes = static_cast<int64_t>(static_cast<uint32_t>(host[0])) | (static_cast<int64_t>(host[1]) << 32);
+    if (mb->last_path != 0) h_dev = nullptr;
+  }
+  if (mb == nullptr || h_dev == nullptr) {
+    if (hipMemcpyAsync(h, text_off, off_cls, hipMemcpyDeviceToHost, stream) != hipSuccess ||
+        hipMemcpyAsync(h + off_cls, kept_cls, sizeof(int32_t) * n_kept, hipMemcpyDeviceToHost, stream) != hipSuccess ||
+        hipMemcpyAsync(h + off_score, kept_score, sizeof(float) * n_kept, hipMemcpyDeviceToHost, stream) != hipSuccess ||
+        hipStreamSynchronize(stream) != hipSuccess) {
+      set_error("sg_scan_instances: result copy failed");
+      return SG_ERR_LAUNCH;
+    }
+    text_bytes = reinterpret_cast<const int64_t *>(h)[n_kept];
+  }
   res->host_needed = off_text + static_cast<size_t>(text_bytes);
   if (host_bytes < res->host_needed) {
     set_error("sg_scan_instances: host buffer too small (%zu bytes, need %zu)", host_bytes, res->host_needed);
diff --git a/softgroup_amd/csrc/spconv_rulebook.hip b/softgroup_amd/csrc/spconv_rulebook.hip
--- a/softgroup_amd/csrc/spconv_rulebook.hip
+++ b/softgroup_amd/csrc/spconv_rulebook.hip
@@ -3,6 +3,7 @@
 #include <mutex>
 
 #include "common.h"
+#include "mailbox.h"
 #include "radix_sort.h"
 #include "scan.h"
 
@@ -186,9 +187,15 @@
   }
 }
 
-__global__ void pyr_rows_kernel(const int32_t *__restrict__ pos, int M0, int L, int32_t *rows) {
+__global__ void __launch_bounds__(64) pyr_rows_kernel(const int32_t *__restrict__ pos, int M0, int L, int32_t *rows,
+                                                      MailPost post) {
   const int l = threadIdx.x;
-  if (l < L) rows[l] = pos[static_cast<size_t>(l + 1) * M0] - pos[static_cast<size_t>(l) * M0];
+  if (l < L) {
+    const int32_t r = pos[static_cast<size_t>(l + 1) * M0] - pos[static_cast<size_t>(l) * M0];
+    rows[l] = r;
+    if (post.words != nullptr) mail_store(post, l, r);
+  }
+  if (post.words != nullptr) mail_stamp(post, l == 0);
 }
 
 struct PyrOut {
@@ -611,6 +618,7 @@
   }
   const dim3 grid((max_rows + 255) / 256, P.n);
   plan_mask_all_kernel<<<grid, 256, 0, stream>>>(P, mask, val, freq);
+  host_mark("plans:mask");
   static const bool raw_env = getenv("SG_PLAN_RAW") != nullptr;
   if (raw_env) hipMemsetAsync(freq, 0, kPyrMaxSegs * 32 * 4, stream);
   plan_pos_all_kernel<<<P.n, 32, 0, stream>>>(P, freq, bitpos);
@@ -656,6 +664,7 @@
   if (mode == 0) plan_tile_order_all_kernel<<<P.n, 1024, 0, stream>>>(Q, tmask, torder);
   else plan_tile_order_xcd_kernel<<<dim3(P.n, 8), 1024, 0, stream>>>(Q, tmask, mode, torder);
   plan_emit_all_kernel<<<dim3(min((max_rows + 31) / 32, 2048), P.n), 256, 0, stream>>>(Q, val, tmask, torder);
+  host_mark("plans:emit");
   return check_launch(who);
 }
 
@@ -784,6 +793,13 @@
 
 int sg_spconv_pyramid_rows(const int32_t *indices, int M0, const int32_t *shape_host, int n_levels,
                            int32_t *rows_dev, void *ws, size_t ws_bytes, sg_stream_t stream_) {
+  return spconv_pyramid_rows_post(indices, M0, shape_host, n_levels, rows_dev, ws, ws_bytes, stream_, MailPost());
+}
+
+}
+
+int sg::spconv_pyramid_rows_post(const int32_t *indices, int M0, const int32_t *shape_host, int n_levels,
+                                 int32_t *rows_dev, void *ws, size_t ws_bytes, sg_stream_t stream_, MailPost post) {
   SG_REQUIRE(M0 >= 0 && shape_host && rows_dev && n_levels >= 1 && n_levels <= kPyrMaxLevels,
              "sg_spconv_pyramid_rows: bad arguments (M0=%d n_levels=%d)", M0, n_levels);
   hipStream_t stream = as_stream(stream_);
@@ -801,11 +817,14 @@
     FillList f;
     f.add(w.keys, static_cast<size_t>(L) * w.cap * 8, 0xff);
     f.add(w.vals, static_cast<size_t>(L) * w.cap * 4, 0x7f);
+    host_mark("rows:enter");
     fill_many(f, stream);
   }
+  host_mark("rows:fill");
   const Shape3 shape{shape_host[0], shape_host[1], shape_host[2]};
   pyr_insert_kernel<<<(M0 + 255) / 256, 256, 0, stream>>>(indices, M0, shape, L, w.keys, w.vals, w.cap,
                                                          w.slot);
+  host_mark("rows:insert");
   const int32_t *slot = w.slot, *vals = w.vals;
   int32_t *pos = w.pos;
   const int m0 = M0;
@@ -819,9 +838,13 @@
       },
       [pos] __device__(int64_t t, int v) { pos[t] = v; }, n, pos + n, w.scan_ws, w.scan_bytes, stream);
   if (rc != SG_OK) return rc;
-  pyr_rows_kernel<<<1, 64, 0, stream>>>(w.pos, M0, L, rows_dev);
+  host_mark("rows:scan");
+  pyr_rows_kernel<<<1, 64, 0, stream>>>(w.pos, M0, L, rows_dev, post);
+  host_mark("rows:tail");
   return check_launch("sg_spconv_pyramid_rows");
 }
+
+extern "C" {
 
 static long long pyr_seg_rows(const sg_pyramid_level *lv, int L, int seg_kind, int l) {
   return seg_kind == 1 ? lv[l + 1].rows : lv[l].rows;
@@ -920,6 +943,7 @@
         indices, M0, L, w.vals, w.rowtab, w.cap, w.slot, w.pos, o);
   }
   pyr_subm_kernel<<<grid_for(o.pre27[L], 256, 8192), 256, 0, stream>>>(L, w.keys, w.rowtab, w.cap, o);
+  host_mark("build:subm");
   return build_plans(P, ws2, ws2_bytes, false, stream, "sg_spconv_pyramid_build");
 }
 
diff --git a/softgroup_amd/csrc/unet_exec.hip b/softgroup_amd/csrc/unet_exec.hip
--- a/softgroup_amd/csrc/unet_exec.hip
+++ b/softgroup_amd/csrc/unet_exec.hip
@@ -6,6 +6,7 @@
 #include <stdlib.h>
 
 #include "common.h"
+#include "mailbox.h"
 #include "radix_sort.h"
 #include "unet_common.h"
 
@@ -206,9 +207,14 @@
   }
   const size_t pws_bytes = sg_spconv_pyramid_workspace_bytes(num_rows, L);
   SG_IALLOC(pws, char, pws_bytes);
-  SG_TRY(sg_spconv_pyramid_rows(indices, num_rows, spatial_shape_host, L, st.dev_rows, pws, pws_bytes, is));
-  if (hipMemcpyAsync(st.host_rows, st.dev_rows, sizeof(int32_t) * L, hipMemcpyDeviceToHost, istream) != hipSuccess ||
-      hipStreamSynchronize(istream) != hipSuccess) {
+  Mailbox *mb = num_rows > 0 ? mailbox_for(istream) : nullptr;
+  const MailPost post = mailbox_next(mb);
+  SG_TRY(spconv_pyramid_rows_post(indices, num_rows, spatial_shape_host, L, st.dev_rows, pws, pws_bytes, is, post));
+  if (mb != nullptr) {
+    SG_TRY(mailbox_wait(mb, post, st.dev_rows, L, st.host_rows, who));
+    host_mark("index:rows-wait");
+  } else if (hipMemcpyAsync(st.host_rows, st.dev_rows, sizeof(int32_t) * L, hipMemcpyDeviceToHost, istream) != hipSuccess ||
+             hipStreamSynchronize(istream) != hipSuccess) {
     set_error("%s: reading the level row counts failed", who);
     return SG_ERR_LAUNCH;
   }
@@ -257,6 +263,7 @@
   {
     const size_t nb = sg_spconv_pyramid_build_workspace_bytes(pl, L);
     SG_IALLOC(ws2, char, nb);
+    host_mark("index:tables");
     SG_TRY(sg_spconv_pyramid_build(indices, num_rows, spatial_shape_host, L, pl, pws, pws_bytes, ws2, nb, is));
   }
   if (L > 1) {
@@ -283,6 +290,7 @@
   }
   *used = ix.off;
   *lock = std::move(guard);
+  host_mark_flush(who);
   return SG_OK;
 }
 
diff --git a/softgroup_amd/csrc/voxelize_idx.hip b/softgroup_amd/csrc/voxelize_idx.hip
--- a/softgroup_amd/csrc/voxelize_idx.hip
+++ b/softgroup_amd/csrc/voxelize_idx.hip
@@ -165,12 +165,18 @@
     set_error("sg_voxelize_idx_build: workspace too small");
     return SG_ERR_WORKSPACE;
   }
-  const int32_t init_meta[2] = {0, 1};
-  hipMemcpyAsync(meta, init_meta, sizeof(init_meta), hipMemcpyHostToDevice, stream);
-  if (n == 0) return SG_OK;
+  if (n == 0) {
+    FillList f;
+    f.add_words(meta, 1, 0u);
+    f.add_words(meta + 1, 1, 1u);
+    fill_many(f, stream);
+    return check_launch("sg_voxelize_idx_build");
+  }
   const int grid = (n + 255) / 256;
   {
     FillList f;
+    f.add_words(meta, 1, 0u);
+    f.add_words(meta + 1, 1, 1u);
     f.add(w.table, static_cast<size_t>(w.cap) * 4, 0x7f);
     f.add(w.count, static_cast<size_t>(n) * 4, 0);
     f.add(w.last, static_cast<size_t>(n) * 4, 0);
```
